# granularai/fabric

Measured on AMD Instinct MI355X. Metric: patch-pairs/sec (fwd+bwd) 13-band 128x128, higher is better.
Workload: dtype bf16

## Files before the change

fabric_amd/_lib.py:

```python
import ctypes as C
import os

_HERE = os.path.dirname(os.path.abspath(__file__))
LIB_PATH = os.environ.get('BIDATE_LIB') or os.path.join(_HERE, 'csrc', 'libbidate_hip.so')

BDN_F32, BDN_BF16, BDN_BF16X3, BDN_BF16X2 = 0, 1, 2, 3
IN_PLAIN, IN_BNRELU = 0, 1
EVAL_STAGE, EVAL_PAIR, EVAL_CLS = 0, 1, 2
WG_SIMPLE, WG_ROLE = 1, 5


def wg_flags(phases=3, kernel=0, blocks=0):
    return phases | (kernel << 8) | (blocks << 16)

_vp, _i, _f, _sz, _i64 = C.c_void_p, C.c_int, C.c_float, C.c_size_t, C.c_int64
_hf = C.POINTER(C.c_float)

SIGNATURES = {
    'bdn_last_error': (C.c_char_p, []),
    'bdn_version': (_i, []),
    'bdn_stream_create': (_i, [_i, C.POINTER(C.c_void_p)]),
    'bdn_stream_destroy': (_i, [_vp]),
    'bdn_event_create': (_i, [C.POINTER(C.c_void_p)]),
    'bdn_event_destroy': (_i, [_vp]),
    'bdn_event_record': (_i, [_vp, _vp]),
    'bdn_stream_wait_event': (_i, [_vp, _vp]),
    'bdn_pack_input': (_i, [_i, _vp, _vp, _vp, _i, _i, _i, _i, _i, _vp]),
    'bdn_pack_weights': (_i, [_i, _vp, _vp, _vp, _i, _i, _i, _vp]),
    'bdn_pack_weights_multi': (_i, [_i, _vp, _i, _vp]),
    'bdn_conv3x3': (_i, [_i, _vp, _i, _vp, _i, _i, _vp, _i, _vp, _vp, _vp, _vp, _i, _i, _i, _i, _vp]),
    'bdn_conv3x3_x3src': (_i, [_i, _vp, _i, _i, _vp, _i, _vp, _vp, _vp, _vp, _vp, _i, _i, _i, _i, _vp]),
    'bdn_conv3x3_num_mtiles': (_i, [_i, _i, _i, _i, _i]),
    'bdn_conv3x3_num_mtiles_ex': (_i, [_i, _i, _i, _i, _i, _i, _i]),
    'bdn_wgrad_workspace_bytes': (_sz, [_i, _i, _i, _i, _i, _i]),
    'bdn_conv3x3_wgrad': (_i, [_i, _vp, _i, _vp, _i, _vp, _i, _i, _vp, _i, _vp, _vp, _i, _i, _i, _i, _vp]),
    'bdn_conv3x3_wgrad_ex': (_i, [_i, _vp, _i, _vp, _i, _vp, _i, _i, _vp, _i, _vp, _vp, _i, _i, _i, _i, _i, _vp]),
    'bdn_conv3x3_wgrad_variant': (_i, [_i, _i, _i, _i, _i, _i, _i, _i, _i, _i]),
    'bdn_wgrad_workspace_bytes_ex': (_sz, [_i, _i, _i, _i, _i, _i, _i, _i, _i, _i]),
    'bdn_conv3x3_wgrad_bnbwd_supported': (_i, [_i, _i, _i, _i, _i, _i, _i]),
    'bdn_conv3x3_wgrad_bnbwd': (_i, [_i, _vp, _i, _vp, _vp, _vp, _i, _i, _vp, _i, _vp, _vp, _i, _i, _i, _i, _vp]),
    'bdn_conv3x3_dgrad_first': (_i, [_i, _vp, _i, _vp, _vp, _vp, _i, _vp, _i, _vp, _vp, _i, _i, _i, _vp]),
    'bdn_bn_finalize_workspace_bytes': (_sz, [_i, _i, _i]),
    'bdn_bn_finalize': (_i, [_vp, _i, _i, _i, _i, _vp, _vp, _f, _f, _vp, _vp, _vp, _vp, _vp, _vp]),
    'bdn_bn_eval': (_i, [_vp, _vp, _vp, _vp, _f, _i, _i, _vp, _vp]),
    'bdn_bn_eval_fold_multi': (_i, [_vp, _i, _i, _f, _vp]),
    'bdn_conv3x3_eval': (_i, [_i, _vp, _i, _vp, _i, _vp, _vp, _vp, _vp, _vp, _vp, _i, _i, _i, _i, _vp]),
    'bdn_conv3x3_eval_pair': (_i, [_i, _vp, _i, _vp, _vp, _vp, _vp, _vp, _i, _i, _i, _i, _vp]),
    'bdn_conv3x3_eval_cls': (_i, [_i, _vp, _i, _vp, _vp, _vp, _vp, _vp, _vp, _i, _vp, _vp, _vp, _i, _i, _i, _i, _i, _i, _vp]),
    'bdn_bn_bwd_workspace_bytes': (_sz, [_i, _i, _i, _i, _i, _i]),
    'bdn_bn_bwd': (_i, [_i, _vp, _i, _vp, _vp, _i, _i, _i, _i, _i, _vp, _vp, _vp, _vp, _vp, _vp]),
    'bdn_conv3d_num_mtiles': (_i, [_i, _i, _i, _i]),
    'bdn_conv3d': (_i, [_i, _vp, _i, _i, _vp, _i, _vp, _vp, _vp, _vp, _i, _i, _i, _i, _i, _vp]),
    'bdn_conv3d_wgrad': (_i, [_i, _vp, _i, _vp, _i, _vp, _vp, _i, _i, _i, _i, _i, _vp]),
    'bdn_split_pack': (_i, [_vp, _i, _vp, _i, _i, _vp, _i, _vp, _i, _i, _i, _vp]),
    'bdn_bnrelu': (_i, [_i, _vp, _vp, _i, _vp, _i, _i, _i, _i, _vp]),
    'bdn_bnrelu_pool': (_i, [_i, _vp, _vp, _i, _vp, _i, _i, _i, _i, _vp]),
    'bdn_fuse_product': (_i, [_i, _vp, _vp, _vp, _i, _i, _i, _i, _vp]),
    'bdn_product_pool': (_i, [_i, _vp, _vp, _vp, _vp, _i, _i, _i, _i, _vp]),
    'bdn_upsample2x': (_i, [_i, _vp, _i, _vp, _vp, _i, _i, _i, _i, _i, _i, _vp]),
    'bdn_product_pool_split': (_i, [_vp, _vp, _vp, _i, _i, _vp, _i, _i, _i, _i, _vp]),
    'bdn_upsample2x_split': (_i, [_vp, _i, _vp, _vp, _i, _i, _i, _i, _i, _i, _i, _i, _i, _vp]),
    'bdn_upsample2x_bwd': (_i, [_i, _vp, _i, _vp, _i, _i, _i, _i, _i, _i, _vp]),
    'bdn_upsample2x_bwd_rows': (_i, [_i, _i, _i, _i, _i]),
    'bdn_upsample2x_bwd_bs': (_i, [_i, _vp, _i, _vp, _vp, _vp, _vp, _i, _i, _i, _i, _i, _i, _vp]),
    'bdn_enc_skip_bwd': (_i, [_i, _vp, _i, _vp, _vp, _vp, _vp, _vp, _i, _i, _i, _i, _vp]),
    'bdn_enc_skip_bwd_rows': (_i, [_i, _i, _i, _i, _i]),
    'bdn_outc_fwd': (_i, [_i, _vp, _vp, _vp, _vp, _vp, _i, _i, _i, _i, _i, _vp]),
    'bdn_outc_bwd_workspace_bytes': (_sz, [_i, _i, _i, _i, _i, _i]),
    'bdn_outc_bwd': (_i, [_i, _vp, _vp, _vp, _vp, _vp, _vp, _vp, _vp, _vp, _i, _i, _i, _i, _i, _vp]),
    'bdn_outc_bn_bwd_apply': (_i, [_i, _vp, _vp, _vp, _vp, _i, _vp, _vp, _i, _i, _i, _i, _i, _vp]),
    'bdn_outc_bwd_rows': (_i, [_i, _i, _i, _i, _i]),
    'bdn_overlap_workspace_bytes': (_sz, [_i, _i, _i, _i, _i]),
    'bdn_tversky': (_i, [_vp, _vp, _f, _f, _f, _vp, _vp, _vp, _vp, _i, _i, _i, _i, _vp]),
    'bdn_conv3x3_variant': (C.c_char_p, [_i, _i, _i, _i, _i, _i, _i, _i]),
    'bdn_conv3x3_dgrad_bb_variant': (C.c_char_p, [_i, _i, _i, _i, _i]),
    'bdn_conv3x3_eval_variant': (C.c_char_p, [_i, _i, _i, _i, _i, _i, _i, _i]),
    'bdn_conv3x3_x3src_variant': (C.c_char_p, [_i, _i, _i, _i, _i, _i, _i]),
    'bdn_conv3x3_dgrad_bs': (_i, [_i, _vp, _i, _vp, _vp, _vp, _vp, _i, _vp, _i, _i, _i, _i, _vp]),
    'bdn_conv3x3_dgrad_bb': (_i, [_i, _vp, _i, _vp, _vp, _vp, _i, _vp, _vp, _vp, _vp, _vp, _vp, _i, _i, _i, _i, _vp]),
    'bdn_bn_bwd_scratch_bytes': (_sz, [_i, _i]),
    'bdn_bn_bwd_finalize': (_i, [_vp, _i, _i, _vp, _i, _i, _vp, _vp, _vp, _vp, _vp]),
    'bdn_bn_bwd_apply': (_i, [_i, _vp, _i, _vp, _vp, _i, _i, _i, _i, _i, _vp, _i, _i, _vp, _vp, _vp, _vp, _vp, _vp]),
    'bdn_bn_bwd_apply_split': (_i, [_vp, _i, _vp, _vp, _i, _i, _i, _i, _i, _vp, _i, _i, _vp, _vp, _vp, _vp, _vp, _vp]),
    'bdn_bn_bwd_finalize_frozen': (_i, [_vp, _i, _i, _vp, _i, _i, _vp, _vp, _vp, _vp, _vp, _vp]),
    'bdn_bn_bwd_apply_frozen': (_i, [_i, _vp, _i, _vp, _vp, _i, _i, _i, _i, _i, _vp, _i, _i, _vp, _vp, _vp, _vp, _vp, _vp, _vp]),
    'bdn_bn_bwd_frozen': (_i, [_i, _vp, _i, _vp, _vp, _i, _i, _i, _i, _i, _vp, _vp, _vp, _vp, _vp, _vp, _vp]),
    'bdn_overlap_loss': (_i, [_vp, _vp, _f, _f, _f, _i, _vp, _vp, _vp, _vp, _i, _i, _i, _i, _vp]),
    'bdn_focal_workspace_bytes': (_sz, []),
    'bdn_focal': (_i, [_vp, _vp, _f, _vp, _i, _vp, _vp, _vp, _vp, _i, _i, _i, _i, _vp]),
    'bdn_criterion_workspace_bytes': (_sz, [_i, _i, _i, _i, _i]),
    'bdn_criterion': (_i, [_vp, _vp, _f, _f, _f, _f, _i, _f, _f, _vp, _i, _vp, _vp, _vp, _vp, _vp, _i, _i, _i, _i, _vp]),
    'bdn_ingest_band': (_i, [_i, _vp, _i, _i, _f, _f, _vp, _i, _i, _vp]),
    'bdn_gather_tiles': (_i, [_i, _vp, _vp, _vp, _vp, _i, _i, _i, _i, _i, _i, _vp]),
    'bdn_upload_band': (_i, [_vp, _vp, _i, _i, _i, _i, _i, _vp]),
    'bdn_argmax': (_i, [_vp, _vp, _i, _i, _i, _i, _vp]),
    'bdn_argmax_stitch': (_i, [_vp, _vp, _vp, _i, _i, _i, _i, _i, _vp]),
    'bdn_gather_tiles_sym': (_i, [_i, _vp, _vp, _vp, _vp, _i, _i, _i, _i, _i, _i, _vp]),
    'bdn_blend_fold': (_i, [_vp, _vp, _vp, _vp, _i, _i, _i, _vp]),
    'bdn_blend_stitch': (_i, [_vp, _vp, _vp, _vp, C.c_longlong, _i, _i, _i, _i, _i, _i, _i, _vp]),
    'bdn_blend_finalize': (_i, [_vp, _vp, _vp, _i, _i, _i, _vp]),
    'bdn_sample_patches': (_i, [_vp, _vp, _i, _i, _vp, _vp, _i, _i, _vp, _vp, _vp, _vp]),
    'bdn_sgd_step': (_i, [_vp, _vp, _f, _f, _sz, _vp]),
    'bdn_sgd_momentum_step': (_i, [_vp, _vp, _vp, _f, _f, _f, _f, _f, _i, _i, _sz, _vp]),
    'bdn_adam_step': (_i, [_vp, _vp, _vp, _vp, _f, _f, C.c_double, C.c_double, _f, _f, _i, _i64, _sz, _vp]),
    'bdn_sgd_step_grouped': (_i, [_vp, _vp, _vp, _vp, _i, _i, _vp, _f, _sz, _vp]),
    'bdn_sgd_momentum_step_grouped': (_i, [_vp, _vp, _vp, _vp, _vp, _i, _i, _vp, _vp, _f, _f, _f, _i, _i, _sz, _vp]),
    'bdn_adam_step_grouped': (_i, [_vp, _vp, _vp, _vp, _vp, _vp, _i, _i, _vp, _vp, _f, C.c_double, C.c_double, _f, _i, _i64, _sz, _vp]),
    'bdn_sgd_step_grouped_ex': (_i, [_vp, _vp, _vp, _vp, _i, _i, _hf, _f, _vp, _sz, _vp]),
    'bdn_sgd_momentum_step_grouped_ex': (_i, [_vp, _vp, _vp, _vp, _vp, _i, _i, _hf, _hf, _f, _vp, _f, _f, _i, _i, _sz, _vp]),
    'bdn_adam_step_grouped_ex': (_i, [_vp, _vp, _vp, _vp, _vp, _vp, _i, _i, _hf, _hf, _f, _vp, C.c_double, C.c_double, _f, _i, _i64, _sz,
                                      _vp]),
    'bdn_grad_accumulate': (_i, [_vp, _vp, _sz, _i, _vp]),
    'bdn_grad_norm_workspace_bytes': (_sz, [_sz]),
    'bdn_grad_norm': (_i, [_vp, _vp, _vp, _i, _f, _f, _vp, _vp, _sz, _vp]),
}


def floats(values):
    return (C.c_float * len(values))(*values)

_lib = None


def load():
    global _lib
    if _lib is not None:
        return _lib
    if not os.path.exists(LIB_PATH):
        raise RuntimeError(
            f'fabric_amd: HIP extension {LIB_PATH} not found. Build it with '
            f'`python -c "import __graft_entry__ as g; g.build()"` or `make -C fabric_amd/csrc`. '
            f'There is no CPU fallback.')
    lib = C.CDLL(LIB_PATH)
    for name, (res, args) in SIGNATURES.items():
        fn = getattr(lib, name)
        fn.restype = res
        fn.argtypes = args
    _lib = lib
    return lib


def ptr(t):
    return None if t is None else t.data_ptr()


PROFILE = None
PHASE = ''
_ext_streams = {}


def _profiled(lib, name, args):
    import torch
    h = args[-1] or 0
    st = _ext_streams.get(h)
    if st is None:
        st = _ext_streams[h] = torch.cuda.ExternalStream(h) if h else torch.cuda.default_stream()
    e0, e1 = torch.cuda.Event(enable_timing=True), torch.cuda.Event(enable_timing=True)
    e0.record(st)
    rc = getattr(lib, name)(*args)
    e1.record(st)
    PROFILE.append((name, PHASE, h, e0, e1))
    return rc


SKIP = None


def call(name, *args):
    lib = load()
    if SKIP is not None and SKIP(name, args):
        return
    if PROFILE is not None and SIGNATURES[name][1] and SIGNATURES[name][1][-1] is _vp and not name.startswith(('bdn_stream', 'bdn_event')):
        rc = _profiled(lib, name, args)
    else:
        rc = getattr(lib, name)(*args)
    if rc != 0:
        msg = lib.bdn_last_error().decode(errors='replace')
        raise RuntimeError(f'{name} failed (rc={rc}): {msg}')


def stream_ptr():
    import torch
    return torch.cuda.current_stream().cuda_stream
```

fabric_amd/csrc/head.hip:

```cpp
#include "common.hpp"

static inline unsigned grid_for(size_t n, int block = 256) { return (unsigned)((n + block - 1) / block); }

template <typename T>
__global__ void pack_input_kernel(const float* __restrict__ x1, const float* __restrict__ x2, T* __restrict__ out,
                                  int B, int C, int H, int W, int Cpad, FastDiv dhw, FastDiv dupp) {
    constexpr int EPU = ET<T>::EPU;
    const int upp = Cpad / EPU;
    const size_t hw = (size_t)H * W, total = (size_t)2 * B * hw * upp;
    const size_t i = (size_t)blockIdx.x * blockDim.x + threadIdx.x;
    if (i >= total) return;
    int ti, pi, n, u; dhw.divmod((int)i, ti, pi); dupp.divmod(ti, n, u);
    const size_t p = pi;
    const float* src = (n < B ? x1 + (size_t)n * C * hw : x2 + (size_t)(n - B) * C * hw) + p;
    float f[EPU];
#pragma unroll
    for (int e = 0; e < EPU; e++) { const int c = u * EPU + e; f[e] = c < C ? src[(size_t)c * hw] : 0.f; }
    *reinterpret_cast<uint4*>(out + ((size_t)n * hw + p) * Cpad + u * EPU) = Unit<T>::pack(f);
}

__global__ void pack_input_split_kernel(const float* __restrict__ x1, const float* __restrict__ x2, bf16s* __restrict__ out,
                                        int B, int C, int H, int W, int Cpad, FastDiv dhw, FastDiv dupp) {
    const int upp = Cpad / 8;
    const size_t hw = (size_t)H * W, total = (size_t)2 * B * hw * upp;
// ... 110 lines not shown
            if (wf) {
                const int tap = rec_l >> 2, kq = rec_l & 3;
                const size_t rec = ((size_t)cb * 9 + tap) * (d.Cin / 16) + (ci0 / 16 + kq);
                *reinterpret_cast<uint4*>(wf + rec * 512 + lane * 8) =
                    *reinterpret_cast<const uint4*>(t + (lane & 31) * ROW + tap * 64 + kq * 16 + (lane >> 5) * 8);
            }
            if (wd) {
                const int cbi = rec_l / 18, rem = rec_l % 18, tap = rem >> 1, kg = rem & 1;
                const int ci = cbi * 32 + (lane & 31), co8 = kg * 16 + (lane >> 5) * 8;
                unsigned short h[8];
#pragma unroll
                for (int e = 0; e < 8; e++) h[e] = t[(co8 + e) * ROW + tap * 64 + ci];
                const size_t rec = ((size_t)(ci0 / 32 + cbi) * 9 + (8 - tap)) * (d.Cout / 16) + (co0 / 16 + kg);
                *reinterpret_cast<uint4*>(wd + rec * 512 + lane * 8) =
                    make_uint4(h[0] | ((unsigned)h[1] << 16), h[2] | ((unsigned)h[3] << 16), h[4] | ((unsigned)h[5] << 16), h[6] | ((unsigned)h[7] << 16));
            }
        }
    }
}
__global__ void pack_weights_irregular_kernel(const PackDesc* __restrict__ desc) {
    if (pack_regular(desc[blockIdx.y])) return;
    constexpr int EPU = 8, KCH = 16, REC = 64 * EPU;
    const PackDesc d = desc[blockIdx.y];
    const size_t total = (size_t)d.Cout * 9 * d.Cinp;
    bf16s* wf = reinterpret_cast<bf16s*>(d.wf); bf16s* wd = reinterpret_cast<bf16s*>(d.wd);
    for (size_t i = (size_t)blockIdx.x * blockDim.x + threadIdx.x; i < total; i += (size_t)gridDim.x * blockDim.x) {
        const int e = i % EPU, lane = (i / EPU) % 64; const size_t rec = i / REC;
        if (wf) {
            const int kgi = rec % (d.Cinp / KCH); const size_t t = rec / (d.Cinp / KCH); const int tap = t % 9, cb = t / 9;
            const int co = cb * 32 + (lane & 31), ci = kgi * KCH + (lane >> 5) * EPU + e;
            wf[i] = from_f<bf16s>(ci < d.Cin ? d.w[((size_t)co * d.Cin + ci) * 9 + tap] : 0.f);
        }
        if (wd) {
            const int kgi = rec % (d.Cout / KCH); const size_t t = rec / (d.Cout / KCH); const int tap = t % 9, cb = t / 9;
            const int ci = cb * 32 + (lane & 31), co = kgi * KCH + (lane >> 5) * EPU + e;
            wd[i] = from_f<bf16s>(ci < d.Cin ? d.w[((size_t)co * d.Cin + ci) * 9 + (8 - tap)] : 0.f);
        }
    }
}

extern "C" int bdn_pack_weights_multi(int dtype, const void* desc, int n_layers, void* stream) {
    if (!desc || n_layers <= 0) BDN_FAIL(BDN_E_ARG, "pack_weights_multi: bad arguments");
    hipStream_t st = (hipStream_t)stream;
    if (dtype == BDN_BF16) {
        hipLaunchKernelGGL(pack_weights_tiles_kernel, dim3(1024), dim3(256), 0, st, (const PackDesc*)desc, n_layers);
        hipLaunchKernelGGL(pack_weights_irregular_kernel, dim3(32, n_layers), dim3(256), 0, st, (const PackDesc*)desc);
    }
    else if (dtype == BDN_F32) hipLaunchKernelGGL(pack_weights_multi_kernel<float>, dim3(256, n_layers), dim3(256), 0, st, (const PackDesc*)desc);
    else if (dtype == BDN_BF16X3) return bdn_pack_weights_x3_multi((const PackDesc*)desc, n_layers, st);
    else BDN_FAIL(BDN_E_ARG, "pack_weights_multi: bad dtype");
    BDN_CHECK_LAUNCH("pack_weights_multi");
    return BDN_OK;
}

constexpr int OUTC_MAXCLS = 8;
constexpr int OUTC_ITERS = 16;
constexpr int OUTC_BWD_ITERS = 32;
template <typename T, int NC, int CUC = 0>
__global__ __launch_bounds__(256) void outc_fwd_kernel(const T* __restrict__ z, const float* __restrict__ bn, const float* __restrict__ w,
                                const float* __restrict__ bias, float* __restrict__ logits, int npix, int hw, int C, int ncls, FastDiv dhw) {
    constexpr int EPU = ET<T>::EPU;
    const int CU = CUC ? CUC : C / EPU, rows = 256 / CU, tid = threadIdx.x, cu = tid % CU, row = tid / CU, c = cu * EPU;
    float sc[EPU], sh[EPU], wk[NC][EPU], bk[NC];
#pragma unroll
    for (int i = 0; i < EPU; i++) { sc[i] = bn_row(bn, 0, 2, C)[c + i]; sh[i] = bn_row(bn, 0, 3, C)[c + i]; }
#pragma unroll
    for (int k = 0; k < NC; k++) {
        const int kk = k < ncls ? k : 0;
        const float bv = bias[kk];
        bk[k] = k < ncls ? bv : 0.f;
#pragma unroll
        for (int i = 0; i < EPU; i++) { const float wv = w[kk * C + c + i]; wk[k][i] = k < ncls ? wv : 0.f; }
    }
    const int p_begin = blockIdx.x * rows * OUTC_ITERS, p_end = min(npix, p_begin + rows * OUTC_ITERS);
    uint4 u[4], un[4];
#define OUTC_LOAD4(dst_, p0_, RAGGED_)                                                                   \
    _Pragma("unroll") for (int j = 0; j < 4; j++) {                                                      \
        const int p_ = (p0_) + j * rows + row;                                                          \
        dst_[j] = *reinterpret_cast<const uint4*>(z + (size_t)(!(RAGGED_) || p_ < p_end ? p_ : (p0_)) * C + c); \
    }
#define OUTC_RUN(RAGGED_)                                                                                \
    {                                                                                                   \
        OUTC_LOAD4(u, p_begin, RAGGED_)                                                                 \
        for (int p0 = p_begin; p0 < p_end; p0 += 4 * rows) {                       \
            const bool more = p0 + 4 * rows < p_end;                                                    \
             \
                                    \
            { const int pn_ = more ? p0 + 4 * rows : p0; OUTC_LOAD4(un, pn_, RAGGED_) }                  \
            _Pragma("unroll") for (int j = 0; j < 4; j++) {                                              \
                const int p = p0 + j * rows + row;                                                      \
                if ((RAGGED_) && p0 + j * rows >= p_end) break;                      \
                const bool in_ = !(RAGGED_) || p < p_end;                                               \
                float f[EPU], acc[NC];                                                                  \
                _Pragma("unroll") for (int k = 0; k < NC; k++) acc[k] = 0.f;                             \
                Unit<T>::unpack(u[j], f);                                                               \
                _Pragma("unroll") for (int i = 0; i < EPU; i++) {                                        \
                    const float a = to_f(from_f<T>(fmaxf(fmaf(f[i], sc[i], sh[i]), 0.f)));              \
                    _Pragma("unroll") for (int k = 0; k < NC; k++) acc[k] = fmaf(a, wk[k][i], acc[k]);   \
                }                                                                                       \
                if constexpr (CUC != 0) {                                                               \
                    _Pragma("unroll") for (int k = 0; k < NC; k++) acc[k] = first_lane_sum<CUC ? CUC : 8>(acc[k]); \
                } else {                                                                                \
                    _Pragma("unroll") for (int k = 0; k < NC; k++)                                       \
                        for (int off = CU >> 1; off > 0; off >>= 1) acc[k] += __shfl_xor(acc[k], off);  \
                }                                                                                       \
                if (cu == 0 && in_) {                                                                   \
                    int b, q; dhw.divmod(p, b, q);                                                      \
                    _Pragma("unroll") for (int k = 0; k < NC; k++) if (k < ncls) logits[((size_t)b * ncls + k) * hw + q] = acc[k] + bk[k]; \
                }                                                                                       \
            }                                                                                           \
            _Pragma("unroll") for (int j = 0; j < 4; j++) u[j] = un[j];                                  \
        }                                                                                               \
    }
    if (p_begin >= p_end) return;
    if (p_begin + rows * OUTC_ITERS <= npix) OUTC_RUN(false) else OUTC_RUN(true)
#undef OUTC_RUN
#undef OUTC_LOAD4
}

extern "C" int bdn_outc_fwd(int dtype, const void* z, const float* bn, const float* w, const float* b,
                            float* logits, int B, int H, int W, int C, int ncls, void* stream) {
    if (!z || !bn || !w || !b || !logits) BDN_FAIL(BDN_E_ARG, "outc_fwd: null pointer");
    if (ncls < 1 || ncls > OUTC_MAXCLS || C % 16 || C > 512 || 512 % C) BDN_FAIL(BDN_E_SHAPE, "outc_fwd: ncls=%d (max %d), C=%d", ncls, OUTC_MAXCLS, C);
    hipStream_t st = (hipStream_t)stream; const int npix = B * H * W, hw = H * W;
    if (dtype == BDN_BF16) {
        const int per = 256 / (C / 8) * OUTC_ITERS; const unsigned grid = (npix + per - 1) / per;
        if (ncls <= 2 && C == 64) hipLaunchKernelGGL((outc_fwd_kernel<bf16s, 2, 8>), dim3(grid), dim3(256), 0, st, (const bf16s*)z, bn, w, b, logits, npix, hw, C, ncls, FastDiv(hw));
        else if (ncls <= 2) hipLaunchKernelGGL((outc_fwd_kernel<bf16s, 2>), dim3(grid), dim3(256), 0, st, (const bf16s*)z, bn, w, b, logits, npix, hw, C, ncls, FastDiv(hw));
        else hipLaunchKernelGGL((outc_fwd_kernel<bf16s, OUTC_MAXCLS>), dim3(grid), dim3(256), 0, st, (const bf16s*)z, bn, w, b, logits, npix, hw, C, ncls, FastDiv(hw));
    } else if (dtype == BDN_F32) {
        const int per = 256 / (C / 4) * OUTC_ITERS; const unsigned grid = (npix + per - 1) / per;
        if (ncls <= 2 && C == 64) hipLaunchKernelGGL((outc_fwd_kernel<float, 2, 16>), dim3(grid), dim3(256), 0, st, (const float*)z, bn, w, b, logits, npix, hw, C, ncls, FastDiv(hw));
        else if (ncls <= 2) hipLaunchKernelGGL((outc_fwd_kernel<float, 2>), dim3(grid), dim3(256), 0, st, (const float*)z, bn, w, b, logits, npix, hw, C, ncls, FastDiv(hw));
        else hipLaunchKernelGGL((outc_fwd_kernel<float, OUTC_MAXCLS>), dim3(grid), dim3(256), 0, st, (const float*)z, bn, w, b, logits, npix, hw, C, ncls, FastDiv(hw));
    }
    else BDN_FAIL(BDN_E_ARG, "outc_fwd: bad dtype");
    BDN_CHECK_LAUNCH("outc_fwd");
    return BDN_OK;
}

template <typename T, int NC, int CUC = 0>
__global__ __launch_bounds__(256) void outc_bwd_kernel(const float* __restrict__ dl, const T* __restrict__ z, const float* __restrict__ bn,
                                const float* __restrict__ w, T* __restrict__ dA, float* __restrict__ wpart,
                                float* __restrict__ bs_partial, int npix, int hw, int C, int ncls, FastDiv dhw) {
    constexpr int EPU = ET<T>::EPU;
    extern __shared__ float sm[];
    const int CU = CUC ? CUC : C / EPU, rows = 256 / CU, tid = threadIdx.x, cu = tid % CU, row = tid / CU, c = cu * EPU;
    for (int i = tid; i < ncls * (C + 1); i += 256) sm[i] = 0.f;
    float sc[EPU], sh[EPU], wk[NC][EPU], acc[NC][EPU], accb[NC], t0[EPU], t1[EPU];
#pragma unroll
    for (int i = 0; i < EPU; i++) { sc[i] = bn_row(bn, 0, 2, C)[c + i]; sh[i] = bn_row(bn, 0, 3, C)[c + i]; t0[i] = 0.f; t1[i] = 0.f; }
    const bool bs = bs_partial != nullptr;
#pragma unroll
    for (int k = 0; k < NC; k++) {
        accb[k] = 0.f;
        const int kk = k < ncls ? k : 0;
#pragma unroll
        for (int i = 0; i < EPU; i++) { const float wv = w[kk * C + c + i]; wk[k][i] = k < ncls ? wv : 0.f; acc[k][i] = 0.f; }
    }
    __syncthreads();
    const int p_begin = blockIdx.x * rows * OUTC_BWD_ITERS, p_end = min(npix, p_begin + rows * OUTC_BWD_ITERS);
    uint4 zu[4], zn[4]; float gv[4][NC], gn[4][NC];
#define OUTC_BLOAD4(zd_, gd_, p0_)                                                                       \
    _Pragma("unroll") for (int j = 0; j < 4; j++) {                                                      \
        const int pj_ = (p0_) + j * rows + row < p_end ? (p0_) + j * rows + row : p_begin + row;          \
        int b_, q_; dhw.divmod(pj_, b_, q_);                                                            \
        _Pragma("unroll") for (int k = 0; k < NC; k++) gd_[j][k] = dl[((size_t)b_ * ncls + (k < ncls ? k : 0)) * hw + q_]; \
        zd_[j] = *reinterpret_cast<const uint4*>(z + (size_t)pj_ * C + c);                              \
    }
    if (p_begin + row < p_end) {
        OUTC_BLOAD4(zu, gv, p_begin)
        for (int p0 = p_begin; p0 < p_end; p0 += 4 * rows) {
            { const int pn_ = p0 + 4 * rows < p_end ? p0 + 4 * rows : p0; OUTC_BLOAD4(zn, gn, pn_) }
#pragma unroll
            for (int j = 0; j < 4; j++) {
                const int p = p0 + j * rows + row;
                if (p < p_end) {
                    float g[NC], f[EPU], o[EPU];
#pragma unroll
                    for (int k = 0; k < NC; k++) g[k] = k < ncls ? gv[j][k] : 0.f;
                    Unit<T>::unpack(zu[j], f);
#pragma unroll
                    for (int i = 0; i < EPU; i++) {
                        const float a = to_f(from_f<T>(fmaxf(fmaf(f[i], sc[i], sh[i]), 0.f)));
                        float s = 0.f;
#pragma unroll
                        for (int k = 0; k < NC; k++) if (k < ncls) { s = fmaf(g[k], wk[k][i], s); acc[k][i] = fmaf(g[k], a, acc[k][i]); }
                        o[i] = s;
                    }
                    if (cu == 0) {
#pragma unroll
                        for (int k = 0; k < NC; k++) accb[k] += g[k];
                    }
                    const uint4 uo = Unit<T>::pack(o);
                    if (dA) *reinterpret_cast<uint4*>(dA + (size_t)p * C + c) = uo;
                    if (bs) {
                        Unit<T>::unpack(uo, o);
#pragma unroll
                        for (int i = 0; i < EPU; i++) {
                            const float gm = fmaf(f[i], sc[i], sh[i]) > 0.f ? o[i] : 0.f;
                            t0[i] += gm; t1[i] = fmaf(gm, f[i], t1[i]);
                        }
                    }
                }
            }
#pragma unroll
            for (int j = 0; j < 4; j++) {
                zu[j] = zn[j];
#pragma unroll
                for (int k = 0; k < NC; k++) gv[j][k] = gn[j][k];
            }
        }
    }
#undef OUTC_BLOAD4
    {
        float* red = sm + ncls * (C + 1);
#pragma unroll
        for (int k = 0; k < NC; k++) {
            if (k < ncls) {
                __syncthreads();
#pragma unroll
                for (int i = 0; i < EPU; i++) red[tid * EPU + i] = acc[k][i];
                if (cu == 0) red[256 * EPU + row] = accb[k];
                __syncthreads();
                for (int o = tid; o <= C; o += 256) {
                    float v = 0.f;
                    if (o < C) { const int ccu = o / EPU, i = o % EPU; for (int r = 0; r < rows; r++) v += red[(r * CU + ccu) * EPU + i]; }
                    else for (int r = 0; r < rows; r++) v += red[256 * EPU + r];
                    sm[k * (C + 1) + o] = v;
                }
            }
        }
    }
    __syncthreads();
    for (int i = tid; i < ncls * (C + 1); i += 256)
        wpart[(size_t)blockIdx.x * ncls * (C + 1) + i] = sm[i];
    if (bs) {
        float* sred = sm + ncls * (C + 1);
#pragma unroll
        for (int i = 0; i < EPU; i++) { sred[(tid * EPU + i) * 2] = t0[i]; sred[(tid * EPU + i) * 2 + 1] = t1[i]; }
        __syncthreads();
        for (int o = tid; o < C * 2; o += 256) {
            const int k = o & 1, cc = o >> 1, ccu = cc / EPU, i = cc % EPU;
            float v = 0.f;
            for (int r = 0; r < rows; r++) v += sred[((r * CU + ccu) * EPU + i) * 2 + k];
            bs_partial[((size_t)blockIdx.x * 2 + k) * C + cc] = v;
        }
    }
}

__global__ __launch_bounds__(256) void outc_dw_reduce_kernel(const float* __restrict__ wpart, int rows, int C, int ncls,
                                                             float* __restrict__ dw, float* __restrict__ db) {
    __shared__ float sm[256];
    const int o = blockIdx.x, n = ncls * (C + 1);
    float a = 0.f;
    for (int r = threadIdx.x; r < rows; r += 256) a += wpart[(size_t)r * n + o];
    sm[threadIdx.x] = a;
    __syncthreads();
    for (int st = 128; st >= 1; st >>= 1) {
        if ((int)threadIdx.x < st) sm[threadIdx.x] += sm[threadIdx.x + st];
        __syncthreads();
    }
    if (threadIdx.x == 0) {
        const int k = o / (C + 1), cc = o % (C + 1);
        if (cc < C) dw[k * C + cc] = sm[0]; else db[k] = sm[0];
    }
}

extern "C" int bdn_outc_bwd_rows(int dtype, int B, int H, int W, int C) {
    if (B <= 0 || H <= 0 || W <= 0 || C <= 0 || C % 16 || C > 1024 || 1024 % C) return 0;
    const int per = 256 / (C / (dtype == BDN_BF16 ? 8 : 4)) * OUTC_BWD_ITERS;
    return (B * H * W + per - 1) / per;
}

extern "C" size_t bdn_outc_bwd_workspace_bytes(int dtype, int B, int H, int W, int C, int ncls) {
    const int rows = bdn_outc_bwd_rows(dtype, B, H, W, C);
    if (rows <= 0 || ncls < 1 || ncls > OUTC_MAXCLS) return 0;
    return (size_t)rows * ncls * (C + 1) * sizeof(float);
}

extern "C" int bdn_outc_bwd(int dtype, const float* dlogits, const void* z, const float* bn, const float* w,
                            void* dA, float* dw, float* db, float* bs_partial, float* ws, int B, int H, int W, int C, int ncls, void* stream) {
    if (!dlogits || !z || !bn || !w || !dw || !db || !ws) BDN_FAIL(BDN_E_ARG, "outc_bwd: null pointer");
    if (!dA && !bs_partial) BDN_FAIL(BDN_E_ARG, "outc_bwd: dA may be omitted only together with bs_partial (bdn_outc_bn_bwd_apply recomputes it)");
    if (ncls < 1 || ncls > OUTC_MAXCLS || C % 16 || C > 1024 || 1024 % C) BDN_FAIL(BDN_E_SHAPE, "outc_bwd: bad shape");
    hipStream_t st = (hipStream_t)stream; const int npix = B * H * W;
    const unsigned grid = bdn_outc_bwd_rows(dtype, B, H, W, C);
    const size_t smem = sizeof(float) * (ncls * (C + 1) + 256 * (dtype == BDN_BF16 ? 8 : 4) * 2);
    if (dtype == BDN_BF16) {
        if (ncls <= 2 && C == 64) hipLaunchKernelGGL((outc_bwd_kernel<bf16s, 2, 8>), dim3(grid), dim3(256), smem, st, dlogits, (const bf16s*)z, bn, w, (bf16s*)dA, ws, bs_partial, npix, H * W, C, ncls, FastDiv(H * W));
        else if (ncls <= 2) hipLaunchKernelGGL((outc_bwd_kernel<bf16s, 2>), dim3(grid), dim3(256), smem, st, dlogits, (const bf16s*)z, bn, w, (bf16s*)dA, ws, bs_partial, npix, H * W, C, ncls, FastDiv(H * W));
        else hipLaunchKernelGGL((outc_bwd_kernel<bf16s, OUTC_MAXCLS>), dim3(grid), dim3(256), smem, st, dlogits, (const bf16s*)z, bn, w, (bf16s*)dA, ws, bs_partial, npix, H * W, C, ncls, FastDiv(H * W));
    } else if (dtype == BDN_F32) {
        if (ncls <= 2 && C == 64) hipLaunchKernelGGL((outc_bwd_kernel<float, 2, 16>), dim3(grid), dim3(256), smem, st, dlogits, (const float*)z, bn, w, (float*)dA, ws, bs_partial, npix, H * W, C, ncls, FastDiv(H * W));
        else if (ncls <= 2) hipLaunchKernelGGL((outc_bwd_kernel<float, 2>), dim3(grid), dim3(256), smem, st, dlogits, (const float*)z, bn, w, (float*)dA, ws, bs_partial, npix, H * W, C, ncls, FastDiv(H * W));
        else hipLaunchKernelGGL((outc_bwd_kernel<float, OUTC_MAXCLS>), dim3(grid), dim3(256), smem, st, dlogits, (const float*)z, bn, w, (float*)dA, ws, bs_partial, npix, H * W, C, ncls, FastDiv(H * W));
    } else BDN_FAIL(BDN_E_ARG, "outc_bwd: bad dtype");
    BDN_CHECK_LAUNCH("outc_bwd");
    hipLaunchKernelGGL(outc_dw_reduce_kernel, dim3(ncls * (C + 1)), dim3(256), 0, st, ws, (int)grid, C, ncls, dw, db);
    BDN_CHECK_LAUNCH("outc_dw_reduce");
    return BDN_OK;
}

template <typename T, int NC, bool SPLIT = false>
__global__ __launch_bounds__(256) void outc_bn_bwd_apply_kernel(const float* __restrict__ dl, const float* __restrict__ w,
                                const T* __restrict__ z, const float* __restrict__ bn, const float* __restrict__ sums,
                                T* __restrict__ dz, int npix, int hw, int pix_per_group, int pix_per_block, int C, int ncls, FastDiv dhw, FastDiv dppg) {
    constexpr int EPU = ET<T>::EPU;
    const int CU = C / EPU, rows = 256 / CU, tid = threadIdx.x, cu = tid % CU, row = tid / CU, c = cu * EPU;
    const int p_begin = blockIdx.x * pix_per_block, p_end = min(npix, p_begin + pix_per_block);
    if (p_begin >= p_end) return;
    const float invM = 1.f / (float)pix_per_group;
    int gcur = -1;
    float mean[EPU], inv[EPU], sc[EPU], sh[EPU], k0[EPU], k1[EPU], wk[NC][EPU];
#pragma unroll
    for (int k = 0; k < NC; k++)
#pragma unroll
        for (int i = 0; i < EPU; i++) wk[k][i] = k < ncls ? w[k * C + c + i] : 0.f;
    for (int pb = p_begin + row; pb < p_end; pb += 4 * rows) {
        uint4 zu[4]; float gv[4][NC];
#pragma unroll
        for (int j = 0; j < 4; j++) {
            const int pj = pb + j * rows < p_end ? pb + j * rows : pb;
            int b, q; dhw.divmod(pj, b, q);
#pragma unroll
            for (int k = 0; k < NC; k++) gv[j][k] = k < ncls ? dl[((size_t)b * ncls + k) * hw + q] : 0.f;
            zu[j] = *reinterpret_cast<const uint4*>(z + (size_t)pj * C + c);
        }
#pragma unroll
        for (int j = 0; j < 4; j++) {
            const int p = pb + j * rows;
            if (p >= p_end) break;
            const int g = dppg.div(p);
            if (g != gcur) {
                gcur = g;
#pragma unroll
                for (int i = 0; i < EPU; i++) {
                    mean[i] = bn_row(bn, g, 0, C)[c + i]; inv[i] = bn_row(bn, g, 1, C)[c + i];
                    sc[i] = bn_row(bn, g, 2, C)[c + i]; sh[i] = bn_row(bn, g, 3, C)[c + i];
                    k0[i] = sums[((size_t)g * 2 + 0) * C + c + i] * invM;
                    k1[i] = sums[((size_t)g * 2 + 1) * C + c + i] * invM;
                }
            }
            float fz[EPU], o[EPU];
            Unit<T>::unpack(zu[j], fz);
#pragma unroll
            for (int i = 0; i < EPU; i++) {
                float s = 0.f;
#pragma unroll
                for (int k = 0; k < NC; k++) if (k < ncls) s = fmaf(gv[j][k], wk[k][i], s);
                o[i] = s;
            }
            Unit<T>::unpack(Unit<T>::pack(o), o);
#pragma unroll
            for (int i = 0; i < EPU; i++) {
                const float gm = fmaf(fz[i], sc[i], sh[i]) > 0.f ? o[i] : 0.f;
                const float xhat = (fz[i] - mean[i]) * inv[i];
                o[i] = sc[i] * (gm - k0[i] - xhat * k1[i]);
            }
            if constexpr (SPLIT) {
                const SplitOut so = {reinterpret_cast<bf16s*>(dz), 2 * C, 0, C};
                store_split4(so, (size_t)p, c, o);
            } else
            *reinterpret_cast<uint4*>(dz + (size_t)p * C + c) = Unit<T>::pack(o);
        }
    }
}

extern "C" int bdn_outc_bn_bwd_apply(int dtype, const float* dlogits, const float* w, const void* z, const float* bn,
                                     int imgs_per_group, const float* sums, void* dz, int B, int H, int W, int C, int ncls, void* stream) {
    if (!dlogits || !w || !z || !bn || !sums || !dz) BDN_FAIL(BDN_E_ARG, "outc_bn_bwd_apply: null pointer");
    if (ncls < 1 || ncls > OUTC_MAXCLS || C % 16 || C > 1024 || 1024 % C || B <= 0 || H <= 0 || W <= 0 || imgs_per_group <= 0 || B % imgs_per_group)
        BDN_FAIL(BDN_E_SHAPE, "outc_bn_bwd_apply: bad shape");
    hipStream_t st = (hipStream_t)stream;
    const int npix = B * H * W, epu = dtype == BDN_BF16 ? 8 : 4, rows = 256 / (C / epu);
    int ppb = (npix + 2047) / 2048; if (ppb < 2 * rows) ppb = 2 * rows; ppb = (ppb + rows - 1) / rows * rows;
    const unsigned grid = (npix + ppb - 1) / ppb;
    if (dtype == BDN_BF16X3) {
#define OUTC_APPLY_S(NC_) hipLaunchKernelGGL((outc_bn_bwd_apply_kernel<float, NC_, true>), dim3(grid), dim3(256), 0, st, dlogits, w, (const float*)z, bn, sums, \
                                               (float*)dz, npix, H * W, imgs_per_group * H * W, ppb, C, ncls, FastDiv(H * W), FastDiv(imgs_per_group * H * W))
        if (ncls <= 2) OUTC_APPLY_S(2); else OUTC_APPLY_S(OUTC_MAXCLS);
#undef OUTC_APPLY_S
        BDN_CHECK_LAUNCH("outc_bn_bwd_apply");
        return BDN_OK;
    }
#define OUTC_APPLY(T_, NC_) hipLaunchKernelGGL((outc_bn_bwd_apply_kernel<T_, NC_>), dim3(grid), dim3(256), 0, st, dlogits, w, (const T_*)z, bn, sums, \
                                               (T_*)dz, npix, H * W, imgs_per_group * H * W, ppb, C, ncls, FastDiv(H * W), FastDiv(imgs_per_group * H * W))
    if (dtype == BDN_BF16) { if (ncls <= 2) OUTC_APPLY(bf16s, 2); else OUTC_APPLY(bf16s, OUTC_MAXCLS); }
    else if (dtype == BDN_F32) { if (ncls <= 2) OUTC_APPLY(float, 2); else OUTC_APPLY(float, OUTC_MAXCLS); }
    else BDN_FAIL(BDN_E_ARG, "outc_bn_bwd_apply: bad dtype");
#undef OUTC_APPLY
    BDN_CHECK_LAUNCH("outc_bn_bwd_apply");
    return BDN_OK;
}

struct FocalStats { const float* calpha; float gamma; double* part; };
__device__ __forceinline__ float focal_mod(float pt, float gamma) { return gamma == 0.f ? 1.f : powf(fmaxf(1.f - pt, 0.f), gamma); }

template <int NC, bool FOCAL = false>
__global__ void tversky_sums_kernel(const float* __restrict__ logits, const uint8_t* __restrict__ labels,
                                    float* __restrict__ part, int32_t* __restrict__ pcounts, int B, int ncls, int H, int W,
                                    int rows_per_block, int We, FastDiv dH, FocalStats fs = {}) {
    extern __shared__ float sm[];
    const int CW = blockDim.y, RL = blockDim.x;
    const int cl = threadIdx.y, rl = threadIdx.x;
    const int x = blockIdx.x * CW + cl;
    const size_t hw = (size_t)H * W;
    float tp[NC], fp[NC], fn[NC];
#pragma unroll
    for (int k = 0; k < NC; k++) { tp[k] = 0.f; fp[k] = 0.f; fn[k] = 0.f; }
    int c_tp = 0, c_fp = 0, c_fn = 0, c_ok = 0;
    double facc = 0.0;
    const int rows = B * H, r_end = min(rows, (int)(blockIdx.y + 1) * rows_per_block);
    if (x < W)
        for (int r0 = blockIdx.y * rows_per_block + rl; r0 < r_end; r0 += 4 * RL) {
            float lv[4][NC]; int tv[4];
#pragma unroll
            for (int u = 0; u < 4; u++) {
                const int r = r0 + u * RL;
                const int rr = r < r_end ? r : r0;
                int b, y; dH.divmod(rr, b, y);
                const size_t q = (size_t)y * W + x;
#pragma unroll
                for (int k = 0; k < NC; k++) lv[u][k] = k < ncls ? logits[((size_t)b * ncls + k) * hw + q] : -INFINITY;
                tv[u] = labels[(size_t)b * hw + q];
            }
#pragma unroll
            for (int u = 0; u < 4; u++) {
                if (r0 + u * RL >= r_end) break;
                float l[NC]; float m = -INFINITY; int am = 0;
#pragma unroll
                for (int k = 0; k < NC; k++) { l[k] = lv[u][k]; if (l[k] > m) { m = l[k]; am = k; } }
                float den = 0.f;
#pragma unroll
                for (int k = 0; k < NC; k++) { l[k] = k < ncls ? expf(l[k] - m) : 0.f; den += l[k]; }
                const int t = tv[u];
                const float inv = 1.f / den;
                float pt = 0.f;
#pragma unroll
                for (int k = 0; k < NC; k++) {
                    const float p = l[k] * inv;
                    if (t == k) { tp[k] += p; fn[k] += 1.f - p; pt = p; } else fp[k] += p;
                }
                if constexpr (FOCAL) {
                    float ltm = 0.f;
#pragma unroll
                    for (int k = 0; k < NC; k++) if (k < ncls && t == k) ltm = lv[u][k] - m;
                    const float a = t < ncls ? (fs.calpha ? fs.calpha[t] : 1.f) : 0.f;
                    facc += (double)(-focal_mod(pt, fs.gamma) * a * (ltm - logf(den)));
                }
                c_tp += (am == 1 && t == 1); c_fp += (am == 1 && t != 1); c_fn += (am != 1 && t == 1); c_ok += (am == t);
            }
        }
#pragma unroll
    for (int k = 0; k < NC; k++) {
        sm[(rl * 3 * NC + 0 * NC + k) * CW + cl] = tp[k];
        sm[(rl * 3 * NC + 1 * NC + k) * CW + cl] = fp[k];
        sm[(rl * 3 * NC + 2 * NC + k) * CW + cl] = fn[k];
    }
    __syncthreads();
    const int nblk_lin = blockIdx.y * gridDim.x + blockIdx.x;
    if (We == W) {
        if (rl == 0 && x < W)
            for (int k = 0; k < ncls; k++)
#pragma unroll
                for (int j = 0; j < 3; j++) {
                    float v = 0.f;
                    for (int r = 0; r < RL; r++) v += sm[(r * 3 * NC + j * NC + k) * CW + cl];
                    part[(size_t)blockIdx.y * 3 * ncls * W + (j * ncls + k) * W + x] = v;
                }
    } else {
        const int tid = rl + RL * cl;
        if (tid < 3 * NC) {
            float v = 0.f;
            for (int i = 0; i < RL * CW; i++) {
                const int r = i / CW, c = i % CW;
                if (blockIdx.x * CW + c < W) v += sm[(r * 3 * NC + tid) * CW + c];
            }
            const int j = tid / NC, k = tid % NC;
            if (k < ncls) part[(size_t)nblk_lin * 3 * ncls + j * ncls + k] = v;
        }
    }
    {
        int* ism = reinterpret_cast<int*>(sm);
        __syncthreads();
        const int tid = rl * CW + cl;
        ism[tid * 4 + 0] = c_tp; ism[tid * 4 + 1] = c_fp; ism[tid * 4 + 2] = c_fn; ism[tid * 4 + 3] = c_ok;
        __syncthreads();
        if (tid < 4) { int v = 0; for (int i = 0; i < 256; i++) v += ism[i * 4 + tid]; pcounts[nblk_lin * 4 + tid] = v; }
        if constexpr (FOCAL) {
            double* dsm = reinterpret_cast<double*>(sm);
            __syncthreads();
            dsm[tid] = facc;
            __syncthreads();
            for (int s = 128; s > 0; s >>= 1) { if (tid < s) dsm[tid] += dsm[tid + s]; __syncthreads(); }
            if (tid == 0) fs.part[nblk_lin] = dsm[0];
        }
    }
}

struct FocalFinish { const double* part; int nfp; double scale; float w_o, w_f; float* terms; };
template <bool FOCAL = false>
__global__ __launch_bounds__(1024) void tversky_finish_kernel(float* __restrict__ sums, const float* __restrict__ part, int nblk,
                                      const int32_t* __restrict__ pcounts, int ncblk, int32_t* __restrict__ counts,
                                      float alpha, float beta, float eps, int ncls, int W, float* __restrict__ loss,
                                      FocalFinish ff = {}) {
    __shared__ double red[256];
    __shared__ float4 lane_sums[1024];
    const int n = 3 * ncls * W, tid = threadIdx.x;
    if (n % 4 == 0 && n / 4 <= 1024) {
        const int n4 = n / 4, LN = 1024 / n4 > 0 ? (1024 / n4 > 16 ? 16 : 1024 / n4) : 1;
        const int q = tid % n4, l = tid / n4;
        float4 a = make_float4(0.f, 0.f, 0.f, 0.f);
        if (l < LN) {
#pragma unroll 8
            for (int b = l; b < nblk; b += LN) {
                const float4 v = *reinterpret_cast<const float4*>(part + (size_t)b * n + 4 * q);
                a.x += v.x; a.y += v.y; a.z += v.z; a.w += v.w;
            }
            lane_sums[tid] = a;
        }
        __syncthreads();
        if (l == 0) {
            for (int k = 1; k < LN; k++) { const float4 v = lane_sums[k * n4 + q]; a.x += v.x; a.y += v.y; a.z += v.z; a.w += v.w; }
            *reinterpret_cast<float4*>(sums + 4 * q) = a;
        }
    } else {
        for (int i = tid; i < n; i += 1024) {
            float a = 0.f;
            for (int b = 0; b < nblk; b++) a += part[(size_t)b * n + i];
            sums[i] = a;
        }
    }
    if (counts) {
        int* ired = reinterpret_cast<int*>(lane_sums);
        __syncthreads();
        const int j = tid & 3, l = tid >> 2;
        int v = 0;
        for (int b = l; b < ncblk; b += 256) v += pcounts[b * 4 + j];
        ired[tid] = v;
        __syncthreads();
        for (int s2 = 512; s2 >= 4; s2 >>= 1) { if (tid < s2) ired[tid] += ired[tid + s2]; __syncthreads(); }
        if (tid < 4) counts[tid] = ired[tid];
    }
    __syncthreads();
    double acc = 0.0;
    const int nc = ncls * W;
    if (tid < 256)
        for (int i = tid; i < nc; i += 256) {
            const float tp = sums[i], fp = sums[nc + i], fn = sums[2 * nc + i];
            const float D = tp + alpha * fp + beta * fn + eps;
            acc += (double)(tp / D);
            sums[i] = 1.f / D; sums[nc + i] = tp / (D * D);
        }
    if (tid < 256) red[tid] = acc;
    __syncthreads();
    for (int s = 128; s > 0; s >>= 1) { if (tid < s) red[tid] += red[tid + s]; __syncthreads(); }
    if constexpr (FOCAL) {
        const float ov = (float)(1.0 - red[0] / nc);
        __syncthreads();
        double f = 0.0;
        if (tid < 256) { for (int i = tid; i < ff.nfp; i += 256) f += ff.part[i]; red[tid] = f; }
        __syncthreads();
        for (int s = 128; s > 0; s >>= 1) { if (tid < s) red[tid] += red[tid + s]; __syncthreads(); }
        if (tid == 0) {
            const float fo = (float)(red[0] * ff.scale);
            *loss = ff.w_o * ov + ff.w_f * fo;
            if (ff.terms) { ff.terms[0] = ov; ff.terms[1] = fo; }
        }
    } else
    if (tid == 0) *loss = (float)(1.0 - red[0] / nc);
}

struct FocalBwd { const float* calpha; float gamma, gscale, w_o, w_f; };
template <bool FOCAL = false>
__global__ void tversky_bwd_kernel(const float* __restrict__ logits, const uint8_t* __restrict__ labels,
                                   const float* __restrict__ coef, float alpha, float beta, float* __restrict__ dlogits,
                                   int B, int ncls, int H, int Wimg, int W, FastDiv dhw, FastDiv dWimg, FocalBwd fb = {}) {
    const size_t hw = (size_t)H * Wimg, npix = (size_t)B * hw;
    const size_t p = (size_t)blockIdx.x * blockDim.x + threadIdx.x;
    if (p >= npix) return;
    int bi, qi, yi, xi; dhw.divmod((int)p, bi, qi); dWimg.divmod(qi, yi, xi);
    const size_t b = bi, q = qi; const int x = W == 1 ? 0 : xi;
    const int n = ncls * W;
    float l[OUTC_MAXCLS], dp[OUTC_MAXCLS]; float m = -INFINITY;
#pragma unroll
    for (int k = 0; k < OUTC_MAXCLS; k++) if (k < ncls) { l[k] = logits[(b * ncls + k) * hw + q]; m = fmaxf(m, l[k]); }
    float den = 0.f;
#pragma unroll
    for (int k = 0; k < OUTC_MAXCLS; k++) if (k < ncls) { l[k] = expf(l[k] - m); den += l[k]; }
    const int t = labels[p];
    const float norm = -1.f / (float)n;
    float dot = 0.f;
#pragma unroll
    for (int k = 0; k < OUTC_MAXCLS; k++) if (k < ncls) {
        l[k] /= den;
        const float invD = coef[k * W + x], tpD2 = coef[n + k * W + x];
        const float tk = t == k ? 1.f : 0.f;
        dp[k] = norm * (tk * invD - tpD2 * (tk + alpha * (1.f - tk) - beta * tk));
        dot += l[k] * dp[k];
    }
    if constexpr (FOCAL) {
        float pt = 0.f;
#pragma unroll
        for (int k = 0; k < OUTC_MAXCLS; k++) if (k < ncls && k == t) pt = l[k];
        const float a = t < ncls ? (fb.calpha ? fb.calpha[t] : 1.f) : 0.f;
        const float c = -focal_mod(pt, fb.gamma) * a * fb.gscale;
#pragma unroll
        for (int k = 0; k < OUTC_MAXCLS; k++) if (k < ncls)
            dlogits[(b * ncls + k) * hw + q] = fb.w_o * (l[k] * (dp[k] - dot)) + fb.w_f * (c * ((k == t ? 1.f : 0.f) - l[k]));
    } else {
#pragma unroll
    for (int k = 0; k < OUTC_MAXCLS; k++) if (k < ncls) dlogits[(b * ncls + k) * hw + q] = l[k] * (dp[k] - dot);
    }
}

struct OverlapPlan { int We, CW, RL, rpb, gx, gy, nblk, n; };
static OverlapPlan overlap_plan(int B, int ncls, int H, int W, int reduce_w) {
    OverlapPlan p;
    p.We = reduce_w ? 1 : W;
    p.CW = 1; while (p.CW < W && p.CW < 256) p.CW *= 2;
    p.RL = 256 / p.CW;
    const int rows = B * H;
    p.rpb = (rows + 255) / 256; if (p.rpb < p.RL) p.rpb = p.RL;
    p.gx = (W + p.CW - 1) / p.CW; p.gy = (rows + p.rpb - 1) / p.rpb;
    p.nblk = reduce_w ? p.gx * p.gy : p.gy;
    p.n = 3 * ncls * p.We;
    return p;
}
extern "C" size_t bdn_overlap_workspace_bytes(int B, int ncls, int H, int W, int reduce_w) {
    if (B <= 0 || H <= 0 || W <= 0 || ncls < 2 || ncls > OUTC_MAXCLS) return 0;
    const OverlapPlan p = overlap_plan(B, ncls, H, W, reduce_w);
    return sizeof(float) * ((size_t)p.n * (p.nblk + 1) + 8) + sizeof(int32_t) * 4 * p.gx * p.gy;
}

extern "C" int bdn_overlap_loss(const float* logits, const uint8_t* labels, float alpha, float beta, float eps,
                                int reduce_w, float* ws, float* loss, int32_t* counts, float* dlogits,
                                int B, int ncls, int H, int W, void* stream) {
    if (!logits || !labels || !ws || !loss) BDN_FAIL(BDN_E_ARG, "overlap_loss: null pointer");
    if (ncls < 2 || ncls > OUTC_MAXCLS) BDN_FAIL(BDN_E_SHAPE, "overlap_loss: ncls=%d unsupported (2..%d)", ncls, OUTC_MAXCLS);
    if (B <= 0 || H <= 0 || W <= 0 || (size_t)B * H * W >= ((size_t)1 << 31)) BDN_FAIL(BDN_E_SHAPE, "overlap_loss: bad shape");
    hipStream_t st = (hipStream_t)stream;
    const OverlapPlan p = overlap_plan(B, ncls, H, W, reduce_w);
    const int We = p.We;
    float* part = ws + p.n;
    int32_t* pcounts = reinterpret_cast<int32_t*>(part + (size_t)p.nblk * p.n);
    dim3 grid(p.gx, p.gy), block(p.RL, p.CW);
    if (ncls <= 2) hipLaunchKernelGGL((tversky_sums_kernel<2, false>), grid, block, sizeof(float) * 256 * 3 * 2, st, logits, labels, part, pcounts, B, ncls, H, W, p.rpb, We, FastDiv(H), FocalStats{});
    else hipLaunchKernelGGL((tversky_sums_kernel<OUTC_MAXCLS, false>), grid, block, sizeof(float) * 256 * 3 * OUTC_MAXCLS, st, logits, labels, part, pcounts, B, ncls, H, W, p.rpb, We, FastDiv(H), FocalStats{});
    BDN_CHECK_LAUNCH("tversky_sums");
    hipLaunchKernelGGL(tversky_finish_kernel<false>, dim3(1), dim3(1024), 0, st, ws, part, p.nblk, pcounts, p.gx * p.gy, counts, alpha, beta, eps, ncls, We, loss, FocalFinish{});
    BDN_CHECK_LAUNCH("tversky_finish");
    if (dlogits) {
        hipLaunchKernelGGL(tversky_bwd_kernel<false>, dim3(grid_for((size_t)B * H * W)), dim3(256), 0, st, logits, labels, ws, alpha, beta, dlogits, B, ncls, H, W, We, FastDiv(H * W), FastDiv(W), FocalBwd{});
        BDN_CHECK_LAUNCH("tversky_bwd");
    }
    return BDN_OK;
}

extern "C" int bdn_tversky(const float* logits, const uint8_t* labels, float alpha, float beta, float eps,
                           float* ws, float* loss, int32_t* counts, float* dlogits,
                           int B, int ncls, int H, int W, void* stream) {
    return bdn_overlap_loss(logits, labels, alpha, beta, eps, 0, ws, loss, counts, dlogits, B, ncls, H, W, stream);
}

__global__ void focal_kernel(const float* __restrict__ logits, const uint8_t* __restrict__ labels,
                             const float* __restrict__ alpha, float gamma, float gscale,
                             double* __restrict__ part, int32_t* __restrict__ counts, float* __restrict__ dlogits,
                             int B, int ncls, size_t hw) {
    __shared__ double red[256];
    __shared__ int ired[256 * 4];
    const size_t npix = (size_t)B * hw;
    double acc = 0.0;
    int c_tp = 0, c_fp = 0, c_fn = 0, c_ok = 0;
    for (size_t p = (size_t)blockIdx.x * 256 + threadIdx.x; p < npix; p += (size_t)gridDim.x * 256) {
        const size_t b = p / hw, q = p % hw;
        float l[OUTC_MAXCLS]; float m = -INFINITY; int am = 0;
#pragma unroll
        for (int k = 0; k < OUTC_MAXCLS; k++) if (k < ncls) { l[k] = logits[(b * ncls + k) * hw + q]; if (l[k] > m) { m = l[k]; am = k; } }
        float den = 0.f;
#pragma unroll
        for (int k = 0; k < OUTC_MAXCLS; k++) if (k < ncls) den += expf(l[k] - m);
        const int t = labels[p];
        const float logden = logf(den);
        float ltm = 0.f;
#pragma unroll
        for (int k = 0; k < OUTC_MAXCLS; k++) if (k < ncls && k == t) ltm = l[k] - m;
        const float logpt = ltm - logden, pt = expf(logpt);
        const float a = t < ncls ? (alpha ? alpha[t] : 1.f) : 0.f;
        const float mod = gamma == 0.f ? 1.f : powf(fmaxf(1.f - pt, 0.f), gamma);
        acc += (double)(-mod * a * logpt);
        if (dlogits) {
            const float c = -mod * a * gscale;
#pragma unroll
            for (int k = 0; k < OUTC_MAXCLS; k++) if (k < ncls)
                dlogits[(b * ncls + k) * hw + q] = c * ((k == t ? 1.f : 0.f) - expf((l[k] - m) - logden));
        }
        c_tp += (am == 1 && t == 1); c_fp += (am == 1 && t != 1); c_fn += (am != 1 && t == 1); c_ok += (am == t);
    }
    red[threadIdx.x] = acc;
    ired[threadIdx.x * 4 + 0] = c_tp; ired[threadIdx.x * 4 + 1] = c_fp; ired[threadIdx.x * 4 + 2] = c_fn; ired[threadIdx.x * 4 + 3] = c_ok;
    __syncthreads();
    for (int s = 128; s > 0; s >>= 1) { if (threadIdx.x < s) red[threadIdx.x] += red[threadIdx.x + s]; __syncthreads(); }
    if (threadIdx.x == 0) part[blockIdx.x] = red[0];
    if (counts && threadIdx.x < 4) { int v = 0; for (int i = 0; i < 256; i++) v += ired[i * 4 + threadIdx.x]; atomicAdd(&counts[threadIdx.x], v); }
}

__global__ void focal_finish_kernel(const double* __restrict__ part, int nblk, double scale, float* __restrict__ loss) {
    __shared__ double red[256];
    double acc = 0.0;
    for (int i = threadIdx.x; i < nblk; i += 256) acc += part[i];
    red[threadIdx.x] = acc; __syncthreads();
    for (int s = 128; s > 0; s >>= 1) { if (threadIdx.x < s) red[threadIdx.x] += red[threadIdx.x + s]; __syncthreads(); }
    if (threadIdx.x == 0) *loss = (float)(red[0] * scale);
}

extern "C" size_t bdn_focal_workspace_bytes(void) { return sizeof(double) * 1024; }

extern "C" int bdn_focal(const float* logits, const uint8_t* labels, float gamma, const float* alpha, int size_average,
                         void* ws, float* loss, int32_t* counts, float* dlogits,
                         int B, int ncls, int H, int W, void* stream) {
    if (!logits || !labels || !ws || !loss) BDN_FAIL(BDN_E_ARG, "focal: null pointer");
    if (ncls < 2 || ncls > OUTC_MAXCLS) BDN_FAIL(BDN_E_SHAPE, "focal: ncls=%d unsupported (2..%d)", ncls, OUTC_MAXCLS);
    if (B <= 0 || H <= 0 || W <= 0 || gamma < 0.f) BDN_FAIL(BDN_E_SHAPE, "focal: bad shape or negative gamma");
    hipStream_t st = (hipStream_t)stream;
    const size_t npix = (size_t)B * H * W;
    int nblk = (int)((npix + 255) / 256); if (nblk > 1024) nblk = 1024;
    if (counts) hipMemsetAsync(counts, 0, sizeof(int32_t) * 4, st);
    const double inv = size_average ? 1.0 / (double)npix : 1.0;
    hipLaunchKernelGGL(focal_kernel, dim3(nblk), dim3(256), 0, st, logits, labels, alpha, gamma, (float)inv,
                       (double*)ws, counts, dlogits, B, ncls, (size_t)H * W);
    BDN_CHECK_LAUNCH("focal");
    hipLaunchKernelGGL(focal_finish_kernel, dim3(1), dim3(256), 0, st, (const double*)ws, nblk, inv, loss);
    BDN_CHECK_LAUNCH("focal_finish");
    return BDN_OK;
}

__global__ void criterion_terms_kernel(const float* __restrict__ loss, float* __restrict__ terms, int slot) {
    terms[slot] = *loss; terms[1 - slot] = 0.f;
}

static inline size_t criterion_focal_part_bytes(const OverlapPlan& p) { return (sizeof(double) * p.gx * p.gy + 15) / 16 * 16; }

extern "C" size_t bdn_criterion_workspace_bytes(int B, int ncls, int H, int W, int reduce_w) {
    const size_t ov = bdn_overlap_workspace_bytes(B, ncls, H, W, reduce_w);
    if (ov == 0 || (size_t)B * H * W >= ((size_t)1 << 31)) return 0;
    const size_t compound = criterion_focal_part_bytes(overlap_plan(B, ncls, H, W, reduce_w)) + ov, focal = bdn_focal_workspace_bytes();
    return compound > focal ? compound : focal;
}

extern "C" int bdn_criterion(const float* logits, const uint8_t* labels, float w_overlap, float alpha, float beta, float eps, int reduce_w,
                             float w_focal, float gamma, const float* class_alpha, int size_average, void* ws, float* loss, float* terms,
                             int32_t* counts, float* dlogits, int B, int ncls, int H, int W, void* stream) {
    if (!logits || !labels || !ws || !loss) BDN_FAIL(BDN_E_ARG, "criterion: null pointer");
    if (!(w_overlap >= 0.f) || !(w_focal >= 0.f)) BDN_FAIL(BDN_E_ARG, "criterion: negative weight (w_overlap=%g, w_focal=%g)", w_overlap, w_focal);
    if (w_overlap == 0.f && w_focal == 0.f) BDN_FAIL(BDN_E_ARG, "criterion: both weights are zero");
    if (!(gamma >= 0.f)) BDN_FAIL(BDN_E_ARG, "criterion: negative gamma");
    if (ncls < 2 || ncls > OUTC_MAXCLS) BDN_FAIL(BDN_E_SHAPE, "criterion: ncls=%d unsupported (2..%d)", ncls, OUTC_MAXCLS);
    if (B <= 0 || H <= 0 || W <= 0 || (size_t)B * H * W >= ((size_t)1 << 31)) BDN_FAIL(BDN_E_SHAPE, "criterion: bad shape (B*H*W must stay below 2^31)");
    if ((uintptr_t)ws & 15) BDN_FAIL(BDN_E_ARG, "criterion: ws must be 16-byte aligned");
    hipStream_t st = (hipStream_t)stream;
    if ((w_focal == 0.f && w_overlap == 1.f) || (w_overlap == 0.f && w_focal == 1.f)) {
        const int focal = w_overlap == 0.f;
        const int rc = focal ? bdn_focal(logits, labels, gamma, class_alpha, size_average, ws, loss, counts, dlogits, B, ncls, H, W, stream)
                             : bdn_overlap_loss(logits, labels, alpha, beta, eps, reduce_w, (float*)ws, loss, counts, dlogits, B, ncls, H, W, stream);
        if (rc != BDN_OK || !terms) return rc;
        hipLaunchKernelGGL(criterion_terms_kernel, dim3(1), dim3(1), 0, st, loss, terms, focal);
        BDN_CHECK_LAUNCH("criterion_terms");
        return BDN_OK;
    }
    const OverlapPlan p = overlap_plan(B, ncls, H, W, reduce_w);
    double* fpart = (double*)ws;
    float* sums = (float*)((char*)ws + criterion_focal_part_bytes(p));
    float* part = sums + p.n;
    int32_t* pcounts = reinterpret_cast<int32_t*>(part + (size_t)p.nblk * p.n);
    const double inv = size_average ? 1.0 / (double)((size_t)B * H * W) : 1.0;
    const FocalStats fs{class_alpha, gamma, fpart};
    dim3 grid(p.gx, p.gy), block(p.RL, p.CW);
    if (ncls <= 2) hipLaunchKernelGGL((tversky_sums_kernel<2, true>), grid, block, sizeof(float) * 256 * 3 * 2, st, logits, labels, part, pcounts, B, ncls, H, W, p.rpb, p.We, FastDiv(H), fs);
    else hipLaunchKernelGGL((tversky_sums_kernel<OUTC_MAXCLS, true>), grid, block, sizeof(float) * 256 * 3 * OUTC_MAXCLS, st, logits, labels, part, pcounts, B, ncls, H, W, p.rpb, p.We, FastDiv(H), fs);
    BDN_CHECK_LAUNCH("criterion_stats");
    hipLaunchKernelGGL(tversky_finish_kernel<true>, dim3(1), dim3(1024), 0, st, sums, part, p.nblk, pcounts, p.gx * p.gy, counts, alpha, beta, eps, ncls, p.We, loss,
                       FocalFinish{fpart, p.gx * p.gy, inv, w_overlap, w_focal, terms});
    BDN_CHECK_LAUNCH("criterion_finish");
    if (dlogits) {
        hipLaunchKernelGGL(tversky_bwd_kernel<true>, dim3(grid_for((size_t)B * H * W)), dim3(256), 0, st, logits, labels, sums, alpha, beta, dlogits, B, ncls, H, W, p.We,
                           FastDiv(H * W), FastDiv(W), FocalBwd{class_alpha, gamma, (float)inv, w_overlap, w_focal});
        BDN_CHECK_LAUNCH("criterion_bwd");
    }
    return BDN_OK;
}

__global__ void sgd_kernel(float* __restrict__ p, const float* __restrict__ g, float step, size_t n4, size_t n) {
    const size_t i = (size_t)blockIdx.x * blockDim.x + threadIdx.x;
    if (i < n4) {
        float4 a = reinterpret_cast<float4*>(p)[i]; const float4 b = reinterpret_cast<const float4*>(g)[i];
        a.x -= step * b.x; a.y -= step * b.y; a.z -= step * b.z; a.w -= step * b.w;
        reinterpret_cast<float4*>(p)[i] = a;
    }
    if (i == 0) for (size_t k = n4 * 4; k < n; k++) p[k] -= step * g[k];
}

extern "C" int bdn_sgd_step(float* params, const float* grads, float lr, float grad_scale, size_t n, void* stream) {
    if (!params || !grads) BDN_FAIL(BDN_E_ARG, "sgd_step: null pointer");
    if (((uintptr_t)params | (uintptr_t)grads) & 15) BDN_FAIL(BDN_E_ARG, "sgd_step: buffers must be 16-byte aligned");
    if (n == 0) return BDN_OK;
    const size_t n4 = n / 4;
    hipLaunchKernelGGL(sgd_kernel, dim3(grid_for(n4 > 0 ? n4 : 1)), dim3(256), 0, (hipStream_t)stream, params, grads, lr * grad_scale, n4, n);
    BDN_CHECK_LAUNCH("sgd_step");
    return BDN_OK;
}

constexpr int OPT_VEC = 4;

static inline unsigned opt_grid(size_t n4) {
    const size_t b = (n4 + 256 * OPT_VEC - 1) / (256 * OPT_VEC);
    return (unsigned)(b == 0 ? 1 : (b < 2048 ? b : 2048));
}

struct SgdmParams { float lr, grad_scale, momentum, damp1 , weight_decay; int first, nesterov; };

template <bool MOM>
__device__ __forceinline__ void sgdm_elem(float& p, float gr, float& buf, const SgdmParams& a) {
    float g = a.grad_scale * gr;
    if (a.weight_decay != 0.f) g = g + a.weight_decay * p;
    if (MOM) {
        buf = a.first ? g : a.momentum * buf + a.damp1 * g;
        g = a.nesterov ? g + a.momentum * buf : buf;
    }
    p = p - a.lr * g;
}

template <bool MOM>
__global__ void __launch_bounds__(256) sgdm_kernel(float* __restrict__ p, const float* __restrict__ g, float* __restrict__ buf,
                                                   SgdmParams a, size_t n4, size_t n) {
    const size_t stride = (size_t)gridDim.x * 256;
    for (size_t base = (size_t)blockIdx.x * 256 + threadIdx.x; base < n4; base += stride * OPT_VEC) {
        float4 P[OPT_VEC], G[OPT_VEC], M[OPT_VEC] = {};
#pragma unroll
        for (int u = 0; u < OPT_VEC; u++) {
            const size_t i = base + u * stride;
            if (i < n4) {
                P[u] = reinterpret_cast<const float4*>(p)[i]; G[u] = reinterpret_cast<const float4*>(g)[i];
                if (MOM && !a.first) M[u] = reinterpret_cast<const float4*>(buf)[i];
            }
        }
#pragma unroll
        for (int u = 0; u < OPT_VEC; u++) {
            const size_t i = base + u * stride;
            if (i < n4) {
                sgdm_elem<MOM>(P[u].x, G[u].x, M[u].x, a); sgdm_elem<MOM>(P[u].y, G[u].y, M[u].y, a);
                sgdm_elem<MOM>(P[u].z, G[u].z, M[u].z, a); sgdm_elem<MOM>(P[u].w, G[u].w, M[u].w, a);
                reinterpret_cast<float4*>(p)[i] = P[u];
                if (MOM) reinterpret_cast<float4*>(buf)[i] = M[u];
            }
        }
    }
    if (blockIdx.x == 0 && threadIdx.x < n - n4 * 4) {
        const size_t k = n4 * 4 + threadIdx.x;
        float m = (MOM && !a.first) ? buf[k] : 0.f, q = p[k];
        sgdm_elem<MOM>(q, g[k], m, a);
        p[k] = q;
        if (MOM) buf[k] = m;
    }
}

extern "C" int bdn_sgd_momentum_step(float* params, const float* grads, float* momentum_buf, float lr, float grad_scale, float momentum,
                                     float dampening, float weight_decay, int nesterov, int first_step, size_t n, void* stream) {
    if (!params || !grads) BDN_FAIL(BDN_E_ARG, "sgd_momentum_step: null pointer");
    if ((momentum != 0.f) != (momentum_buf != nullptr))
        BDN_FAIL(BDN_E_ARG, "sgd_momentum_step: momentum_buf must be given iff momentum != 0");
    if (nesterov && (momentum <= 0.f || dampening != 0.f))
        BDN_FAIL(BDN_E_ARG, "sgd_momentum_step: nesterov needs momentum > 0 and zero dampening");
    if (((uintptr_t)params | (uintptr_t)grads | (uintptr_t)momentum_buf) & 15)
        BDN_FAIL(BDN_E_ARG, "sgd_momentum_step: buffers must be 16-byte aligned");
    if (n == 0) return BDN_OK;
    const size_t n4 = n / 4;
    const SgdmParams a{lr, grad_scale, momentum, (float)(1.0 - (double)dampening), weight_decay, first_step ? 1 : 0, nesterov ? 1 : 0};
    if (momentum_buf)
        hipLaunchKernelGGL(sgdm_kernel<true>, dim3(opt_grid(n4)), dim3(256), 0, (hipStream_t)stream, params, grads, momentum_buf, a, n4, n);
    else
        hipLaunchKernelGGL(sgdm_kernel<false>, dim3(opt_grid(n4)), dim3(256), 0, (hipStream_t)stream, params, grads, momentum_buf, a, n4, n);
    BDN_CHECK_LAUNCH("sgd_momentum_step");
    return BDN_OK;
}

struct AdamParams { float grad_scale, w1 , beta2, c2 , eps, l2 , decay , step_size , bc2_sqrt; int lerp_hi; };

__device__ __forceinline__ void adam_elem(float& p, float gr, float& m, float& v, const AdamParams& a) {
    float g = a.grad_scale * gr;
    p = p * a.decay;
    if (a.l2 != 0.f) g = g + a.l2 * p;
    m = a.lerp_hi ? g - (g - m) * (1.f - a.w1) : m + a.w1 * (g - m);
    v = a.beta2 * v + a.c2 * g * g;
    const float den = sqrtf(v) / a.bc2_sqrt + a.eps;
    p = p - a.step_size * (m / den);
}

__global__ void __launch_bounds__(256) adam_kernel(float* __restrict__ p, const float* __restrict__ g, float* __restrict__ m,
                                                   float* __restrict__ v, AdamParams a, size_t n4, size_t n) {
    const size_t stride = (size_t)gridDim.x * 256;
    for (size_t base = (size_t)blockIdx.x * 256 + threadIdx.x; base < n4; base += stride * OPT_VEC) {
        float4 P[OPT_VEC], G[OPT_VEC], M[OPT_VEC], V[OPT_VEC];
#pragma unroll
        for (int u = 0; u < OPT_VEC; u++) {
            const size_t i = base + u * stride;
            if (i < n4) {
                P[u] = reinterpret_cast<const float4*>(p)[i]; G[u] = reinterpret_cast<const float4*>(g)[i];
                M[u] = reinterpret_cast<const float4*>(m)[i]; V[u] = reinterpret_cast<const float4*>(v)[i];
            }
        }
#pragma unroll
        for (int u = 0; u < OPT_VEC; u++) {
            const size_t i = base + u * stride;
            if (i < n4) {
                adam_elem(P[u].x, G[u].x, M[u].x, V[u].x, a); adam_elem(P[u].y, G[u].y, M[u].y, V[u].y, a);
                adam_elem(P[u].z, G[u].z, M[u].z, V[u].z, a); adam_elem(P[u].w, G[u].w, M[u].w, V[u].w, a);
                reinterpret_cast<float4*>(p)[i] = P[u]; reinterpret_cast<float4*>(m)[i] = M[u]; reinterpret_cast<float4*>(v)[i] = V[u];
            }
        }
    }
    if (blockIdx.x == 0 && threadIdx.x < n - n4 * 4) {
        const size_t k = n4 * 4 + threadIdx.x;
        float q = p[k], mk = m[k], vk = v[k];
        adam_elem(q, g[k], mk, vk, a);
        p[k] = q; m[k] = mk; v[k] = vk;
    }
}

extern "C" int bdn_adam_step(float* params, const float* grads, float* exp_avg, float* exp_avg_sq, float lr, float grad_scale,
                             double beta1, double beta2, float eps, float weight_decay, int decoupled_weight_decay, long long step,
                             size_t n, void* stream) {
    if (!params || !grads || !exp_avg || !exp_avg_sq) BDN_FAIL(BDN_E_ARG, "adam_step: null pointer");
    if (((uintptr_t)params | (uintptr_t)grads | (uintptr_t)exp_avg | (uintptr_t)exp_avg_sq) & 15)
        BDN_FAIL(BDN_E_ARG, "adam_step: buffers must be 16-byte aligned");
    if (step < 1) BDN_FAIL(BDN_E_ARG, "adam_step: step must be >= 1 (1-based, counted after the increment), got %lld", step);
    if (!(beta1 >= 0.0 && beta1 < 1.0 && beta2 >= 0.0 && beta2 < 1.0))
        BDN_FAIL(BDN_E_ARG, "adam_step: betas must lie in [0, 1)");
    if (n == 0) return BDN_OK;
    const double bc1 = 1.0 - std::pow(beta1, (double)step), bc2 = 1.0 - std::pow(beta2, (double)step);
    const float w1 = (float)(1.0 - beta1);
    const bool dec = decoupled_weight_decay != 0;
    const AdamParams a{grad_scale, w1, (float)beta2, (float)(1.0 - beta2), eps, dec ? 0.f : weight_decay,
                       dec ? (float)(1.0 - (double)lr * (double)weight_decay) : 1.f, (float)((double)lr / bc1), (float)std::sqrt(bc2),
                       w1 >= 0.5f ? 1 : 0};
    const size_t n4 = n / 4;
    hipLaunchKernelGGL(adam_kernel, dim3(opt_grid(n4)), dim3(256), 0, (hipStream_t)stream, params, grads, exp_avg, exp_avg_sq, a, n4, n);
    BDN_CHECK_LAUNCH("adam_step");
    return BDN_OK;
}

constexpr int OPT_MAX_GROUPS = 8;
constexpr int OPT_MAX_SEGS = 256;
constexpr int OPT_FROZEN = -1;

struct SegTable { const uint32_t* end; const int32_t* group; int n_seg, n_groups; };
template <typename P> struct GroupArgs { P g[OPT_MAX_GROUPS]; };

struct RuleSgd {
    using Params = float;
    static constexpr int NS = 0;
    static __device__ __forceinline__ void scale(Params& step, float s) { step *= s; }
    static __device__ __forceinline__ bool reads_state(const Params&) { return false; }
    static __device__ __forceinline__ void elem(float& p, float g, float&, float&, const Params& step) { p -= step * g; }
};
template <bool MOM> struct RuleSgdm {
    using Params = SgdmParams;
    static constexpr int NS = MOM ? 1 : 0;
    static __device__ __forceinline__ void scale(Params& a, float s) { a.grad_scale *= s; }
    static __device__ __forceinline__ bool reads_state(const Params& a) { return MOM && !a.first; }
    static __device__ __forceinline__ void elem(float& p, float g, float& buf, float&, const Params& a) { sgdm_elem<MOM>(p, g, buf, a); }
};
struct RuleAdam {
    using Params = AdamParams;
    static constexpr int NS = 2;
    static __device__ __forceinline__ void scale(Params& a, float s) { a.grad_scale *= s; }
    static __device__ __forceinline__ bool reads_state(const Params&) { return true; }
    static __device__ __forceinline__ void elem(float& p, float g, float& m, float& v, const Params& a) { adam_elem(p, g, m, v, a); }
};

__device__ __forceinline__ void seg_step(const uint32_t* s_end, int h, uint32_t i, int& s) {
    if (s_end[s + h - 1] <= i) s += h;
}

template <typename Rule>
__global__ void __launch_bounds__(256) grouped_kernel(float* __restrict__ p, const float* __restrict__ g, float* __restrict__ s0,
                                                      float* __restrict__ s1, SegTable t, GroupArgs<typename Rule::Params> a,
                                                      const float* __restrict__ dev_scale, size_t n4) {
    __shared__ uint32_t s_end[OPT_MAX_SEGS];
    __shared__ int s_grp[OPT_MAX_SEGS];
    __shared__ typename Rule::Params s_par[OPT_MAX_GROUPS];
    int cap = 1;
    while (cap < t.n_seg) cap <<= 1;
    for (int k = threadIdx.x; k < cap; k += 256) {
        s_end[k] = k < t.n_seg ? t.end[k] : 0xffffffffu;
        s_grp[k] = k < t.n_seg ? t.group[k] : OPT_FROZEN;
    }
    if (threadIdx.x == 0) {
#pragma unroll
        for (int k = 0; k < OPT_MAX_GROUPS; k++) s_par[k] = a.g[k];
        if (dev_scale) {
            const float ds = *dev_scale;
#pragma unroll
            for (int k = 0; k < OPT_MAX_GROUPS; k++) Rule::scale(s_par[k], ds);
        }
    }
    __syncthreads();
    const size_t stride = (size_t)gridDim.x * 256;
    for (size_t b0 = (size_t)blockIdx.x * 256; b0 < n4; b0 += stride * OPT_VEC) {
        int gid[OPT_VEC], seg[OPT_VEC] = {};
        for (int h = cap >> 1; h > 0; h >>= 1) {
#pragma unroll
            for (int u = 0; u < OPT_VEC; u++) {
                const size_t first = b0 + u * stride;
                seg_step(s_end, h, (uint32_t)(first < n4 ? first : n4 - 1), seg[u]);
            }
        }
#pragma unroll
        for (int u = 0; u < OPT_VEC; u++) {
            const size_t first = b0 + u * stride, i = first + threadIdx.x;
            int grp = OPT_FROZEN;
            if (i < n4) {
                const size_t last = first + 255 < n4 ? first + 255 : n4 - 1;
                int s = seg[u];
                if (!(s_end[s] > last)) {
                    s = 0;
                    for (int h = cap >> 1; h > 0; h >>= 1) seg_step(s_end, h, (uint32_t)i, s);
                }
                if (s_end[s] > i) grp = s_grp[s];
            }
            gid[u] = (unsigned)grp < (unsigned)t.n_groups ? grp : OPT_FROZEN;
        }
        float4 P[OPT_VEC], G[OPT_VEC], S0[OPT_VEC] = {}, S1[OPT_VEC] = {};
#pragma unroll
        for (int u = 0; u < OPT_VEC; u++) {
            const size_t i = b0 + u * stride + threadIdx.x;
            if (gid[u] != OPT_FROZEN) {
                P[u] = reinterpret_cast<const float4*>(p)[i]; G[u] = reinterpret_cast<const float4*>(g)[i];
                if (Rule::NS > 0 && Rule::reads_state(s_par[0])) S0[u] = reinterpret_cast<const float4*>(s0)[i];
                if (Rule::NS > 1) S1[u] = reinterpret_cast<const float4*>(s1)[i];
            }
        }
#pragma unroll
        for (int u = 0; u < OPT_VEC; u++) {
            const size_t i = b0 + u * stride + threadIdx.x;
            if (gid[u] != OPT_FROZEN) {
                const typename Rule::Params q = s_par[gid[u]];
                Rule::elem(P[u].x, G[u].x, S0[u].x, S1[u].x, q); Rule::elem(P[u].y, G[u].y, S0[u].y, S1[u].y, q);
                Rule::elem(P[u].z, G[u].z, S0[u].z, S1[u].z, q); Rule::elem(P[u].w, G[u].w, S0[u].w, S1[u].w, q);
                reinterpret_cast<float4*>(p)[i] = P[u];
                if (Rule::NS > 0) reinterpret_cast<float4*>(s0)[i] = S0[u];
                if (Rule::NS > 1) reinterpret_cast<float4*>(s1)[i] = S1[u];
            }
        }
    }
}

static int grouped_check(const char* what, const void* params, const void* grads, const void* s0, const void* s1, const uint32_t* seg_end,
                         const int32_t* seg_group, int n_seg, int n_groups, const float* lr, size_t n) {
    if (!params || !grads || !seg_end || !seg_group || !lr) BDN_FAIL(BDN_E_ARG, "%s: null pointer", what);
    if (n_groups < 1 || n_groups > OPT_MAX_GROUPS)
        BDN_FAIL(BDN_E_ARG, "%s: %d groups (1..%d: their hyperparameters travel in the kernel arguments)", what, n_groups, OPT_MAX_GROUPS);
    if (n_seg < 1 || n_seg > OPT_MAX_SEGS) BDN_FAIL(BDN_E_ARG, "%s: %d segments (1..%d)", what, n_seg, OPT_MAX_SEGS);
    if (((uintptr_t)params | (uintptr_t)grads | (uintptr_t)s0 | (uintptr_t)s1) & 15) BDN_FAIL(BDN_E_ARG, "%s: buffers must be 16-byte aligned", what);
    if (((uintptr_t)seg_end | (uintptr_t)seg_group) & 3) BDN_FAIL(BDN_E_ARG, "%s: segment table must be 4-byte aligned", what);
    if (n % 4 != 0 || n / 4 > 0xffffffffull)
        BDN_FAIL(BDN_E_ARG, "%s: n = %zu must be a multiple of 4 (tensors padded to a float4) below 2^34", what, n);
    return BDN_OK;
}

static int ex_check(const char* what, const float* dev_scale) {
    if (!dev_scale) BDN_FAIL(BDN_E_ARG, "%s: null pointer (dev_scale)", what);
    if ((uintptr_t)dev_scale & 3) BDN_FAIL(BDN_E_ARG, "%s: dev_scale must be 4-byte aligned", what);
    return BDN_OK;
}

static int sgd_grouped_launch(const char* what, float* params, const float* grads, const uint32_t* seg_end, const int32_t* seg_group,
                              int n_seg, int n_groups, const float* lr, float grad_scale, const float* dev_scale, size_t n, void* stream) {
    if (int rc = grouped_check(what, params, grads, nullptr, nullptr, seg_end, seg_group, n_seg, n_groups, lr, n)) return rc;
    if (n == 0) return BDN_OK;
    GroupArgs<float> a{};
    for (int k = 0; k < n_groups; k++) a.g[k] = lr[k] * grad_scale;
    const SegTable t{seg_end, seg_group, n_seg, n_groups};
    hipLaunchKernelGGL(grouped_kernel<RuleSgd>, dim3(opt_grid(n / 4)), dim3(256), 0, (hipStream_t)stream, params, grads, (float*)nullptr,
                       (float*)nullptr, t, a, dev_scale, n / 4);
    BDN_CHECK_LAUNCH(what);
    return BDN_OK;
}

extern "C" int bdn_sgd_step_grouped(float* params, const float* grads, const uint32_t* seg_end, const int32_t* seg_group, int n_seg,
                                    int n_groups, const float* lr, float grad_scale, size_t n, void* stream) {
    return sgd_grouped_launch("sgd_step_grouped", params, grads, seg_end, seg_group, n_seg, n_groups, lr, grad_scale, nullptr, n, stream);
// ... 299 lines not shown
```

fabric_amd/engine.py:

```python
from dataclasses import dataclass, field

import torch

from . import _lib
from ._lib import BDN_BF16, BDN_BF16X2, BDN_BF16X3, BDN_F32, IN_BNRELU, IN_PLAIN, WG_ROLE, call, ptr, wg_flags

ENC_CH = (64, 128, 256, 512, 512)
DEC_OUT = (256, 128, 64, 64)
BN_EPS = 1e-5
BN_MOMENTUM = 0.1


def _round_up(v, m):
    return (v + m - 1) // m * m


@dataclass
class ConvLayer:
    name: str
    conv: str
    bn: str
    cin_real: int
    cin: int
    cout: int
    level: int
    enc: bool


def build_layers(n_channels):
    layers = []
    cp = _round_up(n_channels, 16)
    prev_real, prev = n_channels, cp
    for k in range(1, 6):
        base = 'inc.conv.conv' if k == 1 else f'down{k - 1}.mpconv.1.conv'
        co = ENC_CH[k - 1]
        layers.append(ConvLayer(f'e{k}a', f'{base}.0', f'{base}.1', prev_real, prev, co, k, True))
        layers.append(ConvLayer(f'e{k}b', f'{base}.3', f'{base}.4', co, co, co, k, True))
        prev_real = prev = co
    cprev = ENC_CH[4]
    for j in range(1, 5):
        k = 5 - j
        base = f'up{j}.conv.conv'
        ci = ENC_CH[k - 1] + cprev
        co = DEC_OUT[j - 1]
        layers.append(ConvLayer(f'd{j}a', f'{base}.0', f'{base}.1', ci, ci, co, k, False))
        layers.append(ConvLayer(f'd{j}b', f'{base}.3', f'{base}.4', co, co, co, k, False))
        cprev = co
    return layers


def param_order(n_channels):
    layers = build_layers(n_channels)
    order = ['outc.conv.weight', 'outc.conv.bias']
    for L in reversed(layers):
        order += [f'{L.bn}.weight', f'{L.bn}.bias', f'{L.conv}.weight']
    order += [f'{L.conv}.bias' for L in reversed(layers)]
    return order


class _LazyBufs(dict):

    def __init__(self, shapes, alloc):
        super().__init__()
        self._shapes, self._alloc = shapes, alloc

    def __missing__(self, key):
        t = self[key] = self._alloc(*self._shapes[key])
        return t


class Workspace:

    def __init__(self, eng, B, H, W, device):
        self.B, self.H, self.W = B, H, W
        td = eng.tdtype
        self.dims = []
        h, w = H, W
        for k in range(5):
            self.dims.append((h, w))
            h, w = h // 2, w // 2
        if min(self.dims[4]) < 1:
            raise RuntimeError(f'BiDateNet needs H,W >= 16 (got {H}x{W}): four 2x poolings')
        e = lambda *s: torch.empty(*s, dtype=td, device=device)
        f32 = lambda *s: torch.empty(*s, dtype=torch.float32, device=device)
        self.x0 = e(2 * B, H, W, eng.cp)
        self.z, self.bn = {}, {}
        pool_s, f_s, U_s = {}, {}, {}
        for L in eng.layers:
            hk, wk = self.dims[L.level - 1]
            n = 2 * B if L.enc else B
            self.z[L.name] = e(n, hk, wk, L.cout)
            self.bn[L.name] = f32(2 if L.enc else 1, 4, L.cout)
        for k in range(1, 6):
            hk, wk = self.dims[k - 1]
            if k >= 2:
                pool_s[k] = (2 * B, hk, wk, ENC_CH[k - 2])
            f_s[k] = (B, hk, wk, ENC_CH[k - 1])
        cprev = ENC_CH[4]
        for j in range(1, 5):
            hk, wk = self.dims[4 - j]
            U_s[j] = (B, hk, wk, cprev)
            cprev = DEC_OUT[j - 1]
        self.pool, self.f, self.U = _LazyBufs(pool_s, e), _LazyBufs(f_s, e), _LazyBufs(U_s, e)
        if not eng.x3:
            for d_ in (self.pool, self.f, self.U):
                for key in d_._shapes:
                    d_[key]
        lib = _lib.load()
        n_stats = n_bnb = 1
        for L in eng.layers:
            hk, wk = self.dims[L.level - 1]
            n, ipg = (2 * B, B) if L.enc else (B, B)
            n_stats = max(n_stats, eng.mtiles(n, hk, wk, L.cin, L.cout, ipg) * 2 * L.cout)
            if L.name != 'e1a':
                n_stats = max(n_stats, eng.mtiles(n, hk, wk, L.cout, L.cin, ipg) * 2 * L.cin)
            if L.name == 'd4b':
                n_stats = max(n_stats, lib.bdn_outc_bwd_rows(eng.dt, B, hk, wk, L.cout) * 2 * L.cout)
            if not L.enc and L.name[2] == 'b' and L.level > 1:
                n_stats = max(n_stats, lib.bdn_upsample2x_bwd_rows(eng.dt, B, hk, wk, L.cout) * 2 * L.cout)
            if L.enc:
                n_stats = max(n_stats, 2 * lib.bdn_enc_skip_bwd_rows(eng.dt, B, hk, wk, L.cout) * 2 * L.cout)
            n_bnb = max(n_bnb, lib.bdn_bn_bwd_workspace_bytes(eng.dt, n, hk, wk, L.cout, ipg) // 4)
        self.stats = f32(n_stats)
        self.bnws = torch.empty(2 * 64 * 2 * 1024, dtype=torch.float64, device=device)
        self.n_bnb = n_bnb
        self._bwd = None
        self._split = {}
        self._wg, self._wg_bytes = {}, {}
        self._outc_ws = None
        self.logits = None
        self.x0_split = False
        self.leased = False
        self.generation = 0

    def _grown(self, bufs, key, numel, dtype):
        t = bufs.get(key)
        if t is None or t.numel() < numel:
            if t is not None:
                from . import streams
                t.record_stream(streams.get('wgrad', self.x0.device))
            t = bufs[key] = torch.empty(numel, dtype=dtype, device=self.x0.device)
        return t[:numel]

    def split_buf(self, which, numel):
        return self._grown(self._split, which, numel, torch.bfloat16)

    def wgrad_scratch(self, role, size_fn, *args):
        nb = self._wg_bytes.get((size_fn, args))
        if nb is None:
            nb = self._wg_bytes[size_fn, args] = getattr(_lib.load(), size_fn)(*args)
        return self._grown(self._wg, role, max(nb // 4, 1), torch.float32)

    def release_split(self):
        self._split = {}

    def outc_ws(self, eng):
        if self._outc_ws is None:
            n = _lib.load().bdn_outc_bwd_workspace_bytes(eng.dt, self.B, self.H, self.W, eng.layers[-1].cout, eng.n_classes)
            self._outc_ws = torch.empty(max(n // 4, 1), dtype=torch.float32, device=self.x0.device)
        return self._outc_ws

    def bwd_scratch(self, device):
        if self._bwd is None:
            self._bwd = dict(bnb=torch.empty(self.n_bnb, dtype=torch.float32, device=device),
                             sums=torch.empty(2 * 2 * 1024, dtype=torch.float32, device=device))
        return self._bwd


class BiDateEngine:

    def __init__(self, n_channels, n_classes, precision='bf16'):
        if precision not in ('bf16', 'fp32', 'bf16x3', 'bf16x3-fast'):
            raise ValueError(f"precision must be 'bf16', 'bf16x3', 'bf16x3-fast' or 'fp32', got {precision!r}")
        self.n_channels, self.n_classes = n_channels, n_classes
        self.precision = precision
        self.dt = BDN_BF16 if precision == 'bf16' else BDN_F32
        self.x3 = precision in ('bf16x3', 'bf16x3-fast')
        self.mdt = BDN_BF16X3 if self.x3 else self.dt
        self.tdtype = torch.bfloat16 if precision == 'bf16' else torch.float32
        self.esize = 2 if precision == 'bf16' else 4
        self.cp = _round_up(n_channels, 16)
        self.layers = build_layers(n_channels)
        self._ws = {}
        self._packed = {}
        self._packed_valid = False
        self._pack_desc = None
        self._packed_versions = None
        self._ev = None
        self.eval_fused = True
        self.eval_pair = (1, 2, 3, 4, 5)
        self.fold_bn_bwd = ('e1b', 'd4a')
        self.wgrad_kernel = 0
        self.x3_bwd_terms = 2 if precision == 'bf16x3-fast' else 3
        self.x3_src_f32 = True
        self.first_wgrad_fused = True
        self.x3_tail_wgrad_blocks = 512
        self.wgrad_blocks = 0
        self._handoffs = {}
        self._diag_skip_reduce = 0
        self.prof_pick = None
        self._prof_seen = 0
        self.prof_filter = None
        self.prof = None
        _lib.load()

    def conv_kernel_name(self, n, h, w, c0, c1, cout, ipg):
        return _lib.load().bdn_conv3x3_variant(self.mdt, n, h, w, c0 + c1 if self.x3 else c0, 0 if self.x3 else c1, cout, ipg).decode()

    def _timed(self, name, flops, fn, *args, split=None):
        if self.prof is not None:
            name = name()
            picked = self.prof_filter is None or name in self.prof_filter
            if picked and self.prof_pick is not None:
                self._prof_seen += 1
                picked = self._prof_seen - 1 == self.prof_pick
            if picked:
                timed, rest = split or ((fn, *args), None)
                e0, e1 = torch.cuda.Event(enable_timing=True), torch.cuda.Event(enable_timing=True)
                e0.record()
                call(*timed)
                e1.record()
                if rest:
                    call(*rest)
                self.prof.append((name, flops, e0, e1))
                return
        call(fn, *args)

    def _timed_conv(self, n, h, w, c0, c1, cout, ipg, *args, fn='bdn_conv3x3', bb=False):
        def name():
            if bb:
                return _lib.load().bdn_conv3x3_dgrad_bb_variant(n, h, w, cout, ipg).decode()
            if fn == 'bdn_conv3x3_x3src':
                return _lib.load().bdn_conv3x3_x3src_variant(args[0], n, h, w, c0, cout, ipg).decode()
            return self.conv_kernel_name(n, h, w, c0, c1, cout, ipg)
        self._timed(name, 2.0 * n * h * w * cout * 9 * (c0 + c1), fn, *args)

    def mtiles(self, n, h, w, c0, cout, ipg):
        return _lib.load().bdn_conv3x3_num_mtiles_ex(self.mdt, n, h, w, c0, cout, ipg)

    def _side_stream(self, device):
        from . import streams
        return streams.get('wgrad', device)

    def workspace(self, B, H, W, device, slot=0):
        key = (B, H, W, str(device), slot)
        pool = self._ws.setdefault(key, [])
        for ws in pool:
            if not ws.leased:
                return ws
        pool.append(Workspace(self, B, H, W, device))
        return pool[-1]

    def drop_workspaces(self, slot):
        for key in [k for k in self._ws if k[4] == slot]:
            self._ws[key] = [w for w in self._ws[key] if w.leased]
            if not self._ws[key]:
                del self._ws[key]

    def _weights(self, L, P, need_wd):
        if not self._packed_valid:
            self._pack_all(P)
        ent = self._packed[L.conv]
        return ent[0], ent[1]

    def _pack_all(self, P):
        import struct
        ptrs = tuple(P[f'{L.conv}.weight'].data_ptr() for L in self.layers)
        if self._pack_desc is None or self._pack_desc[0] != ptrs:
            kx, pdt = (3, torch.bfloat16) if self.x3 else (1, self.tdtype)
            dev = P[f'{self.layers[0].conv}.weight'].device
            self._packed, rec = {}, b''
            for L in self.layers:
                wf = torch.empty(L.cout, 9, kx * L.cin, dtype=pdt, device=dev)
                wd = torch.empty(L.cin, 9, kx * L.cout, dtype=pdt, device=dev) if L.name != 'e1a' else None
                self._packed[L.conv] = (wf, wd)
                rec += struct.pack('<QQQiiii', P[f'{L.conv}.weight'].data_ptr(), wf.data_ptr(),
                                   wd.data_ptr() if wd is not None else 0, L.cout, L.cin_real, L.cin, 0)
            self._pack_desc = (ptrs, torch.frombuffer(bytearray(rec), dtype=torch.uint8).to(dev))
        call('bdn_pack_weights_multi', self.mdt, ptr(self._pack_desc[1]), len(self.layers), _lib.stream_ptr())
        self._packed_versions = tuple(P[f'{L.conv}.weight']._version for L in self.layers)
        self._packed_valid = True

    def _check_packed(self, P):
        if self._packed_valid and (self._packed_versions != tuple(P[f'{L.conv}.weight']._version for L in self.layers) or
                                   self._pack_desc[0] != tuple(P[f'{L.conv}.weight'].data_ptr() for L in self.layers)):
            self._packed_valid = False

    def invalidate_weights(self):
        self._packed_valid = False

    def release_split_buffers(self):
        for pool in self._ws.values():
            for ws in pool:
                if not ws.leased:
                    ws.release_split()

    def _conv(self, ws, L, P, in0, c0, in1, c1, in_mode, in_bn, n, ipg, training, st, reuse_eval_bn=False, presplit=False, frozen=False):
        hk, wk = ws.dims[L.level - 1]
        keep = training or frozen
        wf, _ = self._weights(L, P, False)
        z, bn = ws.z[L.name], ws.bn[L.name]
        xs = self.x3_src_f32
        if self.x3 and in1 is None and not presplit and c0 % 64 == 0 and c0 <= 512 and xs and \
                (not isinstance(xs, (tuple, list, set)) or L.name in xs or (not training and c0 <= 128)):
            sp = ws.split_buf(('a', L.name), n * hk * wk * 2 * c0) if keep else None
            self._timed_conv(n, hk, wk, c0, 0, L.cout, ipg,
                             self.mdt, ptr(in0), c0, in_mode, ptr(in_bn), ipg, ptr(wf), ptr(P[f'{L.conv}.bias']), ptr(z),
                             ptr(ws.stats) if training else None, ptr(sp), n, hk, wk, L.cout, st, fn='bdn_conv3x3_x3src')
        else:
            if self.x3:
                sp = ws.split_buf(('a', L.name) if keep else 'a', n * hk * wk * 2 * (c0 + c1))
                if not presplit:
                    call('bdn_split_pack', ptr(in0), c0, ptr(in1), c1, in_mode, ptr(in_bn), ipg, ptr(sp), n, hk, wk, st)
                in0, c0, in1, c1, in_mode, in_bn = sp, c0 + c1, None, 0, IN_PLAIN, None
            self._timed_conv(n, hk, wk, c0, c1, L.cout, ipg,
                             self.mdt, ptr(in0), c0, ptr(in1), c1, in_mode, ptr(in_bn), ipg,
                             ptr(wf), ptr(P[f'{L.conv}.bias']), ptr(z), ptr(ws.stats) if training else None,
                             n, hk, wk, L.cout, st)
        G = n // ipg
        if training:
            nt = self.mtiles(n, hk, wk, c0 + c1, L.cout, ipg)
            call('bdn_bn_finalize', ptr(ws.stats), nt, G, L.cout, ipg * hk * wk,
                 ptr(P[f'{L.bn}.weight']), ptr(P[f'{L.bn}.bias']), BN_EPS, BN_MOMENTUM,
                 ptr(P[f'{L.bn}.running_mean']), ptr(P[f'{L.bn}.running_var']),
                 ptr(P[f'{L.bn}.num_batches_tracked']), ptr(bn), ptr(ws.bnws), st)
        elif not reuse_eval_bn:
            call('bdn_bn_eval', ptr(P[f'{L.bn}.weight']), ptr(P[f'{L.bn}.bias']),
                 ptr(P[f'{L.bn}.running_mean']), ptr(P[f'{L.bn}.running_var']), BN_EPS, G, L.cout, ptr(bn), st)
        return z, bn

    def forward(self, x_d1, x_d2, P, training=True, class_map=False, frozen=False):
        self._prof_seen = 0
        if not (x_d1.is_cuda and x_d2.is_cuda):
            raise RuntimeError('fabric_amd: BiDateNet runs only on a ROCm device (MI355X); '
                               'inputs must be CUDA/HIP tensors -- there is no CPU path')
        if x_d1.shape != x_d2.shape or x_d1.dim() != 4 or x_d1.shape[1] != self.n_channels:
            raise RuntimeError(f'expected two [B,{self.n_channels},H,W] tensors, got {tuple(x_d1.shape)} and {tuple(x_d2.shape)}')
        x_d1 = x_d1.contiguous().float()
        x_d2 = x_d2.contiguous().float()
        B, C, H, W = x_d1.shape
        ws = self.workspace(B, H, W, x_d1.device)
        ws.generation += 1
        ws.x0_split = self.x3 and not class_map
        if ws.x0_split:
            sp = ws.split_buf(('a', self.layers[0].name) if training or frozen else 'a', 2 * B * H * W * 2 * self.cp)
            call('bdn_pack_input', BDN_BF16X3, ptr(x_d1), ptr(x_d2), ptr(sp), B, C, H, W, self.cp, _lib.stream_ptr())
        else:
            call('bdn_pack_input', self.dt, ptr(x_d1), ptr(x_d2), ptr(ws.x0), B, C, H, W, self.cp, _lib.stream_ptr())
        if class_map:
            if training:
                raise RuntimeError('class_map=True is an eval-mode output')
            cd = torch.empty(B, H, W, dtype=torch.uint8, device=x_d1.device)
            if self._use_eval_schedule():
                self._forward_eval(ws, P, mask=cd)
            else:
                logits = self._forward_packed(ws, P, False)
                call('bdn_argmax', ptr(logits), ptr(cd), B, self.n_classes, H, W, _lib.stream_ptr())
            return cd, ws
        return self._forward_packed(ws, P, training, frozen=frozen and not training), ws

    def forward_tiles(self, scene_d1, scene_d2, origins, P, patch_size, reuse_eval_bn=False, slot=0, scene_mask=None):
        if not (scene_d1.is_cuda and scene_d2.is_cuda and origins.is_cuda):
            raise RuntimeError('fabric_amd: scene planes and tile origins must be CUDA/HIP tensors -- there is no CPU path')
        if scene_d1.shape != scene_d2.shape or scene_d1.dim() != 3 or scene_d1.shape[0] != self.n_channels:
            raise RuntimeError(f'expected two [{self.n_channels},H,W] scenes, got {tuple(scene_d1.shape)} and {tuple(scene_d2.shape)}')
        if scene_d1.dtype != torch.float32 or scene_d2.dtype != torch.float32 or origins.dtype != torch.int32:
            raise RuntimeError('scene planes must be float32 and origins int32')
        if not (scene_d1.is_contiguous() and scene_d2.is_contiguous() and origins.is_contiguous()):
            raise RuntimeError('scene planes and origins must be contiguous')
        if origins.dim() != 2 or origins.shape[1] not in (2, 3):
            raise RuntimeError(f'origins must be int32 [n,2] (y0,x0) or a symmetry table [n,3] (y0,x0,sym), got {tuple(origins.shape)}')
        sym = origins.shape[1] == 3
        if sym and scene_mask is not None:
            raise RuntimeError('a symmetry table gives logits in the tiles\' own orientation: no scene_mask')
        C, H, W = scene_d1.shape
        n, p = origins.shape[0], patch_size
        ws = self.workspace(n, p, p, scene_d1.device, slot)
        ws.generation += 1
        ws.x0_split = False
        call('bdn_gather_tiles_sym' if sym else 'bdn_gather_tiles', self.dt, ptr(scene_d1), ptr(scene_d2), ptr(origins), ptr(ws.x0),
             n, C, H, W, p, self.cp, _lib.stream_ptr())
        if scene_mask is not None:
            if scene_mask.dtype != torch.uint8 or tuple(scene_mask.shape) != (H, W) or not scene_mask.is_contiguous() or not scene_mask.is_cuda:
                raise RuntimeError(f'scene_mask must be a contiguous uint8 [{H},{W}] device tensor')
            if self._use_eval_schedule():
                self._forward_eval(ws, P, reuse_tables=reuse_eval_bn, mask=scene_mask, origins=origins, scene_hw=(H, W))
            else:
                logits = self._forward_packed(ws, P, False, reuse_eval_bn)
                call('bdn_argmax_stitch', ptr(logits), ptr(origins), ptr(scene_mask), n, logits.shape[1], p, H, W, _lib.stream_ptr())
            return None, ws
        return self._forward_packed(ws, P, False, reuse_eval_bn), ws

    def _forward_packed(self, ws, P, training, reuse_eval_bn=False, frozen=False):
        B, H, W = ws.B, ws.H, ws.W
        dev = ws.x0.device
        st = _lib.stream_ptr()
        _lib.PHASE = 'fwd'
        if not training and not frozen and self._use_eval_schedule():
            return self._forward_eval(ws, P, reuse_tables=reuse_eval_bn)
        self._check_packed(P)
        by = {L.name: L for L in self.layers}
        rb = reuse_eval_bn and not training
        for k in range(1, 6):
            hk, wk = ws.dims[k - 1]
            La, Lb = by[f'e{k}a'], by[f'e{k}b']
            pre = self.x3 and (training or frozen)
            src = ws.x0 if k == 1 else (None if pre else ws.pool[k])
            za, bna = self._conv(ws, La, P, src, La.cin, None, 0, IN_PLAIN, None, 2 * B, B, training, st, rb,
                                 presplit=(pre and k > 1) or (k == 1 and ws.x0_split), frozen=frozen)
            zb, bnb = self._conv(ws, Lb, P, za, Lb.cin, None, 0, IN_BNRELU, bna, 2 * B, B, training, st, rb, frozen=frozen)
            if k < 5 and pre:
                Ld, Ln = by[f'd{5 - k}a'], by[f'e{k + 1}a']
                hn, wn = ws.dims[k]
                call('bdn_product_pool_split', ptr(zb), ptr(bnb), ptr(ws.split_buf(('a', Ld.name), B * hk * wk * 2 * Ld.cin)), 2 * Ld.cin, Ld.cin,
                     ptr(ws.split_buf(('a', Ln.name), 2 * B * hn * wn * 2 * Ln.cin)), B, hk, wk, ENC_CH[k - 1], st)
            elif k < 5:
                call('bdn_product_pool', self.dt, ptr(zb), ptr(bnb), ptr(ws.f[k]), ptr(ws.pool[k + 1]), B, hk, wk, ENC_CH[k - 1], st)
            else:
                call('bdn_fuse_product', self.dt, ptr(zb), ptr(bnb), ptr(ws.f[k]), B, hk, wk, ENC_CH[k - 1], st)
        prev, prev_bn, prev_mode, cprev = ws.f[5], None, IN_PLAIN, ENC_CH[4]
        for j in range(1, 5):
            k = 5 - j
            hk, wk = ws.dims[k - 1]
            hs, wsrc = ws.dims[k]
            La, Lb = by[f'd{j}a'], by[f'd{j}b']
            pre = self.x3 and (training or frozen)
            if pre:
                call('bdn_upsample2x_split', ptr(prev), prev_mode, ptr(prev_bn), ptr(ws.split_buf(('a', La.name), B * hk * wk * 2 * La.cin)),
                     2 * La.cin, ENC_CH[k - 1], La.cin, B, hs, wsrc, hk, wk, cprev, st)
            else:
                call('bdn_upsample2x', self.dt, ptr(prev), prev_mode, ptr(prev_bn), ptr(ws.U[j]),
                     B, hs, wsrc, hk, wk, cprev, st)
            za, bna = self._conv(ws, La, P, None if pre else ws.f[k], ENC_CH[k - 1], None if pre else ws.U[j], cprev, IN_PLAIN, None, B, B,
                                 training, st, rb, presplit=pre, frozen=frozen)
            zb, bnb = self._conv(ws, Lb, P, za, Lb.cin, None, 0, IN_BNRELU, bna, B, B, training, st, rb, frozen=frozen)
            prev, prev_bn, prev_mode, cprev = zb, bnb, IN_BNRELU, Lb.cout
        logits = torch.empty(B, self.n_classes, H, W, dtype=torch.float32, device=dev)
        call('bdn_outc_fwd', self.dt, ptr(prev), ptr(prev_bn), ptr(P['outc.conv.weight']), ptr(P['outc.conv.bias']),
             ptr(logits), B, H, W, cprev, self.n_classes, st)
        return logits

    def _use_eval_schedule(self):
        return self.eval_fused and not self.x3

    def eval_tables(self, P, refold=True):
        import struct
        keys = [(f'{L.bn}.weight', f'{L.bn}.bias', f'{L.bn}.running_mean', f'{L.bn}.running_var', f'{L.conv}.bias') for L in self.layers]
        ptrs = tuple(P[k].data_ptr() for ks in keys for k in ks)
        if self._ev is None or self._ev[0] != ptrs:
            dev = P[keys[0][0]].device
            tab = torch.empty(sum(2 * L.cout for L in self.layers), dtype=torch.float32, device=dev)
            rec, views, off = b'', {}, 0
            for L, ks in zip(self.layers, keys):
                out = tab[off:off + 2 * L.cout]
                off += 2 * L.cout
                rec += struct.pack('<QQQQQQii', *(P[k].data_ptr() for k in ks), out.data_ptr(), L.cout, 0)
                views[L.name] = (out[:L.cout], out[L.cout:])
            ident = torch.zeros(1, 4, self.layers[-1].cout, dtype=torch.float32, device=dev)
            ident[:, 1:3] = 1.0
            self._ev = (ptrs, torch.frombuffer(bytearray(rec), dtype=torch.uint8).to(dev), views, ident, tab)
            refold = True
        if refold:
            call('bdn_bn_eval_fold_multi', ptr(self._ev[1]), len(self.layers), max(L.cout for L in self.layers), BN_EPS, _lib.stream_ptr())
        return self._ev[2]

    def _forward_eval(self, ws, P, reuse_tables=False, mask=None, origins=None, scene_hw=None):
        B, H, W = ws.B, ws.H, ws.W
        dev = ws.x0.device
        st = _lib.stream_ptr()
        _lib.PHASE = 'fwd'
        by = {L.name: L for L in self.layers}
        self._check_packed(P)
        ev = self.eval_tables(P, refold=not reuse_tables)

        def stage(L, in0, c0, in1, c1, out, n, hk, wk, mul=None, pool=None):
            wf, _ = self._weights(L, P, False)
            sc, sh = ev[L.name]
            call('bdn_conv3x3_eval', self.dt, ptr(in0), c0, ptr(in1), c1, ptr(wf), ptr(sc), ptr(sh), ptr(out), ptr(mul), ptr(pool),
                 n, hk, wk, L.cout, st)

        for k in range(1, 6):
            hk, wk = ws.dims[k - 1]
            La, Lb = by[f'e{k}a'], by[f'e{k}b']
            src = ws.x0 if k == 1 else ws.pool[k]
            za, zb = ws.z[La.name], ws.z[Lb.name]
            stage(La, src, La.cin, None, 0, za, 2 * B, hk, wk)
            pn = ws.pool[k + 1] if k < 5 else None
            if k in self.eval_pair:
                wf, _ = self._weights(Lb, P, False)
                sc, sh = ev[Lb.name]
                call('bdn_conv3x3_eval_pair', self.dt, ptr(za), Lb.cin, ptr(wf), ptr(sc), ptr(sh), ptr(ws.f[k]), ptr(pn), B, hk, wk, Lb.cout, st)
            else:
                stage(Lb, za[:B], Lb.cin, None, 0, zb[:B], B, hk, wk, pool=pn[:B] if k < 5 else None)
                stage(Lb, za[B:], Lb.cin, None, 0, ws.f[k], B, hk, wk, mul=zb[:B], pool=pn[B:] if k < 5 else None)
        prev, cprev = ws.f[5], ENC_CH[4]
        logits = None
        for j in range(1, 5):
            k = 5 - j
            hk, wk = ws.dims[k - 1]
            hs, wsrc = ws.dims[k]
            La, Lb = by[f'd{j}a'], by[f'd{j}b']
            call('bdn_upsample2x', self.dt, ptr(prev), IN_PLAIN, None, ptr(ws.U[j]), B, hs, wsrc, hk, wk, cprev, st)
            stage(La, ws.f[k], ENC_CH[k - 1], ws.U[j], cprev, ws.z[La.name], B, hk, wk)
            if j < 4 or self.n_classes > 2:
                stage(Lb, ws.z[La.name], Lb.cin, None, 0, ws.z[Lb.name], B, hk, wk)
            else:
                wf, _ = self._weights(Lb, P, False)
                sc, sh = ev[Lb.name]
                if mask is None:
                    logits = torch.empty(B, self.n_classes, H, W, dtype=torch.float32, device=dev)
                call('bdn_conv3x3_eval_cls', self.dt, ptr(ws.z[La.name]), Lb.cin, ptr(wf), ptr(sc), ptr(sh), None,
                     ptr(P['outc.conv.weight']), ptr(P['outc.conv.bias']), self.n_classes, ptr(logits), ptr(mask), ptr(origins),
                     scene_hw[0] if scene_hw else 0, scene_hw[1] if scene_hw else 0, B, hk, wk, Lb.cout, st)
            prev, cprev = ws.z[Lb.name], Lb.cout
        if self.n_classes > 2:
            logits = torch.empty(B, self.n_classes, H, W, dtype=torch.float32, device=dev)
            call('bdn_outc_fwd', self.dt, ptr(prev), ptr(self._ev[3]), ptr(P['outc.conv.weight']), ptr(P['outc.conv.bias']),
                 ptr(logits), B, H, W, cprev, self.n_classes, st)
            if mask is not None:
                if origins is not None:
                    call('bdn_argmax_stitch', ptr(logits), ptr(origins), ptr(mask), B, self.n_classes, H, scene_hw[0], scene_hw[1], st)
                else:
                    call('bdn_argmax', ptr(logits), ptr(mask), B, self.n_classes, H, W, st)
                return None
        return logits

    @property
    def bwd_dtype(self):
        return BDN_BF16X2 if (self.x3 and self.x3_bwd_terms == 2) else self.mdt

    def folds_bn_bwd(self, L, h, w):
        return (self.mdt == BDN_BF16 and L.name in self.fold_bn_bwd and L.cout == 64 and min(h, w) > 8
                and L is not self.layers[0] and L is not self.layers[-1])

    def first_wgrad_dtype(self, n, h, w, ipg):
        L = self.layers[0]
        if self.first_wgrad_fused and _lib.load().bdn_conv3x3_wgrad_bnbwd_supported(self.mdt, n, h, w, L.cout, L.cin, ipg):
            return self.bwd_dtype
        return None

    def chain_end(self, need, dx=None):
        if need is None or dx is not None:
            return None
        last = 'outc'
        for L in reversed(self.layers):
            if any(k in need for k in (f'{L.conv}.weight', f'{L.conv}.bias', f'{L.bn}.weight', f'{L.bn}.bias')):
                last = L.name
        return None if last == self.layers[0].name else last

    def wgrad_launch(self, L, c0, c1, mode):
        phases = 1 if self._diag_skip_reduce else 3
        if self.x3:
            tail = L.name == 'e1b' and self.x3_tail_wgrad_blocks and self.x3_bwd_terms == 3
            return self.bwd_dtype, c0 + c1, 0, IN_PLAIN, wg_flags(phases, 0, self.x3_tail_wgrad_blocks if tail else self.wgrad_blocks)
        return self.dt, c0, c1, mode, wg_flags(phases, self.wgrad_kernel, self.wgrad_blocks)

    @staticmethod
    def wgrad_gemm_name(dtype, n, h, w, cout, c0, c1, ipg, mode, flags):
        lib = _lib.load()
        if dtype in (BDN_BF16X3, BDN_BF16X2):
            terms = 3 if dtype == BDN_BF16X3 else 2
            if cout % 64 == 0 and c0 % 64 == 0 and lib.bdn_conv3x3_wgrad_variant(BDN_BF16, n, h, w, cout, c0, 0, ipg, IN_PLAIN, flags) == WG_ROLE:
                return f'wgrad7x_kernel<{terms}>'
            xfl = (1 << 30) | ((1 << 29) if terms == 2 else 0)
            return BiDateEngine.wgrad_gemm_name(BDN_BF16, n, h, w, 2 * cout, 2 * c0, 0, ipg, IN_PLAIN, flags | xfl) + '+wgrad_x3_combine_kernel'
        if lib.bdn_conv3x3_wgrad_variant(dtype, n, h, w, cout, c0, c1, ipg, mode, flags) == WG_ROLE:
            return f'wgrad7_kernel<{"true" if mode == IN_BNRELU else "false"}>'
        small = h <= 8 and w <= 8 and ipg % 2 == 0
        return (f'wgrad_kernel<{"bf16" if dtype == BDN_BF16 else "f32"},8,{"8,2" if small else "16,1"},'
                f'{"true" if c0 + c1 <= 32 else "false"}>')

    def backward(self, ws, dlogits, P, grads, on_ready=None, zero_bias_grads=True, wgrad_stream=True, dx=None, bn_mode='batch',
                 need=None):
        if bn_mode not in ('batch', 'running'):
            raise ValueError(f"bn_mode must be 'batch' or 'running', got {bn_mode!r}")
        frozen = bn_mode == 'running'
        B, H, W = ws.B, ws.H, ws.W
        dev = dlogits.device
        dlogits = dlogits.contiguous().float()
        st = _lib.stream_ptr()
        _lib.PHASE = 'bwd'
        by = {L.name: L for L in self.layers}
        sc = ws.bwd_scratch(dev)
        e = lambda *s: torch.empty(*s, dtype=self.tdtype, device=dev)
        ready = on_ready or (lambda keys: None)
        main = torch.cuda.current_stream(dev)
        side = self._side_stream(dev) if wgrad_stream else None
        keep = []
        n_hand = [0]
        end = self.chain_end(need, dx)
        released = set()

        def handoff(src, dst):
            pool = self._handoffs.setdefault(dev.index, [])
            if n_hand[0] == len(pool):
                from .streams import HandOff
                with torch.cuda.device(dev):
                    pool.append(HandOff())
            ho = pool[n_hand[0]]
            n_hand[0] += 1
            ho.signal(src)
            ho.wait(dst)

        def bn_bwd_finalize(L, n, ipg, rows):
            if frozen:
                call('bdn_bn_bwd_finalize_frozen', ptr(ws.bn[L.name]), n // ipg, L.cout, ptr(ws.stats), rows, 1, ptr(sc['sums']),
                     ptr(grads[f'{L.bn}.weight']), ptr(grads[f'{L.bn}.bias']), ptr(grads[f'{L.conv}.bias']), ptr(ws.bnws), st)
                return
            call('bdn_bn_bwd_finalize', ptr(ws.bn[L.name]), n // ipg, L.cout, ptr(ws.stats), rows, 1, ptr(sc['sums']),
                 ptr(grads[f'{L.bn}.weight']), ptr(grads[f'{L.bn}.bias']), ptr(ws.bnws), st)

        def bn_bwd(L, dA, ldA, n, ipg, fused_rows, plain=False):
            hk, wk = ws.dims[L.level - 1]
            if frozen:
                gb = (ptr(grads[f'{L.bn}.weight']), ptr(grads[f'{L.bn}.bias']), ptr(grads[f'{L.conv}.bias']))
                if fused_rows and self.x3 and not plain:
                    sp = ws.split_buf(('d', L.name), n * hk * wk * 2 * L.cout)
                    call('bdn_bn_bwd_apply_frozen', BDN_BF16X3, dA, ldA, ptr(ws.z[L.name]), ptr(ws.bn[L.name]), ipg, n, hk, wk, L.cout,
                         ptr(ws.stats), fused_rows, 1, ptr(sc['sums']), *gb, ptr(sp), ptr(ws.bnws), st)
                    return None
                dz = e(n, hk, wk, L.cout)
                if fused_rows:
                    call('bdn_bn_bwd_apply_frozen', self.dt, dA, ldA, ptr(ws.z[L.name]), ptr(ws.bn[L.name]), ipg, n, hk, wk, L.cout,
                         ptr(ws.stats), fused_rows, 1, ptr(sc['sums']), *gb, ptr(dz), ptr(ws.bnws), st)
                else:
                    call('bdn_bn_bwd_frozen', self.dt, dA, ldA, ptr(ws.z[L.name]), ptr(ws.bn[L.name]), ipg, n, hk, wk, L.cout,
                         ptr(sc['bnb']), ptr(sc['sums']), *gb, ptr(dz), st)
                return dz
            if fused_rows and self.x3 and not plain:
                sp = ws.split_buf(('d', L.name), n * hk * wk * 2 * L.cout)
                call('bdn_bn_bwd_apply_split', dA, ldA, ptr(ws.z[L.name]), ptr(ws.bn[L.name]), ipg, n, hk, wk, L.cout,
                     ptr(ws.stats), fused_rows, 1, ptr(sc['sums']), ptr(grads[f'{L.bn}.weight']),
                     ptr(grads[f'{L.bn}.bias']), ptr(sp), ptr(ws.bnws), st)
                return None
            dz = e(n, hk, wk, L.cout)
            if fused_rows:
                call('bdn_bn_bwd_apply', self.dt, dA, ldA, ptr(ws.z[L.name]), ptr(ws.bn[L.name]), ipg, n, hk, wk, L.cout,
                     ptr(ws.stats), fused_rows, 1, ptr(sc['sums']), ptr(grads[f'{L.bn}.weight']),
                     ptr(grads[f'{L.bn}.bias']), ptr(dz), ptr(ws.bnws), st)
            else:
                call('bdn_bn_bwd', self.dt, dA, ldA, ptr(ws.z[L.name]), ptr(ws.bn[L.name]), ipg, n, hk, wk, L.cout,
                     ptr(sc['bnb']), ptr(sc['sums']), ptr(grads[f'{L.bn}.weight']), ptr(grads[f'{L.bn}.bias']), ptr(dz), st)
            return dz

        def head_bwd(L, rows):
            hk, wk = ws.dims[L.level - 1]
            dz = None if self.x3 else e(B, hk, wk, L.cout)
            out = ws.split_buf(('d', L.name), B * hk * wk * 2 * L.cout) if self.x3 else dz
            bn_bwd_finalize(L, B, B, rows)
            call('bdn_outc_bn_bwd_apply', self.mdt, ptr(dlogits), ptr(P['outc.conv.weight']), ptr(ws.z[L.name]),
                 ptr(ws.bn[L.name]), B, ptr(sc['sums']), ptr(out), B, hk, wk, L.cout, self.n_classes, st)
            return dz

        def fold_dgrad(L, dA, n, ipg, rows, prev):
            hk, wk = ws.dims[L.level - 1]
            bn_bwd_finalize(L, n, ipg, rows)
            _, wd = self._weights(L, P, True)
            dz, out = e(n, hk, wk, L.cout), e(n, hk, wk, L.cin)
            has = prev is not None
            self._timed_conv(n, hk, wk, L.cout, 0, L.cin, ipg,
                             self.mdt, dA, L.cout, ptr(ws.z[L.name]), ptr(ws.bn[L.name]), ptr(sc['sums']), ipg, ptr(wd), ptr(out),
                             ptr(ws.z[prev.name]) if has else None, ptr(ws.bn[prev.name]) if has else None, ptr(ws.stats) if has else None,
                             ptr(dz), n, hk, wk, L.cin, st, fn='bdn_conv3x3_dgrad_bb', bb=True)
            return dz, out, self.mtiles(n, hk, wk, L.cout, L.cin, ipg) // (n // ipg) if has else 0

        def dgrad(L, dz, n, ipg, prev):
            hk, wk = ws.dims[L.level - 1]
            _, wd = self._weights(L, P, True)
            out = e(n, hk, wk, L.cin)
            if self.x3:
                dz = ws.split_buf(('d', L.name), n * hk * wk * 2 * L.cout)
            if prev is None:
                self._timed_conv(n, hk, wk, L.cout, 0, L.cin, ipg,
                                 self.bwd_dtype, ptr(dz), L.cout, None, 0, IN_PLAIN, None, ipg,
                                 ptr(wd), None, ptr(out), None, n, hk, wk, L.cin, st)
                return out, 0
            self._timed_conv(n, hk, wk, L.cout, 0, L.cin, ipg,
                             self.bwd_dtype, ptr(dz), L.cout, ptr(wd), ptr(out), ptr(ws.z[prev.name]), ptr(ws.bn[prev.name]),
                             ipg, ptr(ws.stats), n, hk, wk, L.cin, st, fn='bdn_conv3x3_dgrad_bs')
            return out, self.mtiles(n, hk, wk, L.cout, L.cin, ipg) // (n // ipg)

        def split_dz(L, dz, n, ipg):
            hk, wk = ws.dims[L.level - 1]
            sp = ws.split_buf(('d', L.name), n * hk * wk * 2 * L.cout)
            call('bdn_split_pack', ptr(dz), L.cout, None, 0, IN_PLAIN, None, ipg, ptr(sp), n, hk, wk, st)

        def wgrad_call(L, dz, in0, c0, in1, c1, mode, in_bn, n, ipg, stp, role):
            hk, wk = ws.dims[L.level - 1]
            if self.x3:
                dz = ws.split_buf(('d', L.name), n * hk * wk * 2 * L.cout)
                in0, in1, in_bn = ws.split_buf(('a', L.name), n * hk * wk * 2 * (c0 + c1)), None, None
            dt, c0, c1, mode, flg = self.wgrad_launch(L, c0, c1, mode)
            part = ws.wgrad_scratch(role, 'bdn_wgrad_workspace_bytes_ex', dt, n, hk, wk, L.cout, c0, c1, ipg, mode, flg)
            args = (dt, ptr(dz), L.cout, ptr(in0), c0, ptr(in1), c1, mode, ptr(in_bn), ipg,
                    ptr(part), ptr(grads[f'{L.conv}.weight']), L.cin_real, n, hk, wk)
            if self.x3:
                call('bdn_conv3x3_wgrad_ex', *args, flg, stp)
                return
            ph = flg & ~3
            self._timed(lambda: self.wgrad_gemm_name(dt, n, hk, wk, L.cout, c0, c1, ipg, mode, ph | 3),
                        2.0 * n * hk * wk * L.cout * 9 * (c0 + c1), 'bdn_conv3x3_wgrad_ex', *args, flg, stp,
                        split=(('bdn_conv3x3_wgrad_ex', *args, ph | 1, stp), ('bdn_conv3x3_wgrad_ex', *args, ph | 2, stp)))

        def release(L, launch, last):
            keys = [f'{L.bn}.weight', f'{L.bn}.bias', f'{L.conv}.weight', f'{L.conv}.bias']
            released.add(L.name)
            if need is not None and f'{L.conv}.weight' not in need:
                launch = lambda stp, role: None
            zero_bias = zero_bias_grads and not frozen
            if side is not None and not last:
                handoff(main, side)
                with torch.cuda.stream(side):
                    launch(side.cuda_stream, 'wgrad')
                    if zero_bias:
                        grads[f'{L.conv}.bias'].zero_()
                    ready(keys)
                return
            launch(st, 'chain' if side is not None else 'wgrad')
            if zero_bias:
                grads[f'{L.conv}.bias'].zero_()
            if side is not None:
                handoff(side, main)
            ready(keys)

        def layer(L, n, dA, ldA, rows, operand, prev=None):
            hk, wk = ws.dims[L.level - 1]
            first = L is self.layers[0]
            fdt = self.first_wgrad_dtype(n, hk, wk, B) if first else None
            if fdt is not None:
                bn_bwd_finalize(L, n, B, rows)
                fin = ws.split_buf(('a', L.name), n * hk * wk * 2 * L.cin) if self.x3 else ws.x0
                if dx is not None:
                    call('bdn_conv3x3_dgrad_first', self.dt, dA, L.cout, ptr(ws.z[L.name]), ptr(ws.bn[L.name]), ptr(sc['sums']), B,
                         ptr(P[f'{L.conv}.weight']), L.cin_real, ptr(dx[0]), ptr(dx[1]), B, hk, wk, st)

                def launch(stp, role):
                    part = ws.wgrad_scratch('chain', 'bdn_wgrad_workspace_bytes', n, hk, wk, L.cout, L.cin, B)
                    self._timed(lambda: 'wgrad_first_kernel', 2.0 * n * hk * wk * L.cout * 9 * L.cin, 'bdn_conv3x3_wgrad_bnbwd',
                                fdt, dA, L.cout, ptr(ws.z[L.name]), ptr(ws.bn[L.name]), ptr(sc['sums']), B, L.cout,
                                ptr(fin), L.cin, ptr(part), ptr(grads[f'{L.conv}.weight']), L.cin_real, n, hk, wk, stp)
                release(L, launch, last=True)
                return None, 0
            out, rows_out = None, 0
            if dA is None:
                dz = head_bwd(L, rows)
            elif rows and self.folds_bn_bwd(L, hk, wk):
                dz, out, rows_out = fold_dgrad(L, dA, n, B, rows, prev)
            else:
                dz = bn_bwd(L, dA, ldA, n, B, rows, plain=first and dx is not None)
            if first and dx is not None:
                call('bdn_conv3x3_dgrad_first', self.dt, ptr(dz), L.cout, None, None, None, B,
                     ptr(P[f'{L.conv}.weight']), L.cin_real, ptr(dx[0]), ptr(dx[1]), B, hk, wk, st)
            if self.x3 and dz is not None:
                split_dz(L, dz, n, B)
            release(L, lambda stp, role: wgrad_call(L, dz, *operand, n, B, stp, role), last=first)
            if out is None and not first and L.name != end:
                out, rows_out = dgrad(L, dz, n, B, prev)
            keep.extend((dz, out))
            return out, rows_out

        def chain():
            L4b = by['d4b']
            call('bdn_outc_bwd', self.dt, ptr(dlogits), ptr(ws.z['d4b']), ptr(ws.bn['d4b']), ptr(P['outc.conv.weight']),
                 None, ptr(grads['outc.conv.weight']), ptr(grads['outc.conv.bias']), ptr(ws.stats),
                 ptr(ws.outc_ws(self)), B, H, W, L4b.cout, self.n_classes, st)
            ready(['outc.conv.weight', 'outc.conv.bias'])
            if end == 'outc':
                return
            dA, ldA, rows = None, 0, _lib.load().bdn_outc_bwd_rows(self.dt, B, H, W, L4b.cout)
            dcat = {}
            for j in range(4, 0, -1):
                k = 5 - j
                hk, wk = ws.dims[k - 1]
                hs, wsrc = ws.dims[k]
                La, Lb = by[f'd{j}a'], by[f'd{j}b']
                ck = ENC_CH[k - 1]
                cprev = La.cin - ck
                dAa, rows = layer(Lb, B, dA, ldA, rows, (ws.z[La.name], Lb.cin, None, 0, IN_BNRELU, ws.bn[La.name]), prev=La)
                if end == Lb.name:
                    return
                dc, _ = layer(La, B, ptr(dAa), La.cout, rows, (None if self.x3 else ws.f[k], ck, None if self.x3 else ws.U[j], cprev, IN_PLAIN, None))
                if end == La.name:
                    return
                dcat[k] = dc
                dprev = e(B, hs, wsrc, cprev)
                keep.append(dprev)
                rows = _lib.load().bdn_upsample2x_bwd_rows(self.dt, B, hs, wsrc, cprev) if j > 1 else 0
                if rows:
                    Lp = by[f'd{j - 1}b']
                    call('bdn_upsample2x_bwd_bs', self.dt, dc.data_ptr() + ck * self.esize, La.cin, ptr(dprev), ptr(ws.z[Lp.name]),
                         ptr(ws.bn[Lp.name]), ptr(ws.stats), B, hs, wsrc, hk, wk, cprev, st)
                else:
                    call('bdn_upsample2x_bwd', self.dt, dc.data_ptr() + ck * self.esize, La.cin, ptr(dprev), B, hs, wsrc, hk, wk, cprev, st)
                dA, ldA = ptr(dprev), cprev
            dF, dP = dprev, None
            for k in range(5, 0, -1):
                hk, wk = ws.dims[k - 1]
                La, Lb = by[f'e{k}a'], by[f'e{k}b']
                ck = ENC_CH[k - 1]
                if k < 5:
                    dF = dcat[k]
                dAb = e(2 * B, hk, wk, ck)
                keep.append(dAb)
                call('bdn_enc_skip_bwd', self.dt, ptr(dF), dF.shape[3], ptr(ws.z[Lb.name]), ptr(ws.bn[Lb.name]),
                     ptr(dP), ptr(dAb), ptr(ws.stats), B, hk, wk, ck, st)
                dAa, rows = layer(Lb, 2 * B, ptr(dAb), ck, _lib.load().bdn_enc_skip_bwd_rows(self.dt, B, hk, wk, ck),
                                  (ws.z[La.name], Lb.cin, None, 0, IN_BNRELU, ws.bn[La.name]), prev=La)
                if end == Lb.name:
                    return
                src = ws.x0 if k == 1 else (None if self.x3 else ws.pool[k])
                dP, _ = layer(La, 2 * B, ptr(dAa), La.cout, rows, (src, La.cin, None, 0, IN_PLAIN, None))
                if end == La.name:
                    return
        chain()
        if side is not None:
            handoff(side, main)
        if end is not None:
            ready([k for L in self.layers if L.name not in released
                   for k in (f'{L.bn}.weight', f'{L.bn}.bias', f'{L.conv}.weight', f'{L.conv}.bias')])
        return grads
```

fabric_amd/train_step.py:

```python
import torch
import torch.distributed as dist

from . import _lib
from . import optim as _optim
from .engine import param_order
from .parallel import FlatLayout, GradBucketer


class TrainStep:
    def __init__(self, model, lr=1e-3, tversky_alpha=0.1, tversky_beta=0.9, eps=1e-7,
                 process_group=None, n_buckets=4, distributed=True, force_collectives=False, guard=True,
                 optimizer='sgd', momentum=0.0, dampening=0.0, nesterov=False, weight_decay=None, betas=(0.9, 0.999), adam_eps=1e-8,
                 param_groups=None, bn='batch', criterion=None, accumulate=1, max_grad_norm=None):
        if bn not in ('batch', 'frozen'):
            raise ValueError(f"bn must be 'batch' or 'frozen', got {bn!r}")
        self.accumulate = _optim.check_accumulate(accumulate)
        self.max_grad_norm = _optim.check_max_grad_norm(max_grad_norm)
        self.micro = 0
        self.flat_accum = self._norm = self._clip_table = None
        self.last_grad_norm = self.last_clip_coef = None
        self.model, self.lr, self.bn = model, lr, bn
        self.optim = _optim.OptimConfig(optimizer, lr=lr, momentum=momentum, dampening=dampening, nesterov=nesterov,
                                        weight_decay=weight_decay, betas=betas, eps=adam_eps)
        self._guard = guard
        self.collectives_report = None
        self.alpha, self.beta, self.eps = tversky_alpha, tversky_beta, eps
        if isinstance(criterion, str):
            from .criterion import Criterion
            criterion = Criterion.parse(criterion, tversky_alpha=tversky_alpha, tversky_beta=tversky_beta, eps=eps)
        self.criterion = criterion
        self.group = process_group
        self.high_priority_chain = True
        self._hp = None
        self.world = (dist.get_world_size(process_group)
                      if distributed and dist.is_available() and dist.is_initialized() else 1)
        named = list(model.named_parameters())
        dev = named[0][1].device
        if dev.type != 'cuda':
            raise RuntimeError('fabric_amd: TrainStep needs the model on a ROCm device (model.cuda() first)')
        self._names = [k for k, _ in named]
        self._by_id = {id(p): k for k, p in named}
        self._checked_groups(param_groups)
        order = param_order(model.n_channels)
        self.layout = FlatLayout([(k, p.shape) for k, p in named], order)
        self.flat_params = torch.zeros(self.layout.total, dtype=torch.float32, device=dev)
        self.flat_grads = torch.zeros(self.layout.total, dtype=torch.float32, device=dev)
        for k, p in named:
            v = self.layout.view(self.flat_params, k)
            v.copy_(p.data)
            p.data = v
            p.grad = self.layout.view(self.flat_grads, k)
        self.grads = {k: self.layout.view(self.flat_grads, k) for k, _ in named}
        self.opt_state = {key: torch.zeros_like(self.flat_params) for key in self.optim.state_keys()}
        self.opt_step = 0
        bias_tail = [k for k in order if k.endswith('.bias') and k.split('.')[-2] in ('0', '3')]
        if bn == 'frozen':
            bias_tail = []
        self.bucketer = GradBucketer(self.layout, self.flat_grads, n_buckets, process_group, keys_no_reduce=bias_tail,
                                     enabled=self.world > 1 or force_collectives, force=force_collectives)
        if self.world > 1:
            dist.broadcast(self.flat_params, src=0, group=process_group)
        self._tv = None
        self.last_counts = self.last_terms = self.last_dlogits = None
        self._P = {k: v.detach() for k, v in self.model.state_dict(keep_vars=True).items()}
        self.param_groups = self._groups = self._seg = self._need = None
        self._implicit_group = False
        if param_groups is not None or any(not p.requires_grad for _, p in named):
            self.set_param_groups(param_groups)
        if self.accumulate > 1:
            self.flat_accum = torch.empty_like(self.flat_grads)
            self.bucketer.before_reduce = self._add_pending
        self._adding = False
        if self.max_grad_norm is not None:
            ws = torch.empty(_lib.load().bdn_grad_norm_workspace_bytes(self.layout.total) // 8, dtype=torch.float64, device=dev)
            out = torch.zeros(2, dtype=torch.float32, device=dev)
            self._norm = (ws, out)
            self.last_grad_norm, self.last_clip_coef = out[0], out[1]
            if self._groups is None:
                self._implicit_table()

    def _implicit_table(self):
        if self._clip_table is None:
            dev = self.flat_params.device
            pg = _optim.ParamGroups(self.optim, self._names, None, ())
            ends, ids = _optim.segment_table(self.layout, pg)
            self._clip_table = (pg, (torch.tensor(ends, dtype=torch.int64).to(torch.int32).to(dev),
                                     torch.tensor(ids, dtype=torch.int32).to(dev), len(ends)))
        return self._clip_table

    def _no_pending(self, what):
        if self.micro != 0:
            raise RuntimeError(f'{what}: {self.micro} of {self.accumulate} micro-steps are pending; call flush() (or flush(apply=False)) first')

    def set_param_groups(self, groups):
        self._no_pending('set_param_groups()')
        dev = self.flat_params.device
        pg = self._checked_groups(groups)
        hp, cur = self.stream(dev), torch.cuda.current_stream(dev)
        cur.wait_stream(hp)
        if pg is None:
            self.param_groups = self._groups = self._seg = self._need = None
            self._implicit_group = False
            return
        ends, ids = _optim.segment_table(self.layout, pg)
        seg = (torch.tensor(ends, dtype=torch.int64).to(torch.int32).to(dev), torch.tensor(ids, dtype=torch.int32).to(dev), len(ends))
        frozen = pg.frozen
        for k in frozen:
            self.grads[k].zero_()
            for t in self.opt_state.values():
                self.layout.view(t, k).zero_()
        hp.wait_stream(cur)
        self._groups, self._seg = pg, seg
        self.param_groups = pg.groups
        self._implicit_group = groups is None
        self._need = set(pg.trainable()) if frozen else None

    def _checked_groups(self, groups):
        frozen = {k for k, p in self.model.named_parameters() if not p.requires_grad}
        if groups is None:
            return _optim.ParamGroups(self.optim, self._names, None, frozen) if frozen else None

        def name_of(q):
            k = q if isinstance(q, str) else self._by_id.get(id(q))
            if k is None:
                raise ValueError('param group lists a tensor that is not a parameter of the model')
            return k
        return _optim.ParamGroups(self.optim, self._names, [dict(g, params=[name_of(q) for q in g['params']]) for g in groups], frozen)

    def _state(self):
        return self._P

    def step(self, x_d1, x_d2, labels):
        if self._guard and self.collectives_report is None and self.bucketer.active():
            self.guard_collectives(*[int(v) for v in (x_d1.shape[0], x_d1.shape[2], x_d1.shape[3])], replace_streams=False)
        if not self.high_priority_chain:
            return self._step(x_d1, x_d2, labels)
        cur = torch.cuda.current_stream(x_d1.device)
        hp = self.stream(x_d1.device)
        if cur.cuda_stream == hp.cuda_stream:
            return self._step(x_d1, x_d2, labels)
        self._hp.wait_stream(cur)
        with torch.cuda.stream(self._hp):
            loss = self._step(x_d1, x_d2, labels)
        cur.wait_stream(self._hp)
        for t in (loss, self.last_logits, self.last_counts, self.last_terms, self.last_dlogits, self.last_grad_norm):
            if t is not None:
                t.record_stream(cur)
        return loss

    def flush(self, apply=True):
        m = self.micro
        if m == 0:
            return False
        if not apply:
            self.micro = 0
            return False
        dev = self.flat_params.device

        def run():
            st = _lib.stream_ptr()
            _lib.call('bdn_grad_accumulate', self.flat_grads.data_ptr(), self.flat_accum.data_ptr(), self.layout.total, 0, st)
            self.micro = 0
            self.bucketer.finish()
            self._apply(st, 1.0 / (self.world * m))
            self.model.engine().invalidate_weights()
        cur, hp = torch.cuda.current_stream(dev), self.stream(dev)
        if not self.high_priority_chain or cur.cuda_stream == hp.cuda_stream:
            run()
            return True
        hp.wait_stream(cur)
        with torch.cuda.stream(hp):
            run()
        cur.wait_stream(hp)
        if self.last_grad_norm is not None:
            self.last_grad_norm.record_stream(cur)
        return True

    def stream(self, device=None):
        from . import streams
        self._hp = streams.get('chain', device if device is not None else self.flat_params.device)
        return self._hp

    def _time_steps(self, x1, x2, lbl, n, warm):
        import time
        dev = x1.device
        with torch.cuda.stream(self.stream(dev)):
            for _ in range(warm):
                self._step(x1, x2, lbl)
            torch.cuda.synchronize(dev)
            t0 = time.perf_counter()
            for _ in range(n):
                self._step(x1, x2, lbl)
            torch.cuda.synchronize(dev)
            return (time.perf_counter() - t0) / n

    def _time_exchange(self, n):
        import time
        dev = self.flat_params.device
        b = self.bucketer
        with torch.cuda.stream(self.stream(dev)):
            for it in range(n + 2):
                if it == 2:
                    torch.cuda.synchronize(dev)
                    t0 = time.perf_counter()
                works = [dist.all_reduce(b.flat[a:e], op=dist.ReduceOp.SUM, group=self.group, async_op=True) for a, e, _ in b.buckets]
                for w in works:
                    w.wait()
            torch.cuda.synchronize(dev)
            t = torch.tensor([(time.perf_counter() - t0) / n], dtype=torch.float64, device=dev)
        if self.world > 1:
            dist.all_reduce(t, op=dist.ReduceOp.MAX, group=self.group)
        return float(t[0])

    def guard_collectives(self, B, H, W, steps=8, threshold=0.05, verbose=False, replace_streams=True):
        import warnings
        from . import streams
        dev = self.flat_params.device
        if not self.bucketer.active():
            self.collectives_report = {'active': False}
            return self.collectives_report
        backend = str(dist.get_backend(self.group))
        if 'nccl' not in backend:
            self.collectives_report = {'active': True, 'guarded': False, 'reason': f'backend {backend}: no device-side collective stream'}
            return self.collectives_report
        self.collectives_report = {'running': True}
        ok = False
        eng = self.model.engine()
        saved = saved_flat = saved_opt = saved_acc = None
        tried = []
        from . import streams as _streams
        orig_streams = (_streams.get('chain', dev), _streams.get('wgrad', dev))
        try:
            g = torch.Generator(device='cpu').manual_seed(99)
            C = self.model.n_channels
            x1 = torch.randn(B, C, H, W, generator=g).to(dev)
            x2 = (x1 + 0.3 * torch.randn(B, C, H, W, generator=g).to(dev))
            lbl = (torch.rand(B, H, W, generator=g) < 0.1).to(torch.uint8).to(dev)
            saved = {k: v.clone() for k, v in self._P.items()}
            saved_flat = self.flat_params.clone()
            saved_opt = ({k: v.clone() for k, v in self.opt_state.items()}, self.opt_step)
            saved_acc = (self.accumulate, self.micro, None if self.flat_accum is None else self.flat_accum.clone(),
                         None if self._norm is None else self._norm[1].clone())
            self.accumulate, self.micro = 1, 0

            def timed(collectives, defer=False):
                self.bucketer.enabled, self.bucketer.defer = collectives, defer
                self.stream(dev).wait_stream(torch.cuda.current_stream(dev))
                t = torch.tensor([self._time_steps(x1, x2, lbl, steps, 3)], dtype=torch.float64, device=dev)
                if self.world > 1:
                    dist.all_reduce(t, op=dist.ReduceOp.MAX, group=self.group)
                return float(t[0])

            def measure(name):
                t_local = timed(False)
                t_ov = timed(True)
                rec = {'arrangement': name, 'local_ms': t_local * 1e3, 'overlap_ms': t_ov * 1e3, 'overhead_frac': t_ov / t_local - 1.0,
                       'streams': (streams.get('chain', dev), streams.get('wgrad', dev))}
                tried.append(rec)
                if verbose:
                    print(f'guard_collectives: {name}: overlap overhead {rec["overhead_frac"] * 100:+.1f} %', flush=True)
                return rec

            first = measure('original')
            kept, placement, t_ex = first, None, None
            if first['overhead_frac'] > threshold:
                t_ex = self._time_exchange(steps)
                first['exchange_alone_ms'] = t_ex * 1e3
                explained = first['local_ms'] * 1.02 + 1.1 * t_ex * 1e3
                placement = first['overlap_ms'] > explained
                if placement and replace_streams:
                    for remedy in ('new_wgrad_stream', 'new_chain_stream'):
                        if kept['overhead_frac'] <= threshold:
                            break
                        streams.replace('wgrad' if remedy == 'new_wgrad_stream' else 'chain', dev)
                        rec = measure(remedy)
                        if rec['overhead_frac'] < kept['overhead_frac']:
                            kept = rec
                streams.restore('chain', kept['streams'][0], dev)
                streams.restore('wgrad', kept['streams'][1], dev)
                if placement and kept['overlap_ms'] > explained:
                    t_def = timed(True, defer=True)
                    kept['deferred_ms'] = t_def * 1e3
                    if t_def * 1e3 < kept['overlap_ms']:
                        kept = dict(kept, arrangement=kept['arrangement'] + ' + deferred_buckets', deferred=True,
                                    overhead_frac=t_def * 1e3 / kept['local_ms'] - 1.0)
            self.bucketer.defer = bool(kept.get('deferred'))
            rep = {'active': True, 'threshold': threshold, 'steps': steps, 'world': self.world,
                   'tried': [{k: v for k, v in r.items() if k != 'streams'} for r in tried],
                   'kept': kept['arrangement'], 'overhead_frac': kept['overhead_frac'], 'deferred_buckets': bool(kept.get('deferred')),
                   'placement_problem': placement, 'stream_remedies_allowed': bool(replace_streams),
                   'recovered': bool(placement) and kept is not first}
            still_bad = bool(placement) and kept['overhead_frac'] > threshold and \
                (kept['deferred_ms'] if kept.get('deferred') else kept['overlap_ms']) > kept['local_ms'] * 1.02 + 1.1 * t_ex * 1e3
            rep['ok'] = not still_bad
            rep['exchange_alone_ms'] = None if t_ex is None else t_ex * 1e3
            if still_bad:
                hint = ('' if replace_streams else '  The stream remedies were skipped because the guard ran inside step(): call '
                        'step.guard_collectives(B, H, W) before adopting step.stream().')
                warnings.warn(f'fabric_amd: launching the gradient all-reduces from backward costs the step {first["overhead_frac"] * 100:+.0f} % '
                              f'here, more than the exchange alone ({t_ex * 1e3:.2f} ms) explains -- a stream-placement problem; kept: {kept["arrangement"]} '
                              f'({kept["overhead_frac"] * 100:+.0f} %, threshold {threshold * 100:.0f} %).{hint}  Creating the process group BEFORE the '
                              f'first TrainStep, the default collective-stream priority and the default GPU_MAX_HW_QUEUES avoid it.', RuntimeWarning)
            ok = True
        finally:
            self.bucketer.enabled = True
            if not ok:
                self.bucketer.defer = False
                _streams.restore('chain', orig_streams[0], dev)
                _streams.restore('wgrad', orig_streams[1], dev)
            self.bucketer.reset()
            torch.cuda.synchronize(dev)
            if saved is not None and saved_flat is not None:
                for k, v in saved.items():
                    self._P[k].copy_(v)
                self.flat_params.copy_(saved_flat)
            if saved_opt is not None:
                for k, v in saved_opt[0].items():
                    self.opt_state[k].copy_(v)
                self.opt_step = saved_opt[1]
            if saved_acc is not None:
                self.accumulate, self.micro = saved_acc[0], saved_acc[1]
                if saved_acc[2] is not None:
                    self.flat_accum.copy_(saved_acc[2])
                if saved_acc[3] is not None:
                    self._norm[1].copy_(saved_acc[3])
            eng.invalidate_weights()
            torch.cuda.synchronize(dev)
            if not ok:
                self.collectives_report = None
        self.collectives_report = rep
        return rep

    def _step(self, x_d1, x_d2, labels):
        model = self.model
        eng = model.engine()
        P = self._state()
        frozen_bn = self.bn == 'frozen'
        if frozen_bn:
            from .models.bidate_model import _Lease
            logits, ws = eng.forward(x_d1, x_d2, P, training=False, frozen=True)
            lease = _Lease(ws)
        else:
            logits, ws = eng.forward(x_d1, x_d2, P, training=True)
        st = _lib.stream_ptr()
        if self.criterion is not None:
            loss, counts, dlogits = self._criterion_loss(logits, labels)
        else:
            loss, counts, dlogits = self._tversky_loss(logits, labels, st)
        pending = self.micro
        closing = pending + 1 >= self.accumulate
        on_ready = self.bucketer.on_ready if closing else None
        self._adding = pending > 0
        try:
            if frozen_bn:
                try:
                    eng.backward(ws, dlogits, P, self.grads, on_ready=on_ready, zero_bias_grads=False, bn_mode='running', need=self._need)
                finally:
                    lease.release()
                    if eng.x3:
                        ws.release_split()
            else:
                eng.backward(ws, dlogits, P, self.grads, on_ready=on_ready, zero_bias_grads=False, need=self._need)
            self.last_counts = counts
            self.last_logits = logits
            if not closing:
                _lib.call('bdn_grad_accumulate', self.flat_accum.data_ptr(), self.flat_grads.data_ptr(), self.layout.total, int(pending > 0), st)
                self.micro = pending + 1
                return loss.clone()
            if pending:
                if self.bucketer.active():
                    self._add_pending(self.bucketer.reduce_end, self.layout.total)
                else:
                    self._add_pending(0, self.layout.total)
            self.bucketer.finish()
        finally:
            self._adding = False
        self.micro = 0
        self._apply(st, 1.0 / (self.world * (pending + 1)))
        eng.invalidate_weights()
        return loss.clone()

    def _add_pending(self, a, b):
        if self._adding and b > a:
            _lib.call('bdn_grad_accumulate', self.flat_grads.data_ptr() + 4 * a, self.flat_accum.data_ptr() + 4 * a, b - a, 1,
                      _lib.stream_ptr())

    def _apply(self, st, grad_scale):
        if self._norm is None:
            return self._update(st, grad_scale)
        ws, out = self._norm
        pg, (ends, ids, n_seg) = (self._groups, self._seg) if self._groups is not None else self._implicit_table()
        _lib.call('bdn_grad_norm', self.flat_grads.data_ptr(), ends.data_ptr(), ids.data_ptr(), n_seg, grad_scale, self.max_grad_norm,
                  ws.data_ptr(), out.data_ptr(), self.layout.total, st)
        self._update_grouped(st, grad_scale, out.data_ptr() + 4)

    def _tversky_loss(self, logits, labels, st):
        B, C, H, W = logits.shape
        dev = logits.device
        if self._tv is None or self._tv[3] != (B, C, H, W):
            n = _lib.load().bdn_overlap_workspace_bytes(B, C, H, W, 0) // 4
            self._tv = (torch.empty(n, dtype=torch.float32, device=dev), torch.empty((), dtype=torch.float32, device=dev),
                        torch.empty(4, dtype=torch.int32, device=dev), (B, C, H, W))
        tvws, loss, counts, _ = self._tv
        if labels.dtype != torch.uint8:
            labels = labels.to(torch.uint8)
        labels = labels.contiguous()
        dlogits = torch.empty_like(logits)
        _lib.call('bdn_tversky', logits.data_ptr(), labels.data_ptr(), float(self.alpha), float(self.beta),
                  float(self.eps), tvws.data_ptr(), loss.data_ptr(), counts.data_ptr(), dlogits.data_ptr(), B, C, H, W, st)
        return loss, counts, dlogits

    def _criterion_loss(self, logits, labels):
        shape = tuple(logits.shape)
        if self._tv is None or self._tv[1] != shape:
            self._tv = (self.criterion.buffers(shape, logits.device), shape)
        loss, terms, counts, dlogits = self.criterion.evaluate(logits, labels, out=self._tv[0])
        self.last_terms, self.last_dlogits = terms, dlogits
        return loss, counts, dlogits

    def _update(self, st, grad_scale):
        o, n = self.optim, self.layout.total
        if self._groups is not None:
            return self._update_grouped(st, grad_scale)
        if o.plain:
            _lib.call('bdn_sgd_step', self.flat_params.data_ptr(), self.flat_grads.data_ptr(), float(self.lr), grad_scale, n, st)
            return
        first = self.opt_step == 0
        self.opt_step += 1
        if o.kind == 'sgd':
            buf = self.opt_state.get('momentum_buffer')
            _lib.call('bdn_sgd_momentum_step', self.flat_params.data_ptr(), self.flat_grads.data_ptr(), _lib.ptr(buf), float(self.lr),
                      grad_scale, o.momentum, o.dampening, o.weight_decay, int(o.nesterov), int(first), n, st)
        else:
            _lib.call('bdn_adam_step', self.flat_params.data_ptr(), self.flat_grads.data_ptr(), self.opt_state['exp_avg'].data_ptr(),
                      self.opt_state['exp_avg_sq'].data_ptr(), float(self.lr), grad_scale, o.betas[0], o.betas[1], o.eps,
                      o.weight_decay, int(o.kind == 'adamw'), self.opt_step, n, st)

    def _update_grouped(self, st, grad_scale, dev_scale=None):
        o, n = self.optim, self.layout.total
        if self._groups is not None:
            pg, seg = self._groups, self._seg
            if self._implicit_group:
                pg.groups[0]['lr'] = float(self.lr)
        else:
            pg, seg = self._implicit_table()
            pg.groups[0]['lr'], pg.groups[0]['weight_decay'] = float(self.lr), o.weight_decay
        lrs, wds = pg.hyper('lr'), pg.hyper('weight_decay')
        ends, ids, n_seg = seg
        table = (ends.data_ptr(), ids.data_ptr(), n_seg, len(lrs))
        lr, wd = _lib.floats(lrs), _lib.floats(wds)
        ex, ds = ('', ()) if dev_scale is None else ('_ex', (dev_scale,))
        if o.kind == 'sgd' and o.momentum == 0 and not any(wds):
            _lib.call('bdn_sgd_step_grouped' + ex, self.flat_params.data_ptr(), self.flat_grads.data_ptr(), *table, lr, grad_scale, *ds, n, st)
            return
        first = self.opt_step == 0
        self.opt_step += 1
        if o.kind == 'sgd':
            _lib.call('bdn_sgd_momentum_step_grouped' + ex, self.flat_params.data_ptr(), self.flat_grads.data_ptr(),
                      _lib.ptr(self.opt_state.get('momentum_buffer')), *table, lr, wd, grad_scale, *ds, o.momentum, o.dampening,
                      int(o.nesterov), int(first), n, st)
        else:
            _lib.call('bdn_adam_step_grouped' + ex, self.flat_params.data_ptr(), self.flat_grads.data_ptr(), self.opt_state['exp_avg'].data_ptr(),
                      self.opt_state['exp_avg_sq'].data_ptr(), *table, lr, wd, grad_scale, *ds, o.betas[0], o.betas[1], o.eps,
                      int(o.kind == 'adamw'), self.opt_step, n, st)

    def optimizer_state_dict(self):
        self._no_pending('optimizer_state_dict()')
        self.optim.lr = float(self.lr)
        self.stream(self.flat_params.device)
        torch.cuda.current_stream(self.flat_params.device).wait_stream(self._hp)
        if self._groups is not None:
            if self._implicit_group:
                self._groups.groups[0]['lr'] = float(self.lr)
            return _optim.groups_to_torch(self.optim, self._groups, self.layout, self.opt_state, self.opt_step)
        return _optim.flat_to_torch(self.optim, self.layout, self._names, self.opt_state, self.opt_step)

    def load_optimizer_state_dict(self, sd):
        self._no_pending('load_optimizer_state_dict()')
        dev = self.flat_params.device
        if self._groups is not None:
            cfg, hyper, flat, step = _optim.torch_to_groups(sd, self._groups, self.layout, dev)
        else:
            cfg, flat, step = _optim.torch_to_flat(sd, self.layout, self._names, dev)
        if cfg.family != self.optim.family:
            raise ValueError(f'optimizer state of {cfg.kind}, but this step runs {self.optim.kind}')
        hp = self.stream(dev)
        hp.wait_stream(torch.cuda.current_stream(dev))
        for t in self.opt_state.values():
            t.record_stream(hp)
        if self._groups is not None:
            if hyper is None:
                cfg.lr, cfg.weight_decay = float(self.lr), self.optim.weight_decay
            else:
                for g, h in zip(self._groups.groups, hyper):
                    g.update(h)
                cfg.lr, cfg.weight_decay = hyper[0]['lr'], hyper[0]['weight_decay']
        self.optim, self.lr, self.opt_state, self.opt_step = cfg, cfg.lr, flat, step
```

include/bidate_hip.h:

```cpp
#ifndef BIDATE_HIP_H
#define BIDATE_HIP_H

#include <stddef.h>
#include <stdint.h>

#ifdef __cplusplus
extern "C" {
#endif

enum { BDN_F32 = 0, BDN_BF16 = 1, BDN_BF16X3 = 2,
       BDN_BF16X2 = 3 };
enum { BDN_OK = 0, BDN_E_ARG = -1, BDN_E_SHAPE = -2, BDN_E_HIP = -3 };
enum { BDN_IN_PLAIN = 0, BDN_IN_BNRELU = 1 };

const char* bdn_last_error(void);
int bdn_version(void);

int bdn_stream_create(int priority, void** stream_out);
int bdn_stream_destroy(void* stream);
int bdn_event_create(void** event_out);
int bdn_event_destroy(void* event);
int bdn_event_record(void* event, void* stream);
int bdn_stream_wait_event(void* stream, void* event);

int bdn_pack_input(int dtype, const float* x_d1, const float* x_d2, void* out,
                   int B, int C, int H, int W, int Cpad, void* stream);
int bdn_pack_weights(int dtype, const float* w_oihw, void* wf, void* wd,
                     int Cout, int Cin, int Cin_pad, void* stream);

int bdn_pack_weights_multi(int dtype, const void* desc, int n_layers, void* stream);

int bdn_conv3x3(int dtype, const void* in0, int C0, const void* in1, int C1,
                int in_mode, const float* in_bn, int imgs_per_group,
                const void* w, const float* bias, void* out, float* stats_partial,
                int N, int H, int W, int Cout, void* stream);
int bdn_conv3x3_num_mtiles(int N, int H, int W, int Cout, int imgs_per_group);
int bdn_conv3x3_num_mtiles_ex(int dtype, int N, int H, int W, int C0, int Cout, int imgs_per_group);
const char* bdn_conv3x3_variant(int dtype, int N, int H, int W, int C0, int C1, int Cout, int imgs_per_group);

int bdn_conv3x3_x3src(int dtype, const float* in, int C0, int in_mode, const float* in_bn, int imgs_per_group,
                      const void* w, const float* bias, float* out, float* stats_partial, void* split_out,
                      int N, int H, int W, int Cout, void* stream);
const char* bdn_conv3x3_x3src_variant(int dtype, int N, int H, int W, int C0, int Cout, int imgs_per_group);

int bdn_conv3x3_dgrad_bs(int dtype, const void* dz, int C0, const void* w_dgrad, void* dA,
                         const void* z_prev, const float* bn_prev, int imgs_per_group, float* bs_partial,
                         int N, int H, int W, int Cout, void* stream);

int bdn_conv3x3_dgrad_bb(int dtype, const void* dA, int C0, const void* z, const float* bn, const float* sums, int imgs_per_group,
                         const void* w_dgrad, void* dA_prev, const void* z_prev, const float* bn_prev, float* bs_partial,
                         void* dz_out, int N, int H, int W, int Cout, void* stream);

const char* bdn_conv3x3_dgrad_bb_variant(int N, int H, int W, int Cout, int imgs_per_group);

int bdn_conv3d_num_mtiles(int N, int D, int H, int W);
int bdn_conv3d(int dtype, const void* in, int C, int in_mode, const float* in_bn, int imgs_per_group,
               const void* w, const float* bias, void* out, float* stats_partial,
               int N, int D, int H, int W, int Cout, void* stream);
int bdn_conv3d_wgrad(int dtype, const void* dz, int Cout, const void* in, int C,
                     float* partial, float* dw_oidhw, int Cin_real, int N, int D, int H, int W, void* stream);

int bdn_split_pack(const float* src0, int C0, const float* src1, int C1, int in_mode, const float* in_bn,
                   int imgs_per_group, void* out, int N, int H, int W, void* stream);

size_t bdn_wgrad_workspace_bytes(int N, int H, int W, int Cout, int Cin, int imgs_per_group);
int bdn_conv3x3_wgrad(int dtype, const void* dz, int Cout,
                      const void* in0, int C0, const void* in1, int C1,
                      int in_mode, const float* in_bn, int imgs_per_group,
                      float* partial, float* dw_oihw, int Cin_real,
                      int N, int H, int W, void* stream);
#define BDN_WG_SIMPLE 1
#define BDN_WG_ROLE   5
#define BDN_WG_FLAGS(phases, kernel, blocks) ((phases) | ((kernel) << 8) | ((blocks) << 16))
size_t bdn_wgrad_workspace_bytes_ex(int dtype, int N, int H, int W, int Cout, int C0, int C1, int imgs_per_group,
                                    int in_mode, int flags);
int bdn_conv3x3_wgrad_ex(int dtype, const void* dz, int Cout,
                         const void* in0, int C0, const void* in1, int C1,
                         int in_mode, const float* in_bn, int imgs_per_group,
                         float* partial, float* dw_oihw, int Cin_real,
                         int N, int H, int W, int flags, void* stream);
int bdn_conv3x3_wgrad_variant(int dtype, int N, int H, int W, int Cout, int C0, int C1, int imgs_per_group,
                              int in_mode, int flags);
int bdn_conv3x3_wgrad_bnbwd_supported(int dtype, int N, int H, int W, int Cout, int C0, int imgs_per_group);
int bdn_conv3x3_wgrad_bnbwd(int dtype, const void* dA, int ldA, const void* z, const float* bn, const float* sums,
                            int imgs_per_group, int Cout, const void* in0, int C0,
                            float* partial, float* dw_oihw, int Cin_real, int N, int H, int W, void* stream);
int bdn_conv3x3_dgrad_first(int dtype, const void* dA, int ldA, const void* z, const float* bn, const float* sums,
                            int imgs_per_group, const float* w_oihw, int Cin_real,
                            float* dx1, float* dx2, int B, int H, int W, void* stream);

size_t bdn_bn_finalize_workspace_bytes(int n_mtiles, int G, int C);
int bdn_bn_finalize(const float* stats_partial, int n_mtiles, int G, int C, int count_per_group,
                    const float* gamma, const float* beta, float eps, float momentum,
                    float* running_mean, float* running_var, int64_t* num_batches_tracked,
                    float* bn, void* ws, void* stream);
int bdn_bn_eval(const float* gamma, const float* beta, const float* running_mean,
                const float* running_var, float eps, int G, int C, float* bn, void* stream);

int bdn_bn_eval_fold_multi(const void* desc, int n_layers, int max_C, float eps, void* stream);
int bdn_conv3x3_eval(int dtype, const void* in0, int C0, const void* in1, int C1, const void* w,
                     const float* ep_scale, const float* ep_shift, void* out, const void* mul, void* pool,
                     int N, int H, int W, int Cout, void* stream);
int bdn_conv3x3_eval_pair(int dtype, const void* in, int C0, const void* w, const float* ep_scale, const float* ep_shift,
                          void* f_out, void* pool, int B, int H, int W, int Cout, void* stream);
int bdn_conv3x3_eval_cls(int dtype, const void* in0, int C0, const void* w, const float* ep_scale, const float* ep_shift, void* act_out,
                         const float* cls_w, const float* cls_b, int ncls, float* logits, uint8_t* mask, const int32_t* origins,
                         int Hs, int Ws, int N, int H, int W, int Cout, void* stream);
enum { BDN_EVAL_STAGE = 0, BDN_EVAL_PAIR = 1, BDN_EVAL_CLS = 2 };
const char* bdn_conv3x3_eval_variant(int kind, int dtype, int N, int H, int W, int C0, int C1, int Cout);

size_t bdn_bn_bwd_workspace_bytes(int dtype, int N, int H, int W, int C, int imgs_per_group);
int bdn_bn_bwd(int dtype, const void* dA, int ldA, const void* z, const float* bn,
               int imgs_per_group, int N, int H, int W, int C,
               float* ws, float* sums, float* dgamma, float* dbeta, void* dz, void* stream);

size_t bdn_bn_bwd_scratch_bytes(int G, int C);
int bdn_bn_bwd_apply(int dtype, const void* dA, int ldA, const void* z, const float* bn,
                     int imgs_per_group, int N, int H, int W, int C,
                     const float* partial, int rows_per_group, int raw_moment,
                     float* sums, float* dgamma, float* dbeta, void* dz, void* scratch, void* stream);
int bdn_bn_bwd_apply_split(const void* dA, int ldA, const void* z, const float* bn,
                           int imgs_per_group, int N, int H, int W, int C,
                           const float* partial, int rows_per_group, int raw_moment,
                           float* sums, float* dgamma, float* dbeta, void* dz_split, void* scratch, void* stream);
int bdn_bn_bwd_finalize(const float* bn, int G, int C, const float* partial, int rows_per_group, int raw_moment,
                        float* sums, float* dgamma, float* dbeta, void* scratch, void* stream);
int bdn_bn_bwd_finalize_frozen(const float* bn, int G, int C, const float* partial, int rows_per_group, int raw_moment,
                               float* sums, float* dgamma, float* dbeta, float* dbias, void* scratch, void* stream);
int bdn_bn_bwd_apply_frozen(int dtype, const void* dA, int ldA, const void* z, const float* bn,
                            int imgs_per_group, int N, int H, int W, int C,
                            const float* partial, int rows_per_group, int raw_moment,
                            float* sums, float* dgamma, float* dbeta, float* dbias, void* dz, void* scratch, void* stream);
int bdn_bn_bwd_frozen(int dtype, const void* dA, int ldA, const void* z, const float* bn,
                      int imgs_per_group, int N, int H, int W, int C,
                      float* ws, float* sums, float* dgamma, float* dbeta, float* dbias, void* dz, void* stream);

int bdn_bnrelu(int dtype, const void* z, const float* bn, int imgs_per_group, void* out,
               int N, int H, int W, int C, void* stream);
int bdn_bnrelu_pool(int dtype, const void* z, const float* bn, int imgs_per_group,
                    void* out, int N, int H, int W, int C, void* stream);

int bdn_fuse_product(int dtype, const void* z, const float* bn, void* f,
                     int B, int H, int W, int C, void* stream);
int bdn_product_pool(int dtype, const void* z, const float* bn, void* f, void* pool,
                     int B, int H, int W, int C, void* stream);

int bdn_product_pool_split(const void* z, const float* bn, void* f_split, int f_ld, int f_half, void* pool_split,
                           int B, int H, int W, int C, void* stream);

int bdn_upsample2x(int dtype, const void* src, int in_mode, const float* bn,
                   void* out, int B, int h, int w, int H, int W, int C, void* stream);
int bdn_upsample2x_split(const void* src, int in_mode, const float* bn, void* out_split, int ld, int off, int half,
                         int B, int h, int w, int H, int W, int C, void* stream);
int bdn_upsample2x_bwd(int dtype, const void* dU, int ldU, void* dsrc,
                       int B, int h, int w, int H, int W, int C, void* stream);
int bdn_upsample2x_bwd_rows(int dtype, int B, int h, int w, int C);
int bdn_upsample2x_bwd_bs(int dtype, const void* dU, int ldU, void* dsrc, const void* z_prev, const float* bn_prev,
                          float* bs_partial, int B, int h, int w, int H, int W, int C, void* stream);

int bdn_enc_skip_bwd(int dtype, const void* dF, int ldF, const void* z, const float* bn,
                     const void* dP, void* dA, float* bs_partial, int B, int H, int W, int C, void* stream);
int bdn_enc_skip_bwd_rows(int dtype, int B, int H, int W, int C);

int bdn_outc_fwd(int dtype, const void* z, const float* bn, const float* w, const float* b,
                 float* logits, int B, int H, int W, int C, int ncls, void* stream);
size_t bdn_outc_bwd_workspace_bytes(int dtype, int B, int H, int W, int C, int ncls);
int bdn_outc_bwd(int dtype, const float* dlogits, const void* z, const float* bn, const float* w,
                 void* dA, float* dw, float* db, float* bs_partial, float* ws, int B, int H, int W, int C, int ncls, void* stream);
int bdn_outc_bn_bwd_apply(int dtype, const float* dlogits, const float* w, const void* z, const float* bn,
                          int imgs_per_group, const float* sums, void* dz, int B, int H, int W, int C, int ncls, void* stream);
int bdn_outc_bwd_rows(int dtype, int B, int H, int W, int C);

size_t bdn_overlap_workspace_bytes(int B, int ncls, int H, int W, int reduce_w);
int bdn_tversky(const float* logits, const uint8_t* labels, float alpha, float beta, float eps,
                float* ws, float* loss, int32_t* counts, float* dlogits,
                int B, int ncls, int H, int W, void* stream);

int bdn_overlap_loss(const float* logits, const uint8_t* labels, float alpha, float beta, float eps,
                     int reduce_w, float* ws, float* loss, int32_t* counts, float* dlogits,
                     int B, int ncls, int H, int W, void* stream);

size_t bdn_focal_workspace_bytes(void);
int bdn_focal(const float* logits, const uint8_t* labels, float gamma, const float* alpha, int size_average,
              void* ws, float* loss, int32_t* counts, float* dlogits,
              int B, int ncls, int H, int W, void* stream);

size_t bdn_criterion_workspace_bytes(int B, int ncls, int H, int W, int reduce_w);
int bdn_criterion(const float* logits, const uint8_t* labels, float w_overlap, float alpha, float beta, float eps, int reduce_w,
                  float w_focal, float gamma, const float* class_alpha, int size_average, void* ws, float* loss, float* terms,
                  int32_t* counts, float* dlogits, int B, int ncls, int H, int W, void* stream);

int bdn_ingest_band(int src_is_f32, const void* src, int hs, int ws, float mean, float stdv,
                    float* dst, int H, int W, void* stream);

int bdn_gather_tiles(int dtype, const float* scene_d1, const float* scene_d2, const int32_t* origins,
                     void* out, int n_tiles, int C, int H, int W, int p, int Cpad, void* stream);
int bdn_upload_band(float* dst_planes, const float* src_planes_host, int C, int H, int W, int r0, int r1, void* stream);
int bdn_argmax(const float* logits, uint8_t* out, int n, int ncls, int H, int W, void* stream);
int bdn_argmax_stitch(const float* logits, const int32_t* origins, uint8_t* mask,
                      int n_tiles, int ncls, int p, int H, int W, void* stream);

int bdn_gather_tiles_sym(int dtype, const float* scene_d1, const float* scene_d2, const int32_t* table,
                         void* out, int n_tiles, int C, int H, int W, int p, int Cpad, void* stream);
int bdn_blend_fold(const float* logits, const int32_t* table, const float* window, float* out, int n_img, int ncls, int p, void* stream);
int bdn_blend_stitch(const float* fold, const float* window, float* acc, float* wsum, long long img0, int n_img,
                     int n_syms, int ncls, int H, int W, int p, int stride, void* stream);
int bdn_blend_finalize(float* acc, const float* wsum, uint8_t* mask, int ncls, int H, int W, void* stream);

int bdn_sample_patches(const void* cities_dev, const int32_t* city_hw_host, int n_cities, int C,
                       const int32_t* desc_host, const int32_t* desc_dev, int n, int S,
                       float* out_d1, float* out_d2, uint8_t* out_labels, void* stream);

int bdn_sgd_step(float* params, const float* grads, float lr, float grad_scale, size_t n, void* stream);
int bdn_sgd_momentum_step(float* params, const float* grads, float* momentum_buf, float lr, float grad_scale, float momentum,
                          float dampening, float weight_decay, int nesterov, int first_step, size_t n, void* stream);
int bdn_adam_step(float* params, const float* grads, float* exp_avg, float* exp_avg_sq, float lr, float grad_scale,
                  double beta1, double beta2, float eps, float weight_decay, int decoupled_weight_decay, long long step,
                  size_t n, void* stream);
int bdn_sgd_step_grouped(float* params, const float* grads, const uint32_t* seg_end, const int32_t* seg_group, int n_seg, int n_groups,
                         const float* lr, float grad_scale, size_t n, void* stream);
int bdn_sgd_momentum_step_grouped(float* params, const float* grads, float* momentum_buf, const uint32_t* seg_end,
                                  const int32_t* seg_group, int n_seg, int n_groups, const float* lr, const float* weight_decay,
                                  float grad_scale, float momentum, float dampening, int nesterov, int first_step, size_t n, void* stream);
int bdn_adam_step_grouped(float* params, const float* grads, float* exp_avg, float* exp_avg_sq, const uint32_t* seg_end,
                          const int32_t* seg_group, int n_seg, int n_groups, const float* lr, const float* weight_decay, float grad_scale,
                          double beta1, double beta2, float eps, int decoupled_weight_decay, long long step, size_t n, void* stream);

int bdn_sgd_step_grouped_ex(float* params, const float* grads, const uint32_t* seg_end, const int32_t* seg_group, int n_seg, int n_groups,
                            const float* lr, float grad_scale, const float* dev_scale, size_t n, void* stream);
int bdn_sgd_momentum_step_grouped_ex(float* params, const float* grads, float* momentum_buf, const uint32_t* seg_end,
                                     const int32_t* seg_group, int n_seg, int n_groups, const float* lr, const float* weight_decay,
                                     float grad_scale, const float* dev_scale, float momentum, float dampening, int nesterov,
                                     int first_step, size_t n, void* stream);
int bdn_adam_step_grouped_ex(float* params, const float* grads, float* exp_avg, float* exp_avg_sq, const uint32_t* seg_end,
                             const int32_t* seg_group, int n_seg, int n_groups, const float* lr, const float* weight_decay,
                             float grad_scale, const float* dev_scale, double beta1, double beta2, float eps,
                             int decoupled_weight_decay, long long step, size_t n, void* stream);

int bdn_grad_accumulate(float* dst, const float* src, size_t n, int add, void* stream);

size_t bdn_grad_norm_workspace_bytes(size_t n);
int bdn_grad_norm(const float* grads, const uint32_t* seg_end, const int32_t* seg_group, int n_seg, float grad_scale, float max_norm,
                  void* workspace, float* out, size_t n, void* stream);

#ifdef __cplusplus
}
#endif
#endif
```

Before: 10590.

## Fuse Tversky loss gradient into outc backward and tail reductions into BN apply

The Tversky loss is split into a stats-only kernel, and the per-pixel softmax gradient is recomputed inside the outc backward kernel instead of being materialised by a separate loss pass. The outc weight/bias reduction and the final loss/count write move into the tail blocks of the fused BN backward apply kernel, so several small launches and a round trip of dlogits through memory go away. It only applies to C=64, ncls=2, fp32 logits, bf16/f32 and non-x3 paths, and it adds a HeadGrad plumbing path between the loss and the engine backward.

```diff
diff --git a/fabric_amd/_lib.py b/fabric_amd/_lib.py
--- a/fabric_amd/_lib.py
+++ b/fabric_amd/_lib.py
@@ -72,6 +72,11 @@
     'bdn_outc_bwd_rows': (_i, [_i, _i, _i, _i, _i]),
     'bdn_overlap_workspace_bytes': (_sz, [_i, _i, _i, _i, _i]),
     'bdn_tversky': (_i, [_vp, _vp, _f, _f, _f, _vp, _vp, _vp, _vp, _i, _i, _i, _i, _vp]),
+    'bdn_head_fused_supported': (_i, [_i, _i, _i, _i, _i, _i, _i]),
+    'bdn_head_fused_workspace_bytes': (_sz, [_i, _i, _i, _i]),
+    'bdn_tversky_stats': (_i, [_vp, _vp, _f, _f, _f, _vp, _i, _i, _i, _i, _vp]),
+    'bdn_outc_bwd_tversky': (_i, [_i, _vp, _vp, _vp, _f, _f, _vp, _vp, _vp, _vp, _vp, _vp, _i, _i, _i, _i, _i, _vp]),
+    'bdn_outc_bn_bwd_apply_tail': (_i, [_i, _vp, _vp, _vp, _vp, _i, _vp, _vp, _vp, _vp, _vp, _vp, _vp, _vp, _i, _i, _i, _i, _i, _vp]),
     'bdn_conv3x3_variant': (C.c_char_p, [_i, _i, _i, _i, _i, _i, _i, _i]),
     'bdn_conv3x3_dgrad_bb_variant': (C.c_char_p, [_i, _i, _i, _i, _i]),
     'bdn_conv3x3_eval_variant': (C.c_char_p, [_i, _i, _i, _i, _i, _i, _i, _i]),
diff --git a/fabric_amd/csrc/head.hip b/fabric_amd/csrc/head.hip
--- a/fabric_amd/csrc/head.hip
+++ b/fabric_amd/csrc/head.hip
@@ -436,69 +436,73 @@
     return BDN_OK;
 }
 
+#define OUTC_APPLY_BODY(BLK_) \
+    constexpr int EPU = ET<T>::EPU;                                                                                     \
+    const int CU = C / EPU, rows = 256 / CU, tid = threadIdx.x, cu = tid % CU, row = tid / CU, c = cu * EPU;            \
+    const int p_begin = (BLK_) * pix_per_block, p_end = min(npix, p_begin + pix_per_block);                             \
+    if (p_begin >= p_end) return;                                                                                       \
+    const float invM = 1.f / (float)pix_per_group;                                                                      \
+    int gcur = -1;                                                                                                      \
+    float mean[EPU], inv[EPU], sc[EPU], sh[EPU], k0[EPU], k1[EPU], wk[NC][EPU];                                         \
+_Pragma("unroll")                                                                                                       \
+    for (int k = 0; k < NC; k++)                                                                                        \
+_Pragma("unroll")                                                                                                       \
+        for (int i = 0; i < EPU; i++) wk[k][i] = k < ncls ? w[k * C + c + i] : 0.f;                                     \
+    for (int pb = p_begin + row; pb < p_end; pb += 4 * rows) {                                                          \
+                                                      \
+        uint4 zu[4]; float gv[4][NC];                                                                                   \
+_Pragma("unroll")                                                                                                       \
+        for (int j = 0; j < 4; j++) {                                                                                   \
+            const int pj = pb + j * rows < p_end ? pb + j * rows : pb;                                                  \
+            int b, q; dhw.divmod(pj, b, q);                                                                             \
+_Pragma("unroll")                                                                                                       \
+            for (int k = 0; k < NC; k++) gv[j][k] = k < ncls ? dl[((size_t)b * ncls + k) * hw + q] : 0.f;               \
+            zu[j] = *reinterpret_cast<const uint4*>(z + (size_t)pj * C + c);                                            \
+        }                                                                                                               \
+_Pragma("unroll")                                                                                                       \
+        for (int j = 0; j < 4; j++) {                                                                                   \
+            const int p = pb + j * rows;                                                                                \
+            if (p >= p_end) break;                                                                                      \
+            const int g = dppg.div(p);                                                                                  \
+            if (g != gcur) {                        \
+                gcur = g;                                                                                               \
+_Pragma("unroll")                                                                                                       \
+                for (int i = 0; i < EPU; i++) {                                                                         \
+                    mean[i] = bn_row(bn, g, 0, C)[c + i]; inv[i] = bn_row(bn, g, 1, C)[c + i];                          \
+                    sc[i] = bn_row(bn, g, 2, C)[c + i]; sh[i] = bn_row(bn, g, 3, C)[c + i];                             \
+                    k0[i] = sums[((size_t)g * 2 + 0) * C + c + i] * invM;                                               \
+                    k1[i] = sums[((size_t)g * 2 + 1) * C + c + i] * invM;                                               \
+                }                                                                                                       \
+            }                                                                                                           \
+            float fz[EPU], o[EPU];                                                                                      \
+            Unit<T>::unpack(zu[j], fz);                                                                                 \
+_Pragma("unroll")                                                                                                       \
+            for (int i = 0; i < EPU; i++) {                                                                             \
+                float s = 0.f;                                                                                          \
+_Pragma("unroll")                                                                                                       \
+                for (int k = 0; k < NC; k++) if (k < ncls) s = fmaf(gv[j][k], wk[k][i], s);                             \
+                o[i] = s;                                                                                               \
+            }                                                                                                           \
+            Unit<T>::unpack(Unit<T>::pack(o), o);                    \
+_Pragma("unroll")                                                                                                       \
+            for (int i = 0; i < EPU; i++) {                                                                             \
+                const float gm = fmaf(fz[i], sc[i], sh[i]) > 0.f ? o[i] : 0.f;                                          \
+                const float xhat = (fz[i] - mean[i]) * inv[i];                                                          \
+                o[i] = sc[i] * (gm - k0[i] - xhat * k1[i]);                                                             \
+            }                                                                                                           \
+            if constexpr (SPLIT) {   \
+                const SplitOut so = {reinterpret_cast<bf16s*>(dz), 2 * C, 0, C};                                        \
+                store_split4(so, (size_t)p, c, o);                                                                      \
+            } else                                                                                                      \
+            *reinterpret_cast<uint4*>(dz + (size_t)p * C + c) = Unit<T>::pack(o);                                       \
+        }                                                                                                               \
+    }                                                                                                                   \
+
 template <typename T, int NC, bool SPLIT = false>
 __global__ __launch_bounds__(256) void outc_bn_bwd_apply_kernel(const float* __restrict__ dl, const float* __restrict__ w,
                                 const T* __restrict__ z, const float* __restrict__ bn, const float* __restrict__ sums,
                                 T* __restrict__ dz, int npix, int hw, int pix_per_group, int pix_per_block, int C, int ncls, FastDiv dhw, FastDiv dppg) {
-    constexpr int EPU = ET<T>::EPU;
-    const int CU = C / EPU, rows = 256 / CU, tid = threadIdx.x, cu = tid % CU, row = tid / CU, c = cu * EPU;
-    const int p_begin = blockIdx.x * pix_per_block, p_end = min(npix, p_begin + pix_per_block);
-    if (p_begin >= p_end) return;
-    const float invM = 1.f / (float)pix_per_group;
-    int gcur = -1;
-    float mean[EPU], inv[EPU], sc[EPU], sh[EPU], k0[EPU], k1[EPU], wk[NC][EPU];
-#pragma unroll
-    for (int k = 0; k < NC; k++)
-#pragma unroll
-        for (int i = 0; i < EPU; i++) wk[k][i] = k < ncls ? w[k * C + c + i] : 0.f;
-    for (int pb = p_begin + row; pb < p_end; pb += 4 * rows) {
-        uint4 zu[4]; float gv[4][NC];
-#pragma unroll
-        for (int j = 0; j < 4; j++) {
-            const int pj = pb + j * rows < p_end ? pb + j * rows : pb;
-            int b, q; dhw.divmod(pj, b, q);
-#pragma unroll
-            for (int k = 0; k < NC; k++) gv[j][k] = k < ncls ? dl[((size_t)b * ncls + k) * hw + q] : 0.f;
-            zu[j] = *reinterpret_cast<const uint4*>(z + (size_t)pj * C + c);
-        }
-#pragma unroll
-        for (int j = 0; j < 4; j++) {
-            const int p = pb + j * rows;
-            if (p >= p_end) break;
-            const int g = dppg.div(p);
-            if (g != gcur) {
-                gcur = g;
-#pragma unroll
-                for (int i = 0; i < EPU; i++) {
-                    mean[i] = bn_row(bn, g, 0, C)[c + i]; inv[i] = bn_row(bn, g, 1, C)[c + i];
-                    sc[i] = bn_row(bn, g, 2, C)[c + i]; sh[i] = bn_row(bn, g, 3, C)[c + i];
-                    k0[i] = sums[((size_t)g * 2 + 0) * C + c + i] * invM;
-                    k1[i] = sums[((size_t)g * 2 + 1) * C + c + i] * invM;
-                }
-            }
-            float fz[EPU], o[EPU];
-            Unit<T>::unpack(zu[j], fz);
-#pragma unroll
-            for (int i = 0; i < EPU; i++) {
-                float s = 0.f;
-#pragma unroll
-                for (int k = 0; k < NC; k++) if (k < ncls) s = fmaf(gv[j][k], wk[k][i], s);
-                o[i] = s;
-            }
-            Unit<T>::unpack(Unit<T>::pack(o), o);
-#pragma unroll
-            for (int i = 0; i < EPU; i++) {
-                const float gm = fmaf(fz[i], sc[i], sh[i]) > 0.f ? o[i] : 0.f;
-                const float xhat = (fz[i] - mean[i]) * inv[i];
-                o[i] = sc[i] * (gm - k0[i] - xhat * k1[i]);
-            }
-            if constexpr (SPLIT) {
-                const SplitOut so = {reinterpret_cast<bf16s*>(dz), 2 * C, 0, C};
-                store_split4(so, (size_t)p, c, o);
-            } else
-            *reinterpret_cast<uint4*>(dz + (size_t)p * C + c) = Unit<T>::pack(o);
-        }
-    }
+    OUTC_APPLY_BODY(blockIdx.x)
 }
 
 extern "C" int bdn_outc_bn_bwd_apply(int dtype, const float* dlogits, const float* w, const void* z, const float* bn,
@@ -922,6 +926,310 @@
                            FastDiv(H * W), FastDiv(W), FocalBwd{class_alpha, gamma, (float)inv, w_overlap, w_focal});
         BDN_CHECK_LAUNCH("criterion_bwd");
     }
+    return BDN_OK;
+}
+
+constexpr int FIN_QB = 4;
+
+static bool head_fused_ok(int dtype, int B, int H, int W, int C, int ncls, int reduce_w) {
+    if (dtype != BDN_BF16 && dtype != BDN_F32) return false;
+    if (B <= 0 || H <= 0 || W <= 0 || (size_t)B * H * W >= ((size_t)1 << 31)) return false;
+    if (C != 64 || ncls != 2 || reduce_w) return false;
+    return (ncls * W) % 4 == 0 && 3 * ncls * W / 4 <= 1024;
+}
+static inline int finish_lanes(int n4) { const int ln = 1024 / n4; return ln > 0 ? (ln > 16 ? 16 : ln) : 1; }
+
+extern "C" int bdn_head_fused_supported(int dtype, int B, int H, int W, int C, int ncls, int reduce_w) {
+    return head_fused_ok(dtype, B, H, W, C, ncls, reduce_w) ? 1 : 0;
+}
+extern "C" size_t bdn_head_fused_workspace_bytes(int B, int ncls, int H, int W) {
+    const size_t ov = bdn_overlap_workspace_bytes(B, ncls, H, W, 0);
+    return ov ? ov + sizeof(float) * ncls * W : 0;
+}
+
+__global__ __launch_bounds__(192) void tversky_finish_cells_kernel(float* __restrict__ sums, const float* __restrict__ part, int nblk,
+                                                                   float alpha, float beta, float eps, int nc, int LN, float* __restrict__ ratio) {
+    __shared__ float4 lane_sums[16 * 3 * FIN_QB];
+    __shared__ float4 cell[3 * FIN_QB];
+    const int n = 3 * nc, nq = nc / 4, tid = threadIdx.x;
+    const int qb = tid % FIN_QB, j = (tid / FIN_QB) % 3, l = tid / (3 * FIN_QB);
+    const int qc = blockIdx.x * FIN_QB + qb;
+    const bool on = qc < nq;
+    float4 a = make_float4(0.f, 0.f, 0.f, 0.f);
+    if (on) {
+        const float* src = part + (size_t)j * nc + 4 * qc;
+#pragma unroll 16
+        for (int b = l; b < nblk; b += LN) {
+            const float4 v = *reinterpret_cast<const float4*>(src + (size_t)b * n);
+            a.x += v.x; a.y += v.y; a.z += v.z; a.w += v.w;
+        }
+        lane_sums[tid] = a;
+    }
+    __syncthreads();
+    if (l == 0 && on) {
+        for (int k = 1; k < LN; k++) { const float4 v = lane_sums[k * 3 * FIN_QB + j * FIN_QB + qb]; a.x += v.x; a.y += v.y; a.z += v.z; a.w += v.w; }
+        cell[j * FIN_QB + qb] = a;
+    }
+    __syncthreads();
+    if (tid < FIN_QB && on) {
+        const float4 t4 = cell[qb], p4 = cell[FIN_QB + qb], n4 = cell[2 * FIN_QB + qb];
+        const float tpv[4] = {t4.x, t4.y, t4.z, t4.w}, fpv[4] = {p4.x, p4.y, p4.z, p4.w}, fnv[4] = {n4.x, n4.y, n4.z, n4.w};
+#pragma unroll
+        for (int e = 0; e < 4; e++) {
+#pragma clang fp contract(off)
+            const int i = 4 * qc + e;
+            const float tp = tpv[e], fp = fpv[e], fn = fnv[e];
+            const float D = tp + alpha * fp + beta * fn + eps;
+            ratio[i] = tp / D;
+            sums[i] = 1.f / D; sums[nc + i] = tp / (D * D); sums[2 * nc + i] = fn;
+        }
+    }
+}
+
+extern "C" int bdn_tversky_stats(const float* logits, const uint8_t* labels, float alpha, float beta, float eps,
+                                 float* ws, int B, int ncls, int H, int W, void* stream) {
+    if (!logits || !labels || !ws) BDN_FAIL(BDN_E_ARG, "tversky_stats: null pointer");
+    if (!head_fused_ok(BDN_F32, B, H, W, 64, ncls, 0)) BDN_FAIL(BDN_E_SHAPE, "tversky_stats: shape outside bdn_head_fused_supported (B=%d ncls=%d H=%d W=%d)", B, ncls, H, W);
+    hipStream_t st = (hipStream_t)stream;
+    const OverlapPlan p = overlap_plan(B, ncls, H, W, 0);
+    float* part = ws + p.n;
+    int32_t* pcounts = reinterpret_cast<int32_t*>(part + (size_t)p.nblk * p.n);
+    float* ratio = ws + bdn_overlap_workspace_bytes(B, ncls, H, W, 0) / sizeof(float);
+    hipLaunchKernelGGL((tversky_sums_kernel<2, false>), dim3(p.gx, p.gy), dim3(p.RL, p.CW), sizeof(float) * 256 * 3 * 2, st, logits, labels, part, pcounts, B, ncls, H, W, p.rpb, p.We, FastDiv(H), FocalStats{});
+    BDN_CHECK_LAUNCH("tversky_sums");
+    const int nc = ncls * W, LN = finish_lanes(p.n / 4);
+    hipLaunchKernelGGL(tversky_finish_cells_kernel, dim3((nc / 4 + FIN_QB - 1) / FIN_QB), dim3(3 * FIN_QB * LN), 0, st, ws, part, p.nblk, alpha, beta, eps, nc, LN, ratio);
+    BDN_CHECK_LAUNCH("tversky_finish_cells");
+    return BDN_OK;
+}
+
+__device__ __forceinline__ void tversky_grad_pixel(const float (&lg)[2], int t, const float (&cinv)[2], const float (&ctp)[2],
+                                                   float alpha, float beta, float norm, float (&out)[2]) {
+#pragma clang fp contract(off)
+    float l[2], dp[2]; float m = -INFINITY;
+#pragma unroll
+    for (int k = 0; k < 2; k++) { l[k] = lg[k]; m = fmaxf(m, l[k]); }
+    float den = 0.f;
+#pragma unroll
+    for (int k = 0; k < 2; k++) { l[k] = expf(l[k] - m); den += l[k]; }
+    float dot = 0.f;
+#pragma unroll
+    for (int k = 0; k < 2; k++) {
+        l[k] /= den;
+        const float invD = cinv[k], tpD2 = ctp[k];
+        const float tk = t == k ? 1.f : 0.f;
+        const float x = fmaf(-beta, tk, fmaf(alpha, 1.f - tk, tk));
+        dp[k] = norm * (tk * invD - tpD2 * x);
+        dot = fmaf(l[k], dp[k], dot);
+    }
+#pragma unroll
+    for (int k = 0; k < 2; k++) out[k] = l[k] * (dp[k] - dot);
+}
+
+struct TvGrad { const float* logits; const uint8_t* labels; const float* coef; float alpha, beta; int W; };
+template <typename T, int CUC>
+__global__ __launch_bounds__(256) void outc_bwd_tversky_kernel(TvGrad tv, float* __restrict__ dl, const T* __restrict__ z, const float* __restrict__ bn,
+                                const float* __restrict__ w, float* __restrict__ wpart, float* __restrict__ bs_partial,
+                                int npix, int hw, FastDiv dhw, FastDiv dW) {
+    constexpr int EPU = ET<T>::EPU, NC = 2, ncls = 2, C = 64, CU = CUC, rows = 256 / CU, PPW = 64 / CU, EV = 4 * PPW;
+    static_assert(CU * EPU == C, "64 channels");
+    extern __shared__ float sm[];
+    const int tid = threadIdx.x, cu = tid % CU, row = tid / CU, c = cu * EPU, lane = tid & 63;
+    const int e = lane % EV, ej = e / PPW, er = (tid >> 6) * PPW + e % PPW, src0 = lane / CU;
+    for (int i = tid; i < ncls * (C + 1); i += 256) sm[i] = 0.f;
+    float sc[EPU], sh[EPU], wk[NC][EPU], acc[NC][EPU], accb[NC], t0[EPU], t1[EPU];
+#pragma unroll
+    for (int i = 0; i < EPU; i++) { sc[i] = bn_row(bn, 0, 2, C)[c + i]; sh[i] = bn_row(bn, 0, 3, C)[c + i]; t0[i] = 0.f; t1[i] = 0.f; }
+#pragma unroll
+    for (int k = 0; k < NC; k++) {
+        accb[k] = 0.f;
+#pragma unroll
+        for (int i = 0; i < EPU; i++) { wk[k][i] = w[k * C + c + i]; acc[k][i] = 0.f; }
+    }
+    __syncthreads();
+    const int p_begin = blockIdx.x * rows * OUTC_BWD_ITERS, p_end = min(npix, p_begin + rows * OUTC_BWD_ITERS);
+    const int nW = ncls * tv.W;
+    const float norm = -1.f / (float)nW;
+    uint4 zu[4], zn[4]; float lgc[2], lgn[2], cic[2], cin[2], ctc[2], ctn[2]; int tc, tn; size_t oc, on;
+#define OUTC_TLOAD(zd_, lg_, ci_, ct_, t_, o_, p0_)                                                      \
+    {                                                                                                   \
+        _Pragma("unroll") for (int j = 0; j < 4; j++) {                                                  \
+            const int pj_ = (p0_) + j * rows + row < p_end ? (p0_) + j * rows + row : p_begin;           \
+            zd_[j] = *reinterpret_cast<const uint4*>(z + (size_t)pj_ * C + c);                          \
+        }                                                                                               \
+        const int pe_ = (p0_) + ej * rows + er < p_end ? (p0_) + ej * rows + er : p_begin;               \
+        int b_, q_, y_, x_; dhw.divmod(pe_, b_, q_); dW.divmod(q_, y_, x_);                              \
+        o_ = (size_t)b_ * ncls * hw + q_;                                                               \
+        _Pragma("unroll") for (int k = 0; k < NC; k++) {                                                 \
+            lg_[k] = tv.logits[o_ + (size_t)k * hw];                                                    \
+            ci_[k] = tv.coef[k * tv.W + x_]; ct_[k] = tv.coef[nW + k * tv.W + x_];                       \
+        }                                                                                               \
+        t_ = tv.labels[pe_];                                                                            \
+    }
+    OUTC_TLOAD(zu, lgc, cic, ctc, tc, oc, p_begin)
+    for (int p0 = p_begin; p0 < p_end; p0 += 4 * rows) {
+        { const int pn_ = p0 + 4 * rows < p_end ? p0 + 4 * rows : p0; OUTC_TLOAD(zn, lgn, cin, ctn, tn, on, pn_) }
+        float dv[NC], gv[4][NC];
+        tversky_grad_pixel(lgc, tc, cic, ctc, tv.alpha, tv.beta, norm, dv);
+        if (lane < EV && p0 + ej * rows + er < p_end) {
+#pragma unroll
+            for (int k = 0; k < NC; k++) dl[oc + (size_t)k * hw] = dv[k];
+        }
+#pragma unroll
+        for (int j = 0; j < 4; j++)
+#pragma unroll
+            for (int k = 0; k < NC; k++) gv[j][k] = __shfl(dv[k], j * PPW + src0);
+#pragma unroll
+        for (int j = 0; j < 4; j++) {
+            const int p = p0 + j * rows + row;
+            if (p < p_end) {
+                float g[NC], f[EPU], o[EPU];
+#pragma unroll
+                for (int k = 0; k < NC; k++) g[k] = gv[j][k];
+                Unit<T>::unpack(zu[j], f);
+#pragma unroll
+                for (int i = 0; i < EPU; i++) {
+                    const float a = to_f(from_f<T>(fmaxf(fmaf(f[i], sc[i], sh[i]), 0.f)));
+                    float s = 0.f;
+#pragma unroll
+                    for (int k = 0; k < NC; k++) { s = fmaf(g[k], wk[k][i], s); acc[k][i] = fmaf(g[k], a, acc[k][i]); }
+                    o[i] = s;
+                }
+                if (cu == 0) {
+#pragma unroll
+                    for (int k = 0; k < NC; k++) accb[k] += g[k];
+                }
+                const uint4 uo = Unit<T>::pack(o);
+                Unit<T>::unpack(uo, o);
+#pragma unroll
+                for (int i = 0; i < EPU; i++) {
+                    const float gm = fmaf(f[i], sc[i], sh[i]) > 0.f ? o[i] : 0.f;
+                    t0[i] += gm; t1[i] = fmaf(gm, f[i], t1[i]);
+                }
+            }
+        }
+#pragma unroll
+        for (int j = 0; j < 4; j++) zu[j] = zn[j];
+#pragma unroll
+        for (int k = 0; k < NC; k++) { lgc[k] = lgn[k]; cic[k] = cin[k]; ctc[k] = ctn[k]; }
+        tc = tn; oc = on;
+    }
+#undef OUTC_TLOAD
+    {
+        float* red = sm + ncls * (C + 1);
+#pragma unroll
+        for (int k = 0; k < NC; k++) {
+            __syncthreads();
+#pragma unroll
+            for (int i = 0; i < EPU; i++) red[tid * EPU + i] = acc[k][i];
+            if (cu == 0) red[256 * EPU + row] = accb[k];
+            __syncthreads();
+            for (int o = tid; o <= C; o += 256) {
+                float v = 0.f;
+                if (o < C) { const int ccu = o / EPU, i = o % EPU; for (int r = 0; r < rows; r++) v += red[(r * CU + ccu) * EPU + i]; }
+                else for (int r = 0; r < rows; r++) v += red[256 * EPU + r];
+                sm[k * (C + 1) + o] = v;
+            }
+        }
+    }
+    __syncthreads();
+    for (int i = tid; i < ncls * (C + 1); i += 256) wpart[(size_t)blockIdx.x * ncls * (C + 1) + i] = sm[i];
+    {
+        float* sred = sm + ncls * (C + 1);
+#pragma unroll
+        for (int i = 0; i < EPU; i++) { sred[(tid * EPU + i) * 2] = t0[i]; sred[(tid * EPU + i) * 2 + 1] = t1[i]; }
+        __syncthreads();
+        for (int o = tid; o < C * 2; o += 256) {
+            const int k = o & 1, cc = o >> 1, ccu = cc / EPU, i = cc % EPU;
+            float v = 0.f;
+            for (int r = 0; r < rows; r++) v += sred[((r * CU + ccu) * EPU + i) * 2 + k];
+            bs_partial[((size_t)blockIdx.x * 2 + k) * C + cc] = v;
+        }
+    }
+}
+
+extern "C" int bdn_outc_bwd_tversky(int dtype, const float* logits, const uint8_t* labels, const float* tv_ws, float alpha, float beta,
+                                    const void* z, const float* bn, const float* w, float* dlogits, float* bs_partial, float* ws,
+                                    int B, int H, int W, int C, int ncls, void* stream) {
+    if (!logits || !labels || !tv_ws || !z || !bn || !w || !dlogits || !bs_partial || !ws) BDN_FAIL(BDN_E_ARG, "outc_bwd_tversky: null pointer");
+    if (!head_fused_ok(dtype, B, H, W, C, ncls, 0)) BDN_FAIL(BDN_E_SHAPE, "outc_bwd_tversky: outside bdn_head_fused_supported (dtype=%d B=%d H=%d W=%d C=%d ncls=%d)", dtype, B, H, W, C, ncls);
+    hipStream_t st = (hipStream_t)stream; const int npix = B * H * W;
+    const unsigned grid = bdn_outc_bwd_rows(dtype, B, H, W, C);
+    const size_t smem = sizeof(float) * (ncls * (C + 1) + 256 * (dtype == BDN_BF16 ? 8 : 4) * 2);
+    const TvGrad tv{logits, labels, tv_ws, alpha, beta, W};
+    if (dtype == BDN_BF16) hipLaunchKernelGGL((outc_bwd_tversky_kernel<bf16s, 8>), dim3(grid), dim3(256), smem, st, tv, dlogits, (const bf16s*)z, bn, w, ws, bs_partial, npix, H * W, FastDiv(H * W), FastDiv(W));
+    else hipLaunchKernelGGL((outc_bwd_tversky_kernel<float, 16>), dim3(grid), dim3(256), smem, st, tv, dlogits, (const float*)z, bn, w, ws, bs_partial, npix, H * W, FastDiv(H * W), FastDiv(W));
+    BDN_CHECK_LAUNCH("outc_bwd_tversky");
+    return BDN_OK;
+}
+
+struct HeadTail { const float* wpart; int rows; float* dw; float* db; const float* ratio; int nc; const int32_t* pcounts; int ncblk; int32_t* counts; float* loss; };
+__device__ __forceinline__ void head_tail_block(const HeadTail& h, int blk, int C, int ncls) {
+    __shared__ double red[256];
+    __shared__ int ired[256];
+    const int tid = threadIdx.x;
+    if (blk == 0) {
+        double acc = 0.0;
+        for (int i = tid; i < h.nc; i += 256) acc += (double)h.ratio[i];
+        red[tid] = acc;
+        __syncthreads();
+        for (int s = 128; s > 0; s >>= 1) { if (tid < s) red[tid] += red[tid + s]; __syncthreads(); }
+        if (tid == 0) *h.loss = (float)(1.0 - red[0] / h.nc);
+        if (h.counts) {
+            const int j = tid & 3;
+            int v = 0;
+            for (int b = tid >> 2; b < h.ncblk; b += 64) v += h.pcounts[b * 4 + j];
+            ired[tid] = v;
+            __syncthreads();
+            for (int s2 = 128; s2 >= 4; s2 >>= 1) { if (tid < s2) ired[tid] += ired[tid + s2]; __syncthreads(); }
+            if (tid < 4) h.counts[tid] = ired[tid];
+        }
+        return;
+    }
+    float* fsm = reinterpret_cast<float*>(red);
+    const int o = blk - 1, n = ncls * (C + 1);
+    float a = 0.f;
+    for (int r = tid; r < h.rows; r += 256) a += h.wpart[(size_t)r * n + o];
+    fsm[tid] = a;
+    __syncthreads();
+    for (int st = 128; st >= 1; st >>= 1) {
+        if (tid < st) fsm[tid] += fsm[tid + st];
+        __syncthreads();
+    }
+    if (tid == 0) {
+        const int k = o / (C + 1), cc = o % (C + 1);
+        if (cc < C) h.dw[k * C + cc] = fsm[0]; else h.db[k] = fsm[0];
+    }
+}
+template <typename T>
+__global__ __launch_bounds__(256) void outc_bn_bwd_apply_tail_kernel(HeadTail h, int ntail, const float* __restrict__ dl, const float* __restrict__ w,
+                                const T* __restrict__ z, const float* __restrict__ bn, const float* __restrict__ sums,
+                                T* __restrict__ dz, int npix, int hw, int pix_per_group, int pix_per_block, int C, int ncls, FastDiv dhw, FastDiv dppg) {
+    if ((int)blockIdx.x < ntail) { head_tail_block(h, blockIdx.x, C, ncls); return; }
+    constexpr int NC = 2; constexpr bool SPLIT = false;
+    OUTC_APPLY_BODY(blockIdx.x - ntail)
+}
+
+extern "C" int bdn_outc_bn_bwd_apply_tail(int dtype, const float* dlogits, const float* w, const void* z, const float* bn,
+                                          int imgs_per_group, const float* sums, void* dz, const float* outc_ws, float* dw, float* db,
+                                          const float* tv_ws, float* loss, int32_t* counts, int B, int H, int W, int C, int ncls, void* stream) {
+    if (!dlogits || !w || !z || !bn || !sums || !dz || !outc_ws || !dw || !db || !tv_ws || !loss) BDN_FAIL(BDN_E_ARG, "outc_bn_bwd_apply_tail: null pointer");
+    if (!head_fused_ok(dtype, B, H, W, C, ncls, 0) || imgs_per_group <= 0 || B % imgs_per_group)
+        BDN_FAIL(BDN_E_SHAPE, "outc_bn_bwd_apply_tail: outside bdn_head_fused_supported (dtype=%d B=%d H=%d W=%d C=%d ncls=%d)", dtype, B, H, W, C, ncls);
+    hipStream_t st = (hipStream_t)stream;
+    const int npix = B * H * W, epu = dtype == BDN_BF16 ? 8 : 4, rows = 256 / (C / epu);
+    int ppb = (npix + 2047) / 2048; if (ppb < 2 * rows) ppb = 2 * rows; ppb = (ppb + rows - 1) / rows * rows;
+    const int ntail = 1 + ncls * (C + 1);
+    const unsigned grid = (npix + ppb - 1) / ppb + ntail;
+    const OverlapPlan p = overlap_plan(B, ncls, H, W, 0);
+    const float* part = tv_ws + p.n;
+    const HeadTail h{outc_ws, bdn_outc_bwd_rows(dtype, B, H, W, C), dw, db, tv_ws + bdn_overlap_workspace_bytes(B, ncls, H, W, 0) / sizeof(float), ncls * W,
+                     reinterpret_cast<const int32_t*>(part + (size_t)p.nblk * p.n), p.gx * p.gy, counts, loss};
+    if (dtype == BDN_BF16) hipLaunchKernelGGL(outc_bn_bwd_apply_tail_kernel<bf16s>, dim3(grid), dim3(256), 0, st, h, ntail, dlogits, w, (const bf16s*)z, bn, sums, (bf16s*)dz,
+                                              npix, H * W, imgs_per_group * H * W, ppb, C, ncls, FastDiv(H * W), FastDiv(imgs_per_group * H * W));
+    else hipLaunchKernelGGL(outc_bn_bwd_apply_tail_kernel<float>, dim3(grid), dim3(256), 0, st, h, ntail, dlogits, w, (const float*)z, bn, sums, (float*)dz,
+                            npix, H * W, imgs_per_group * H * W, ppb, C, ncls, FastDiv(H * W), FastDiv(imgs_per_group * H * W));
+    BDN_CHECK_LAUNCH("outc_bn_bwd_apply_tail");
     return BDN_OK;
 }
 
diff --git a/fabric_amd/engine.py b/fabric_amd/engine.py
--- a/fabric_amd/engine.py
+++ b/fabric_amd/engine.py
@@ -167,6 +167,18 @@
         return self._bwd
 
 
+@dataclass
+class HeadGrad:
+    logits: torch.Tensor
+    labels: torch.Tensor
+    tvws: torch.Tensor
+    alpha: float
+    beta: float
+    dlogits: torch.Tensor
+    loss: torch.Tensor
+    counts: torch.Tensor
+
+
 class BiDateEngine:
 
     def __init__(self, n_channels, n_classes, precision='bf16'):
@@ -190,6 +202,7 @@
         self.eval_fused = True
         self.eval_pair = (1, 2, 3, 4, 5)
         self.fold_bn_bwd = ('e1b', 'd4a')
+        self.head_fused = True
         self.wgrad_kernel = 0
         self.x3_bwd_terms = 2 if precision == 'bf16x3-fast' else 3
         self.x3_src_f32 = True
@@ -539,6 +552,10 @@
             return self.bwd_dtype
         return None
 
+    def head_fused_supported(self, B, H, W, need=None, dx=None):
+        return bool(self.head_fused and not self.x3 and self.chain_end(need, dx) != 'outc'
+                    and _lib.load().bdn_head_fused_supported(self.dt, B, H, W, self.layers[-1].cout, self.n_classes, 0))
+
     def chain_end(self, need, dx=None):
         if need is None or dx is not None:
             return None
@@ -576,6 +593,11 @@
             raise ValueError(f"bn_mode must be 'batch' or 'running', got {bn_mode!r}")
         frozen = bn_mode == 'running'
         B, H, W = ws.B, ws.H, ws.W
+        head = dlogits if isinstance(dlogits, HeadGrad) else None
+        if head is not None:
+            if not self.head_fused_supported(B, H, W, need, dx):
+                raise RuntimeError('backward: HeadGrad given outside head_fused_supported()')
+            dlogits = head.dlogits
         dev = dlogits.device
         dlogits = dlogits.contiguous().float()
         st = _lib.stream_ptr()
@@ -648,6 +670,12 @@
             dz = None if self.x3 else e(B, hk, wk, L.cout)
             out = ws.split_buf(('d', L.name), B * hk * wk * 2 * L.cout) if self.x3 else dz
             bn_bwd_finalize(L, B, B, rows)
+            if head is not None:
+                call('bdn_outc_bn_bwd_apply_tail', self.dt, ptr(dlogits), ptr(P['outc.conv.weight']), ptr(ws.z[L.name]),
+                     ptr(ws.bn[L.name]), B, ptr(sc['sums']), ptr(out), ptr(ws.outc_ws(self)), ptr(grads['outc.conv.weight']),
+                     ptr(grads['outc.conv.bias']), ptr(head.tvws), ptr(head.loss), ptr(head.counts), B, hk, wk, L.cout, self.n_classes, st)
+                ready(['outc.conv.weight', 'outc.conv.bias'])
+                return dz
             call('bdn_outc_bn_bwd_apply', self.mdt, ptr(dlogits), ptr(P['outc.conv.weight']), ptr(ws.z[L.name]),
                  ptr(ws.bn[L.name]), B, ptr(sc['sums']), ptr(out), B, hk, wk, L.cout, self.n_classes, st)
             return dz
@@ -761,10 +789,15 @@
 
         def chain():
             L4b = by['d4b']
-            call('bdn_outc_bwd', self.dt, ptr(dlogits), ptr(ws.z['d4b']), ptr(ws.bn['d4b']), ptr(P['outc.conv.weight']),
-                 None, ptr(grads['outc.conv.weight']), ptr(grads['outc.conv.bias']), ptr(ws.stats),
-                 ptr(ws.outc_ws(self)), B, H, W, L4b.cout, self.n_classes, st)
-            ready(['outc.conv.weight', 'outc.conv.bias'])
+            if head is not None:
+                call('bdn_outc_bwd_tversky', self.dt, ptr(head.logits), ptr(head.labels), ptr(head.tvws), float(head.alpha), float(head.beta),
+                     ptr(ws.z['d4b']), ptr(ws.bn['d4b']), ptr(P['outc.conv.weight']), ptr(dlogits), ptr(ws.stats),
+                     ptr(ws.outc_ws(self)), B, H, W, L4b.cout, self.n_classes, st)
+            else:
+                call('bdn_outc_bwd', self.dt, ptr(dlogits), ptr(ws.z['d4b']), ptr(ws.bn['d4b']), ptr(P['outc.conv.weight']),
+                     None, ptr(grads['outc.conv.weight']), ptr(grads['outc.conv.bias']), ptr(ws.stats),
+                     ptr(ws.outc_ws(self)), B, H, W, L4b.cout, self.n_classes, st)
+                ready(['outc.conv.weight', 'outc.conv.bias'])
             if end == 'outc':
                 return
             dA, ldA, rows = None, 0, _lib.load().bdn_outc_bwd_rows(self.dt, B, H, W, L4b.cout)
diff --git a/fabric_amd/train_step.py b/fabric_amd/train_step.py
--- a/fabric_amd/train_step.py
+++ b/fabric_amd/train_step.py
@@ -3,7 +3,7 @@
 
 from . import _lib
 from . import optim as _optim
-from .engine import param_order
+from .engine import HeadGrad, param_order
 from .parallel import FlatLayout, GradBucketer
 
 
@@ -397,8 +397,10 @@
     def _tversky_loss(self, logits, labels, st):
         B, C, H, W = logits.shape
         dev = logits.device
+        eng = self.model.engine()
+        fused = logits.dtype == torch.float32 and logits.is_contiguous() and eng.head_fused_supported(B, H, W, self._need)
         if self._tv is None or self._tv[3] != (B, C, H, W):
-            n = _lib.load().bdn_overlap_workspace_bytes(B, C, H, W, 0) // 4
+            n = max(_lib.load().bdn_overlap_workspace_bytes(B, C, H, W, 0), _lib.load().bdn_head_fused_workspace_bytes(B, C, H, W)) // 4
             self._tv = (torch.empty(n, dtype=torch.float32, device=dev), torch.empty((), dtype=torch.float32, device=dev),
                         torch.empty(4, dtype=torch.int32, device=dev), (B, C, H, W))
         tvws, loss, counts, _ = self._tv
@@ -406,6 +408,10 @@
             labels = labels.to(torch.uint8)
         labels = labels.contiguous()
         dlogits = torch.empty_like(logits)
+        if fused:
+            _lib.call('bdn_tversky_stats', logits.data_ptr(), labels.data_ptr(), float(self.alpha), float(self.beta), float(self.eps),
+                      tvws.data_ptr(), B, C, H, W, st)
+            return loss, counts, HeadGrad(logits, labels, tvws, self.alpha, self.beta, dlogits, loss, counts)
         _lib.call('bdn_tversky', logits.data_ptr(), labels.data_ptr(), float(self.alpha), float(self.beta),
                   float(self.eps), tvws.data_ptr(), loss.data_ptr(), counts.data_ptr(), dlogits.data_ptr(), B, C, H, W, st)
         return loss, counts, dlogits
diff --git a/include/bidate_hip.h b/include/bidate_hip.h
--- a/include/bidate_hip.h
+++ b/include/bidate_hip.h
@@ -180,6 +180,17 @@
                      int reduce_w, float* ws, float* loss, int32_t* counts, float* dlogits,
                      int B, int ncls, int H, int W, void* stream);
 
+int bdn_head_fused_supported(int dtype, int B, int H, int W, int C, int ncls, int reduce_w);
+size_t bdn_head_fused_workspace_bytes(int B, int ncls, int H, int W);
+int bdn_tversky_stats(const float* logits, const uint8_t* labels, float alpha, float beta, float eps,
+                      float* ws, int B, int ncls, int H, int W, void* stream);
+int bdn_outc_bwd_tversky(int dtype, const float* logits, const uint8_t* labels, const float* ws, float alpha, float beta,
+                         const void* z, const float* bn, const float* w, float* dlogits, float* bs_partial, float* outc_ws,
+                         int B, int H, int W, int C, int ncls, void* stream);
+int bdn_outc_bn_bwd_apply_tail(int dtype, const float* dlogits, const float* w, const void* z, const float* bn,
+                               int imgs_per_group, const float* sums, void* dz, const float* outc_ws, float* dw, float* db,
+                               const float* ws, float* loss, int32_t* counts, int B, int H, int W, int C, int ncls, void* stream);
+
 size_t bdn_focal_workspace_bytes(void);
 int bdn_focal(const float* logits, const uint8_t* labels, float gamma, const float* alpha, int size_average,
               void* ws, float* loss, int32_t* counts, float* dlogits,
```

Measured after the change: 10620 (median of 3 runs). Within noise of the previous version (+0.3%).
